# cv-stuttgart/PCFA

Hardware: AMD Instinct MI355X
Metric: attack_steps_per_sec (higher is better)
Workload: dtype f32; 1 GPU; RAFT, 1 synthetic 436x1024 pair per GPU (padded 440x1024), disjoint delta, change_of_variables, delta_bound=0.005, zero target, L-BFGS max_iter=10; weights=random:1234, parallelism=pairs sharded 1/GPU, closure_launch=hipGraph replay

## Files before the change

include/pcfa_hip.h:

```cpp
#ifndef PCFA_HIP_H
#define PCFA_HIP_H

#include <stddef.h>
#include <stdint.h>

#ifdef __cplusplus
extern "C" {
#endif

#define PCFA_OK 0
#define PCFA_ERR_INVALID_ARG (-1)
#define PCFA_ERR_UNSUPPORTED (-2)
#define PCFA_ERR_WORKSPACE (-3)

#if defined(__GNUC__)
#define PCFA_API __attribute__((visibility("default")))
#else
#define PCFA_API
#endif

#define PCFA_MAX_LEVELS 8
#define PCFA_ABI_VERSION 2

#define PCFA_LOSS_AEE 0
#define PCFA_LOSS_MSE 1
#define PCFA_LOSS_COSIM 2

#define PCFA_BOX_CLIPPING 0
#define PCFA_BOX_CHANGE_OF_VARIABLES 1

PCFA_API int pcfa_abi_version(void);
PCFA_API int pcfa_timing_arm(void* start_event, void* stop_event, int nth);

PCFA_API int pcfa_null_launch(void* stream);
PCFA_API int pcfa_poison_lds(unsigned pattern, void* stream);
PCFA_API int pcfa_peek_lds(unsigned* out, int n, void* stream);
PCFA_API long long pcfa_calib_mfma_f32(float* scratch, int blocks, int iters, void* stream);
PCFA_API int pcfa_calib_copy(const float* src, float* dst, long long n_floats, void* stream);
PCFA_API const char* pcfa_status_string(int status);


PCFA_API long long pcfa_corr_slab_floats(int H, int W, int num_levels);
PCFA_API long long pcfa_corr_level_offset(int H, int W, int num_levels, int level, int* h_l, int* w_l);

PCFA_API long long pcfa_corr_tiled_index(int H, int W, int num_levels, int level, int y, int x);

PCFA_API int pcfa_corr_f2ext_fwd(const float* fmap2, float* f2ext, int B, int D, int H, int W,
                        int num_levels, void* stream);

PCFA_API int pcfa_corr_pyramid_fwd(const float* fmap1, const float* f2ext, float* pyr, int B, int D,
                          int H, int W, int num_levels, void* stream);

PCFA_API size_t pcfa_corr_pyramid_bwd_workspace_bytes(int B, int D, int H, int W, int num_levels);
PCFA_API int pcfa_corr_pyramid_bwd(const float* dpyr, const float* fmap1, const float* f2ext,
                          float* dfmap1, float* dfmap2, void* workspace, size_t workspace_bytes,
                          int B, int D, int H, int W, int num_levels, void* stream);
PCFA_API size_t pcfa_corr_pyramid_bwd_windows_workspace_bytes(int B, int D, int H, int W, int num_levels);
PCFA_API int pcfa_corr_pyramid_bwd_windows(const float* dpyr, const float* fmap1, const float* f2ext, float* dfmap1,
                                  float* dfmap2, void* workspace, size_t workspace_bytes,
                                  const float* const* coords, int n_coords, int radius, int B, int D, int H, int W,
                                  int num_levels, void* stream);

PCFA_API int pcfa_corr_lookup_fwd(const float* pyr, const float* coords, float* out, int B, int H, int W,
                         int num_levels, int radius, void* stream);

PCFA_API int pcfa_corr_lookup_bwd(float* dpyr, const float* coords, const float* grad_out, int B, int H,
                         int W, int num_levels, int radius, void* stream);

PCFA_API size_t pcfa_corr_ondemand_workspace_bytes(int B, int D, int H, int W, int num_levels);
PCFA_API int pcfa_corr_ondemand_prepare(const float* fmap1, const float* fmap2, void* workspace, int B, int D, int H,
                               int W, int num_levels, void* stream);
PCFA_API int pcfa_corr_ondemand_fwd(const void* workspace, const float* coords, float* out, int B, int D, int H, int W,
                           int num_levels, int radius, void* stream);
PCFA_API int pcfa_corr_ondemand_bwd(void* workspace, const float* coords, const float* grad_out, int accumulate, int B,
                           int D, int H, int W, int num_levels, int radius, void* stream);
PCFA_API int pcfa_corr_ondemand_finish(const void* workspace, float* dfmap1, float* dfmap2, int B, int D, int H, int W,
                              int num_levels, void* stream);

PCFA_API size_t pcfa_gemm_f32_workspace_bytes(int M, int N, int batch, int splits);
PCFA_API int pcfa_gemm_f32(const float* A, const float* B, float* C, int M, int N, int K, long long lda, long long ldb,
                  long long ldc, int a_kmajor, int b_kmajor, int batch, long long bsA, long long bsB, long long bsC,
                  float alpha, int splits, void* workspace, size_t workspace_bytes, void* stream);
PCFA_API int pcfa_softmax_rows_fwd(const float* x, float* y, long long rows, int cols, void* stream);
PCFA_API int pcfa_softmax_rows_bwd(const float* y, const float* grad_y, float* grad_x, long long rows, int cols,
                          void* stream);

PCFA_API int pcfa_attn_stream_lse(const float* q, const float* k, float* lse, int BH, int N, int d, float scale,
                         void* stream);
PCFA_API int pcfa_attn_stream_fwd(const float* q, const float* k, const float* v, const float* lse, float* out, int BH,
                         int N, int d, float scale, void* stream);
PCFA_API int pcfa_attn_stream_dv(const float* q, const float* k, const float* g, const float* lse, float* dv, int BH,
                        int N, int d, float scale, void* stream);
PCFA_API int pcfa_attn_stream_delta(const float* g, const float* out, float* delta, long long rows, int d,
                           int accumulate, void* stream);
PCFA_API int pcfa_attn_stream_dqk(const float* q, const float* k, const float* lse, const float* G, const float* V,
                         const float* delta, float* dq, float* dk, int BH, int N, int d, int n, float scale,
                         void* stream);

PCFA_API long long pcfa_lookup_convc1_packed_floats(int Cout);
PCFA_API int pcfa_lookup_convc1_pack_weights(const float* weight, float* packed, int Cout, int Cin, void* stream);
PCFA_API int pcfa_lookup_convc1_fwd(const float* pyr, const float* coords, const float* packed, const float* bias,
                           float* out, int B, int H, int W, int num_levels, int radius, int Cout, int relu,
                           void* stream);
PCFA_API int pcfa_lookup_convc1_bwd(float* dpyr, const float* coords, const float* packed, const float* out,
                           const float* grad_out, int B, int H, int W, int num_levels, int radius, int Cout,
                           int relu, void* stream);

PCFA_API int pcfa_spatial_corr_out_size(int iH, int iW, int kH, int kW, int padH, int padW, int dilH,
                               int dilW, int dH, int dW, int* oH, int* oW);
PCFA_API int pcfa_spatial_corr_fwd(const float* in1, const float* in2, float* out, int B, int C, int iH,
                          int iW, int kH, int kW, int patchH, int patchW, int padH, int padW,
                          int dilH, int dilW, int dil_patchH, int dil_patchW, int dH, int dW,
                          void* stream);
PCFA_API int pcfa_spatial_corr_bwd(const float* in1, const float* in2, const float* grad_out,
                          float* grad_in1, float* grad_in2, int B, int C, int iH, int iW, int kH,
                          int kW, int patchH, int patchW, int padH, int padW, int dilH, int dilW,
                          int dil_patchH, int dil_patchW, int dH, int dW, void* stream);

PCFA_API int pcfa_cost_volume9_fwd(const float* in1, const float* in2, float* out, int B, int C, int iH, int iW,
                          float scale, float slope, void* stream);
PCFA_API int pcfa_cost_volume9_bwd(const float* in1, const float* in2, const float* fwd_out, const float* grad_out,
                          float* grad_in1, float* grad_in2, int B, int C, int iH, int iW, float scale,
                          float slope, void* stream);

PCFA_API int pcfa_flownet_corr_out_size(int H, int W, int pad_size, int kernel_size, int max_displacement,
                                        int stride1, int stride2, int* out_channels, int* oH, int* oW);
PCFA_API int pcfa_flownet_corr_fwd(const float* in1, const float* in2, float* out, int B, int C, int H, int W,
                                   int pad_size, int kernel_size, int max_displacement, int stride1, int stride2,
                                   void* stream);
PCFA_API int pcfa_flownet_corr_bwd(const float* in1, const float* in2, const float* grad_out, float* grad_in1,
                                   float* grad_in2, int B, int C, int H, int W, int pad_size, int kernel_size,
                                   int max_displacement, int stride1, int stride2, void* stream);
PCFA_API int pcfa_resample2d_fwd(const float* in1, const float* flow, float* out, int B, int C, int iH, int iW,
                                 int H, int W, int kernel_size, int bilinear, void* stream);
PCFA_API int pcfa_resample2d_bwd(const float* in1, const float* flow, const float* grad_out, float* grad_in1,
                                 float* grad_flow, int B, int C, int iH, int iW, int H, int W, int kernel_size,
                                 int bilinear, void* stream);
PCFA_API int pcfa_channelnorm_fwd(const float* in, float* out, int B, int C, long long plane, int norm_deg,
                                  void* stream);
PCFA_API int pcfa_channelnorm_bwd(const float* in, const float* out, const float* grad_out, float* grad_in, int B,
                                  int C, long long plane, int norm_deg, void* stream);


PCFA_API int pcfa_box_transform_fwd(const float* image, const float* delta, float* out, int B,
                           long long n_per_item, int change_of_variables, double eps_box,
                           float scale, void* stream);
PCFA_API int pcfa_box_transform_bwd(const float* image, const float* delta, const float* grad_out,
                           float* grad_image, float* grad_delta, int B, long long n_per_item,
                           int change_of_variables, double eps_box, float scale, void* stream);

PCFA_API int pcfa_pm1_pair_fwd(const float* image1, const float* image2, float* pair, float* ctx, int B, long long n,
                               void* stream);
PCFA_API int pcfa_pm1_pair_bwd(const float* grad_pair, const float* grad_ctx, float* grad_image1, float* grad_image2, int B,
                               long long n, void* stream);

PCFA_API int pcfa_extract_deltas_fwd(const float* nw_input, const float* image, float* delta,
                            long long n, int change_of_variables, double eps_box, void* stream);
PCFA_API int pcfa_extract_deltas_bwd(const float* nw_input, const float* grad_delta, float* grad_nw_input,
                            long long n, int change_of_variables, double eps_box, void* stream);

PCFA_API int pcfa_extract_deltas_joint_fwd(const float* nw_delta, const float* images_max,
                                  const float* images_min, float* delta, long long n,
                                  void* stream);
PCFA_API int pcfa_extract_deltas_joint_bwd(const float* nw_delta, const float* images_max,
                                  const float* images_min, const float* grad_delta,
                                  float* grad_nw_delta, long long n, void* stream);

PCFA_API size_t pcfa_flow_loss_workspace_bytes(void);
PCFA_API int pcfa_flow_loss_fwd(const float* pred, const long long pred_strides[4], const float* target,
                       const long long target_strides[4], int B, int H, int W,
                       const float* delta1, long long n1, const float* delta2, long long n2,
                       float delta_bound, float mu, int f_type, float* out_scalars,
                       void* workspace, void* stream);
PCFA_API int pcfa_flow_loss_bwd(const float* pred, const long long pred_strides[4], const float* target,
                       const long long target_strides[4], int B, int H, int W,
                       const float* delta1, long long n1, const float* delta2, long long n2,
                       float mu, int f_type, int joint, const float* fwd_scalars,
                       const float* grad_loss, float* grad_pred, float* grad_delta1,
                       float* grad_delta2, void* stream);

PCFA_API int pcfa_gru_gates_fwd(const float* zc, const float* rc, const float* h, const float* bias_z,
                       const float* bias_r, const float* add_z, const float* add_r, float* z, float* r,
                       float* rh, long long n, int plane, int channels, void* stream);
PCFA_API int pcfa_gru_gates_bwd(const float* z, const float* r, const float* h, const float* dz, const float* drh,
                       float* dzc, float* drc, float* dh, long long n, void* stream);
PCFA_API int pcfa_gru_gates_bwd_acc(const float* z, const float* r, const float* h, const float* dz, const float* drh,
                           const float* dh_in, float* dzc, float* drc, float* dh, long long n, void* stream);
PCFA_API int pcfa_gru_update_fwd(const float* z, const float* qc, const float* h, const float* bias_q,
                        const float* add_q, float* q, float* hnew, long long n, int plane, int channels,
                        void* stream);
PCFA_API int pcfa_gru_update_bwd(const float* z, const float* q, const float* h, const float* g, float* dz,
                        float* dqc, float* dh, long long n, void* stream);

PCFA_API long long pcfa_sepconv5_packed_floats(int Cout, int Cin);
PCFA_API int pcfa_sepconv5_algo(int use_winograd);
PCFA_API int pcfa_sepconv5_uses_winograd(int B, int Ca, int Cb, int Cout, int H, int W, int vertical);
PCFA_API int pcfa_sepconv5_pack_weights(const float* w, float* fwd_packed, float* bwd_packed, int Cout, int Cin,
                               void* stream);
PCFA_API int pcfa_sepconv5_fwd(const float* in_a, int Ca, const float* in_b, int Cb, const float* w_packed,
                      float* out, int B, int Cout, int H, int W, int vertical, void* stream);

PCFA_API int pcfa_sepconv5_fwd_split(const float* in_a, int Ca, const float* in_b, int Cb, const float* w_packed,
                            float* out_a, int Cout_a, int accumulate_a, float* out_b, int accumulate_b, int B,
                            int Cout, int H, int W, int vertical, void* stream);
PCFA_API int pcfa_sepconv5_fwd_split_masked(const float* in_a, int Ca, const float* in_b, int Cb, const float* w_packed,
                                   float* out_a, int Cout_a, int accumulate_a, float* out_b, int accumulate_b,
                                   const float* mask_b, int mask_channels, int B, int Cout, int H, int W,
                                   int vertical, void* stream);

PCFA_API int pcfa_sepconv5_gru_gates_fwd(const float* h, int C, const float* rest, int Cr, const float* w_packed,
                                const float* add_zr, float* z, float* r, float* rh, int B, int H, int W,
                                int vertical, void* stream);
PCFA_API int pcfa_sepconv5_gru_update_fwd(const float* rh, int C, const float* rest, int Cr, const float* w_packed,
                                 const float* add_q, const float* z, const float* h, float* q, float* hnew, int B,
                                 int H, int W, int vertical, void* stream);
PCFA_API int pcfa_sepconv5_gru_gates_bwd(const float* dqc, int C, int Cr, const float* w_packed_bwd, const float* z,
                                const float* r, const float* h, const float* dz, const float* dh_in, float* dzr,
                                float* dh, float* d_rest, int accumulate_rest, int B, int H, int W, int vertical,
                                void* stream);
PCFA_API int pcfa_sepconv5_gru_update_bwd(const float* dzr, int C, int Cr, const float* w_packed_bwd, const float* dh_acc,
                                 const float* z_prev, const float* q_prev, const float* h_prev, float* dz_prev,
                                 float* dqc_prev, float* dh_prev, float* d_rest, int B, int H, int W, int vertical,
                                 void* stream);

PCFA_API long long pcfa_conv3x3_packed_floats(int K, int N);
PCFA_API int pcfa_conv3x3_pack_weights(const float* w, float* fwd_packed, float* bwd_packed, int Cout, int Cin,
                              void* stream);
PCFA_API int pcfa_conv3x3_fwd(const float* x, const float* packed, const float* bias, float* out, int B, int K, int N,
                     int H, int W, int relu, void* stream);
PCFA_API int pcfa_conv3x3_act_fwd(const float* x, const float* packed, const float* bias, float* out, int B, int K,
                         int N, int H, int W, int act, float slope, void* stream);
PCFA_API int pcfa_leaky_relu_fwd(const float* x, float* y, float slope, long long n, void* stream);
PCFA_API int pcfa_leaky_relu_bwd(const float* out, const float* grad_out, float* grad_x, float slope, long long n,
                        void* stream);
PCFA_API int pcfa_conv3x3_act_fwd_pair(const float* x, const float* packed, const float* bias, float* out, int K, int N,
                              const float* x2, const float* packed2, const float* bias2, float* out2, int K2, int N2,
                              int H, int W, int act, float slope, void* stream);
PCFA_API int pcfa_conv3x3_fused_bwd(const float* g, const float* packed_bwd, const float* mask, const float* addend,
                           float* grad_in, int B, int K, int N, int H, int W, void* stream);
PCFA_API int pcfa_conv3x3_masked_fwd(const float* x, const float* packed, const float* mask, float* out, int B, int K,
                            int N, int H, int W, void* stream);
PCFA_API int pcfa_conv3x3_algo(int B, int K, int N, int H, int W);
PCFA_API size_t pcfa_conv3x3_workspace_bytes(int B, int K, int N, int H, int W);
PCFA_API int pcfa_conv3x3_run(const float* x, const float* packed, const float* bias, const float* mask,
                     const float* addend, float* out, int B, int K, int N, int H, int W, int act, float slope,
                     int mask_channels, void* workspace, size_t workspace_bytes, void* stream);

PCFA_API int pcfa_bias_relu_fwd(const float* x, const float* bias, float* out, long long n, int plane, int channels,
                       void* stream);
PCFA_API int pcfa_relu_bwd(const float* out, const float* grad_out, float* grad_x, long long n, void* stream);
PCFA_API int pcfa_relu_bwd2(const float* out, const float* out2, const float* grad_out, float* grad_x, float* grad_x2,
                   long long n, void* stream);

PCFA_API int pcfa_conv_fewin_fwd(const float* x, const float* w, const float* bias, float* out, int B, int Cin, int N,
                                 int H, int W, int ksize, int relu, void* stream);
PCFA_API long long pcfa_conv_fewin_packed_floats(int Cin, int N, int ksize);
PCFA_API int pcfa_conv_fewin_pack(const float* w, float* packed, int Cin, int N, int ksize, void* stream);
PCFA_API int pcfa_conv_fewin_packed_fwd(const float* x, const float* packed, const float* bias, float* out, int B, int Cin,
                               int N, int H, int W, int ksize, int relu, void* stream);

PCFA_API int pcfa_conv_s2_supported(int Cin, int N, int ksize, int H, int W);
PCFA_API long long pcfa_conv_s2_packed_floats(int Cin, int N, int ksize);
PCFA_API int pcfa_conv_s2_pack(const float* w, float* packed, int Cin, int N, int ksize, void* stream);
PCFA_API int pcfa_conv_s2_fwd(const float* x, const float* packed, const float* bias, float* out, int B, int Cin, int N,
                              int H, int W, int ksize, int act, float slope, void* stream);
PCFA_API int pcfa_conv_s2_bwd_supported(int Cin, int N, int ksize, int H, int W);
PCFA_API long long pcfa_conv_s2_bwd_packed_floats(int Cin, int N, int ksize);
PCFA_API int pcfa_conv_s2_bwd_pack(const float* w, float* packed, int Cin, int N, int ksize, void* stream);
PCFA_API int pcfa_conv_s2_bwd(const float* grad_out, const float* packed, float* grad_x, int B, int Cin, int N, int H, int W,
                              int ksize, void* stream);
PCFA_API long long pcfa_conv_s2_ds_packed_floats(int Cin, int N);
PCFA_API int pcfa_conv_s2_ds_pack(const float* w, const float* wd, float* packed, int Cin, int N, void* stream);
PCFA_API int pcfa_conv_s2_ds_fwd(const float* x, const float* packed, const float* bias, float* out, const float* bias_d,
                                 float* out_d, int B, int Cin, int N, int H, int W, int act, float slope, void* stream);
PCFA_API long long pcfa_conv_s2_ds_bwd_packed_floats(int Cin, int N);
PCFA_API int pcfa_conv_s2_ds_bwd_pack(const float* w, const float* wd, float* packed, int Cin, int N, void* stream);
PCFA_API int pcfa_conv_s2_ds_bwd(const float* grad_out, const float* grad_out_d, const float* packed, float* grad_x, int B,
                                 int Cin, int N, int H, int W, void* stream);

PCFA_API int pcfa_pwc_warp_fwd(const float* x, const float* flo, float* out, int B, int C, int H, int W,
                               float mask_threshold, float flow_scale, void* stream);
PCFA_API int pcfa_pwc_warp_bwd(const float* x, const float* flo, const float* grad_out, float* grad_x,
                               float* grad_flo, int B, int C, int H, int W, float mask_threshold, float flow_scale,
                               void* stream);
PCFA_API size_t pcfa_pwc_warp_bwd_det_workspace_bytes(int B, int C, int H, int W);
PCFA_API int pcfa_pwc_warp_bwd_det(const float* x, const float* flo, const float* grad_out, float* grad_x,
                          float* grad_flo, void* workspace, size_t workspace_bytes, int B, int C, int H, int W,
                          float mask_threshold, float flow_scale, void* stream);

PCFA_API int pcfa_spynet_warp_fwd(const float* x, const float* flo, const float* hor, const float* ver, float* out, int B,
                                  int C, int H, int W, float sx, float sy, void* stream);
PCFA_API size_t pcfa_spynet_warp_bwd_workspace_bytes(int B, int C, int H, int W);
PCFA_API int pcfa_spynet_warp_bwd(const float* x, const float* flo, const float* hor, const float* ver,
                                  const float* grad_out, float* grad_x, float* grad_flo, void* workspace,
                                  size_t workspace_bytes, int B, int C, int H, int W, float sx, float sy, void* stream);

PCFA_API int pcfa_conv7x7_tile(int Cout, int* mt, int* cot);
PCFA_API long long pcfa_conv7x7_packed_floats(int Cin, int Cout);
PCFA_API int pcfa_conv7x7(const float* x, const float* mask, const float* packed, const float* bias, const float* addend,
                          float* out, int B, int Cin, int Cout, int H, int W, int relu, void* stream);

PCFA_API int pcfa_conv_gather_tile(int Cout, int* mt, int* cot);
PCFA_API int pcfa_conv_gather_supported(int stride, int taps, int npar);
PCFA_API long long pcfa_conv_gather_packed_floats(int Cin, int Cout, int taps, int npar);
PCFA_API int pcfa_conv_gather(const float* x, const float* mask, float mask_slope, const float* packed, const float* bias,
                              float* out, int B, int Cin, int H, int W, int Cout, int OH, int OW, int stride, int taps,
                              int npar, int off0, int off1, int act, float slope, void* stream);

PCFA_API size_t pcfa_resample2d_bwd_det_workspace_bytes(int B, int C, int H, int W);
PCFA_API int pcfa_resample2d_bwd_det(const float* in1, const float* flow, const float* grad_out, float* grad_in1,
                                     float* grad_flow, void* workspace, size_t workspace_bytes, int B, int C, int H, int W,
                                     void* stream);

PCFA_API int pcfa_upsample_nearest4_fwd(const float* in, float* out, int planes, int H, int W, float s, int div,
                                        void* stream);
PCFA_API int pcfa_upsample_nearest4_bwd(const float* grad_out, float* grad_in, int planes, int H, int W, float s, int div,
                                        void* stream);

PCFA_API size_t pcfa_conv3x3_fewout_workspace_bytes(int B, int K, int N, int H, int W);
PCFA_API int pcfa_conv3x3_fewout_fwd(const float* x, const float* w, const float* bias, float* out, void* workspace,
                                     int B, int K, int N, int H, int W, void* stream);
PCFA_API int pcfa_conv3x3_fewout_bwd(const float* grad_out, const float* w, const float* addend, float* grad_x, int B,
                                     int K, int N, int H, int W, void* stream);

PCFA_API size_t pcfa_deconv4s2_fewout_workspace_bytes(int B, int K, int N, int H, int W);
PCFA_API int pcfa_deconv4s2_fewout_fwd(const float* x, const float* w, const float* bias, float* out, void* workspace,
                                       int B, int K, int N, int H, int W, void* stream);
PCFA_API int pcfa_deconv4s2_fewout_bwd(const float* grad_out, const float* w, float* grad_x, int B, int K, int N, int H,
                                       int W, void* stream);

PCFA_API int pcfa_upsample_bilinear_fwd(const float* in, float* out, int planes, int H, int W, int factor, float mul,
                                        void* stream);
PCFA_API int pcfa_upsample_bilinear_bwd(const float* grad_out, float* grad_in, int planes, int H, int W, int factor,
                                        float mul, void* stream);

PCFA_API size_t pcfa_instnorm_workspace_bytes(int planes, long long plane);
PCFA_API int pcfa_instnorm_fwd(const float* x, float* y, float* mean_rstd, void* workspace, int planes,
                               long long plane, float eps, int relu, void* stream);
PCFA_API int pcfa_instnorm_bwd(const float* x, const float* mean_rstd, const float* grad_out, float* grad_x,
                               void* workspace, int planes, long long plane, int relu, void* stream);
PCFA_API int pcfa_add_relu_fwd(const float* a, const float* b, float* out, long long n, void* stream);
PCFA_API int pcfa_convex_upsample_fwd(const float* flow, const float* mask, float* out, int N, int H, int W, void* stream);
PCFA_API long long pcfa_convex_upsample_workspace_floats(int N, int H, int W);
PCFA_API int pcfa_convex_upsample_bwd(const float* flow, const float* mask, const float* grad_out, float* grad_flow,
                             float* grad_mask, float* workspace, int N, int H, int W, void* stream);

PCFA_API int pcfa_flow_step(const float* coords1, const float* delta, const float* coords0, float* coords1_new,
                   float* flow_new, long long n, void* stream);

PCFA_API int pcfa_sum_n(const float* const* srcs, int n, float* out, long long numel, void* stream);

PCFA_API int pcfa_avg_epe(const float* flow1, const long long strides1[4], const float* flow2,
                 const long long strides2[4], int B, int H, int W, float* out, void* workspace,
                 void* stream);
PCFA_API int pcfa_sum_squares(const float* x, long long n, float* out, void* workspace, void* stream);

PCFA_API size_t pcfa_lbfgs_workspace_floats(void);
PCFA_API int pcfa_lbfgs_pair(const float* g, float* g_prev, const float* d, float t, float* y_out, float* s_out,
                             float* scal4, float* workspace, int update_prev, long long n, void* stream);
PCFA_API int pcfa_lbfgs_direction(const float* g, const float* S, const float* Y, const float* ro, const float* H,
                                  float* al, float* d, float* workspace, int first, int count, int capacity,
                                  long long ld, long long n, void* stream);

PCFA_API size_t pcfa_lbfgs_gram_state_bytes(int capacity);
PCFA_API size_t pcfa_lbfgs_gram_workspace_bytes(int capacity, long long ld);
PCFA_API int pcfa_lbfgs_gram_reset(void* state, int capacity, void* stream);
PCFA_API int pcfa_lbfgs_gram_update(const float* g, float* g_prev, const float* d, float t, float* S, float* Y,
                                    void* state, void* workspace, int capacity, long long ld, void* stream);
PCFA_API int pcfa_lbfgs_gram_direction(const float* g, const float* S, const float* Y, void* state, float* d,
                                       float* out_gtd_dmax, void* workspace, int capacity, long long ld, void* stream);

#ifdef __cplusplus
}
#endif
#endif
```

pcfa_amd/_hip.py:

```python
import ctypes
import os
from ctypes import c_char_p, c_double, c_float, c_int, c_longlong, c_size_t, c_uint, c_void_p, POINTER

ABI_VERSION = 2
LIB_PATH = os.environ.get("PCFA_HIP_LIB") or os.path.join(os.path.dirname(os.path.abspath(__file__)), "lib",
                                                          "libpcfa_hip.so")

PCFA_LOSS = {"aee": 0, "mse": 1, "cosim": 2}


class HipLibraryError(RuntimeError):
    pass


_P = c_void_p
_S4 = POINTER(c_longlong)

SIGNATURES = {
    "pcfa_abi_version": (c_int, []),
    "pcfa_timing_arm": (c_int, [_P, _P, c_int]),
    "pcfa_null_launch": (c_int, [_P]),
    "pcfa_poison_lds": (c_int, [c_uint, _P]),
    "pcfa_peek_lds": (c_int, [_P, c_int, _P]),
    "pcfa_calib_mfma_f32": (c_longlong, [_P, c_int, c_int, _P]),
    "pcfa_calib_copy": (c_int, [_P, _P, c_longlong, _P]),
    "pcfa_status_string": (c_char_p, [c_int]),
    "pcfa_corr_slab_floats": (c_longlong, [c_int, c_int, c_int]),
    "pcfa_corr_level_offset": (c_longlong, [c_int, c_int, c_int, c_int, POINTER(c_int), POINTER(c_int)]),
    "pcfa_corr_tiled_index": (c_longlong, [c_int, c_int, c_int, c_int, c_int, c_int]),
    "pcfa_corr_f2ext_fwd": (c_int, [_P, _P, c_int, c_int, c_int, c_int, c_int, _P]),
    "pcfa_corr_pyramid_fwd": (c_int, [_P, _P, _P, c_int, c_int, c_int, c_int, c_int, _P]),
    "pcfa_corr_pyramid_bwd_workspace_bytes": (c_size_t, [c_int, c_int, c_int, c_int, c_int]),
    "pcfa_corr_pyramid_bwd": (c_int, [_P, _P, _P, _P, _P, _P, c_size_t, c_int, c_int, c_int, c_int, c_int, _P]),
    "pcfa_corr_pyramid_bwd_windows_workspace_bytes": (c_size_t, [c_int, c_int, c_int, c_int, c_int]),
    "pcfa_corr_pyramid_bwd_windows": (c_int, [_P, _P, _P, _P, _P, _P, c_size_t, POINTER(c_void_p), c_int, c_int, c_int,
                                              c_int, c_int, c_int, c_int, _P]),
    "pcfa_corr_lookup_fwd": (c_int, [_P, _P, _P, c_int, c_int, c_int, c_int, c_int, _P]),
    "pcfa_corr_lookup_bwd": (c_int, [_P, _P, _P, c_int, c_int, c_int, c_int, c_int, _P]),
    "pcfa_corr_ondemand_workspace_bytes": (c_size_t, [c_int, c_int, c_int, c_int, c_int]),
    "pcfa_corr_ondemand_prepare": (c_int, [_P, _P, _P, c_int, c_int, c_int, c_int, c_int, _P]),
    "pcfa_corr_ondemand_fwd": (c_int, [_P, _P, _P, c_int, c_int, c_int, c_int, c_int, c_int, _P]),
    "pcfa_corr_ondemand_bwd": (c_int, [_P, _P, _P, c_int, c_int, c_int, c_int, c_int, c_int, c_int, _P]),
    "pcfa_corr_ondemand_finish": (c_int, [_P, _P, _P, c_int, c_int, c_int, c_int, c_int, _P]),
    "pcfa_gemm_f32_workspace_bytes": (c_size_t, [c_int, c_int, c_int, c_int]),
    "pcfa_gemm_f32": (c_int, [_P, _P, _P, c_int, c_int, c_int, c_longlong, c_longlong, c_longlong, c_int, c_int, c_int,
                              c_longlong, c_longlong, c_longlong, c_float, c_int, _P, c_size_t, _P]),
    "pcfa_softmax_rows_fwd": (c_int, [_P, _P, c_longlong, c_int, _P]),
    "pcfa_softmax_rows_bwd": (c_int, [_P, _P, _P, c_longlong, c_int, _P]),
    "pcfa_attn_stream_lse": (c_int, [_P, _P, _P, c_int, c_int, c_int, c_float, _P]),
    "pcfa_attn_stream_fwd": (c_int, [_P, _P, _P, _P, _P, c_int, c_int, c_int, c_float, _P]),
    "pcfa_attn_stream_dv": (c_int, [_P, _P, _P, _P, _P, c_int, c_int, c_int, c_float, _P]),
    "pcfa_attn_stream_delta": (c_int, [_P, _P, _P, c_longlong, c_int, c_int, _P]),
    "pcfa_attn_stream_dqk": (c_int, [_P, _P, _P, _P, _P, _P, _P, _P, c_int, c_int, c_int, c_int, c_float, _P]),
    "pcfa_lookup_convc1_packed_floats": (c_longlong, [c_int]),
    "pcfa_lookup_convc1_pack_weights": (c_int, [_P, _P, c_int, c_int, _P]),
    "pcfa_lookup_convc1_fwd": (c_int, [_P, _P, _P, _P, _P, c_int, c_int, c_int, c_int, c_int, c_int, c_int, _P]),
    "pcfa_lookup_convc1_bwd": (c_int, [_P, _P, _P, _P, _P, c_int, c_int, c_int, c_int, c_int, c_int, c_int, _P]),
    "pcfa_spatial_corr_out_size": (c_int, [c_int] * 10 + [POINTER(c_int), POINTER(c_int)]),
    "pcfa_spatial_corr_fwd": (c_int, [_P, _P, _P] + [c_int] * 16 + [_P]),
    "pcfa_spatial_corr_bwd": (c_int, [_P, _P, _P, _P, _P] + [c_int] * 16 + [_P]),
    "pcfa_cost_volume9_fwd": (c_int, [_P, _P, _P, c_int, c_int, c_int, c_int, c_float, c_float, _P]),
    "pcfa_cost_volume9_bwd": (c_int, [_P, _P, _P, _P, _P, _P, c_int, c_int, c_int, c_int, c_float, c_float, _P]),
    "pcfa_flownet_corr_out_size": (c_int, [c_int] * 7 + [POINTER(c_int)] * 3),
    "pcfa_flownet_corr_fwd": (c_int, [_P, _P, _P] + [c_int] * 9 + [_P]),
    "pcfa_flownet_corr_bwd": (c_int, [_P, _P, _P, _P, _P] + [c_int] * 9 + [_P]),
    "pcfa_resample2d_fwd": (c_int, [_P, _P, _P] + [c_int] * 8 + [_P]),
    "pcfa_resample2d_bwd": (c_int, [_P, _P, _P, _P, _P] + [c_int] * 8 + [_P]),
    "pcfa_channelnorm_fwd": (c_int, [_P, _P, c_int, c_int, c_longlong, c_int, _P]),
    "pcfa_channelnorm_bwd": (c_int, [_P, _P, _P, _P, c_int, c_int, c_longlong, c_int, _P]),
    "pcfa_box_transform_fwd": (c_int, [_P, _P, _P, c_int, c_longlong, c_int, c_double, c_float, _P]),
    "pcfa_box_transform_bwd": (c_int, [_P, _P, _P, _P, _P, c_int, c_longlong, c_int, c_double, c_float, _P]),
    "pcfa_pm1_pair_fwd": (c_int, [_P, _P, _P, _P, c_int, c_longlong, _P]),
    "pcfa_pm1_pair_bwd": (c_int, [_P, _P, _P, _P, c_int, c_longlong, _P]),
    "pcfa_extract_deltas_fwd": (c_int, [_P, _P, _P, c_longlong, c_int, c_double, _P]),
    "pcfa_extract_deltas_bwd": (c_int, [_P, _P, _P, c_longlong, c_int, c_double, _P]),
    "pcfa_extract_deltas_joint_fwd": (c_int, [_P, _P, _P, _P, c_longlong, _P]),
    "pcfa_extract_deltas_joint_bwd": (c_int, [_P, _P, _P, _P, _P, c_longlong, _P]),
    "pcfa_flow_loss_workspace_bytes": (c_size_t, []),
    "pcfa_flow_loss_fwd": (c_int, [_P, _S4, _P, _S4, c_int, c_int, c_int, _P, c_longlong, _P, c_longlong,
                                   c_float, c_float, c_int, _P, _P, _P]),
    "pcfa_flow_loss_bwd": (c_int, [_P, _S4, _P, _S4, c_int, c_int, c_int, _P, c_longlong, _P, c_longlong,
                                   c_float, c_int, c_int, _P, _P, _P, _P, _P, _P]),
    "pcfa_gru_gates_fwd": (c_int, [_P] * 10 + [c_longlong, c_int, c_int, _P]),
    "pcfa_gru_gates_bwd": (c_int, [_P] * 8 + [c_longlong, _P]),
    "pcfa_gru_update_fwd": (c_int, [_P] * 7 + [c_longlong, c_int, c_int, _P]),
    "pcfa_gru_update_bwd": (c_int, [_P] * 7 + [c_longlong, _P]),
    "pcfa_sepconv5_packed_floats": (c_longlong, [c_int, c_int]),
    "pcfa_sepconv5_algo": (c_int, [c_int]),
    "pcfa_sepconv5_uses_winograd": (c_int, [c_int] * 7),
    "pcfa_sepconv5_pack_weights": (c_int, [_P, _P, _P, c_int, c_int, _P]),
    "pcfa_sepconv5_fwd": (c_int, [_P, c_int, _P, c_int, _P, _P, c_int, c_int, c_int, c_int, c_int, _P]),
    "pcfa_sepconv5_fwd_split": (c_int, [_P, c_int, _P, c_int, _P, _P, c_int, c_int, _P, c_int, c_int, c_int, c_int, c_int,
                                        c_int, _P]),
    "pcfa_gru_gates_bwd_acc": (c_int, [_P, _P, _P, _P, _P, _P, _P, _P, _P, c_longlong, _P]),
    "pcfa_sepconv5_fwd_split_masked": (c_int, [_P, c_int, _P, c_int, _P, _P, c_int, c_int, _P, c_int, _P, c_int, c_int,
                                               c_int, c_int, c_int, c_int, _P]),
    "pcfa_sepconv5_gru_gates_fwd": (c_int, [_P, c_int, _P, c_int, _P, _P, _P, _P, _P, c_int, c_int, c_int, c_int, _P]),
    "pcfa_sepconv5_gru_update_fwd": (c_int, [_P, c_int, _P, c_int, _P, _P, _P, _P, _P, _P, c_int, c_int, c_int, c_int, _P]),
    "pcfa_sepconv5_gru_gates_bwd": (c_int, [_P, c_int, c_int, _P, _P, _P, _P, _P, _P, _P, _P, _P, c_int, c_int, c_int,
                                            c_int, c_int, _P]),
    "pcfa_sepconv5_gru_update_bwd": (c_int, [_P, c_int, c_int, _P, _P, _P, _P, _P, _P, _P, _P, _P, c_int, c_int, c_int,
                                             c_int, _P]),
    "pcfa_convex_upsample_fwd": (c_int, [_P, _P, _P, c_int, c_int, c_int, _P]),
    "pcfa_convex_upsample_workspace_floats": (c_longlong, [c_int, c_int, c_int]),
    "pcfa_convex_upsample_bwd": (c_int, [_P, _P, _P, _P, _P, _P, c_int, c_int, c_int, _P]),
    "pcfa_flow_step": (c_int, [_P, _P, _P, _P, _P, c_longlong, _P]),
    "pcfa_conv3x3_act_fwd_pair": (c_int, [_P, _P, _P, _P, c_int, c_int, _P, _P, _P, _P, c_int, c_int, c_int, c_int, c_int,
                                          c_float, _P]),
    "pcfa_relu_bwd2": (c_int, [_P, _P, _P, _P, _P, c_longlong, _P]),
    "pcfa_conv3x3_fused_bwd": (c_int, [_P, _P, _P, _P, _P, c_int, c_int, c_int, c_int, c_int, _P]),
    "pcfa_conv3x3_masked_fwd": (c_int, [_P, _P, _P, _P, c_int, c_int, c_int, c_int, c_int, _P]),
    "pcfa_conv3x3_algo": (c_int, [c_int] * 5),
    "pcfa_conv3x3_workspace_bytes": (c_size_t, [c_int] * 5),
    "pcfa_conv3x3_run": (c_int, [_P] * 6 + [c_int] * 6 + [c_float, c_int, _P, c_size_t, _P]),
    "pcfa_conv3x3_packed_floats": (c_longlong, [c_int, c_int]),
    "pcfa_conv3x3_pack_weights": (c_int, [_P, _P, _P, c_int, c_int, _P]),
    "pcfa_conv3x3_fwd": (c_int, [_P, _P, _P, _P, c_int, c_int, c_int, c_int, c_int, c_int, _P]),
    "pcfa_conv3x3_act_fwd": (c_int, [_P, _P, _P, _P, c_int, c_int, c_int, c_int, c_int, c_int, c_float, _P]),
    "pcfa_leaky_relu_fwd": (c_int, [_P, _P, c_float, c_longlong, _P]),
    "pcfa_leaky_relu_bwd": (c_int, [_P, _P, _P, c_float, c_longlong, _P]),
    "pcfa_lbfgs_gram_state_bytes": (c_size_t, [c_int]),
    "pcfa_lbfgs_gram_workspace_bytes": (c_size_t, [c_int, c_longlong]),
    "pcfa_lbfgs_gram_reset": (c_int, [_P, c_int, _P]),
    "pcfa_lbfgs_gram_update": (c_int, [_P, _P, _P, c_float, _P, _P, _P, _P, c_int, c_longlong, _P]),
    "pcfa_lbfgs_gram_direction": (c_int, [_P, _P, _P, _P, _P, _P, _P, c_int, c_longlong, _P]),
    "pcfa_lbfgs_workspace_floats": (c_size_t, []),
    "pcfa_lbfgs_pair": (c_int, [_P, _P, _P, c_float, _P, _P, _P, _P, c_int, c_longlong, _P]),
    "pcfa_lbfgs_direction": (c_int, [_P, _P, _P, _P, _P, _P, _P, _P, c_int, c_int, c_int, c_longlong, c_longlong,
                                     _P]),
    "pcfa_bias_relu_fwd": (c_int, [_P, _P, _P, c_longlong, c_int, c_int, _P]),
    "pcfa_relu_bwd": (c_int, [_P, _P, _P, c_longlong, _P]),
    "pcfa_conv_fewin_packed_floats": (c_longlong, [c_int, c_int, c_int]),
    "pcfa_conv_s2_supported": (c_int, [c_int, c_int, c_int, c_int, c_int]),
    "pcfa_conv_s2_packed_floats": (c_longlong, [c_int, c_int, c_int]),
    "pcfa_conv_s2_pack": (c_int, [_P, _P, c_int, c_int, c_int, _P]),
    "pcfa_conv_s2_fwd": (c_int, [_P, _P, _P, _P, c_int, c_int, c_int, c_int, c_int, c_int, c_int, c_float, _P]),
    "pcfa_conv_s2_bwd_supported": (c_int, [c_int, c_int, c_int, c_int, c_int]),
    "pcfa_conv_s2_bwd_packed_floats": (c_longlong, [c_int, c_int, c_int]),
    "pcfa_conv_s2_bwd_pack": (c_int, [_P, _P, c_int, c_int, c_int, _P]),
    "pcfa_conv_s2_bwd": (c_int, [_P, _P, _P, c_int, c_int, c_int, c_int, c_int, c_int, _P]),
    "pcfa_conv_s2_ds_packed_floats": (c_longlong, [c_int, c_int]),
    "pcfa_conv_s2_ds_pack": (c_int, [_P, _P, _P, c_int, c_int, _P]),
    "pcfa_conv_s2_ds_fwd": (c_int, [_P, _P, _P, _P, _P, _P, c_int, c_int, c_int, c_int, c_int, c_int, c_float, _P]),
    "pcfa_conv_s2_ds_bwd_packed_floats": (c_longlong, [c_int, c_int]),
    "pcfa_conv_s2_ds_bwd_pack": (c_int, [_P, _P, _P, c_int, c_int, _P]),
    "pcfa_conv_s2_ds_bwd": (c_int, [_P, _P, _P, _P, c_int, c_int, c_int, c_int, c_int, _P]),
    "pcfa_conv_fewin_pack": (c_int, [_P, _P, c_int, c_int, c_int, _P]),
    "pcfa_conv_fewin_packed_fwd": (c_int, [_P, _P, _P, _P, c_int, c_int, c_int, c_int, c_int, c_int, c_int, _P]),
    "pcfa_conv_fewin_fwd": (c_int, [_P, _P, _P, _P, c_int, c_int, c_int, c_int, c_int, c_int, c_int, _P]),
    "pcfa_pwc_warp_fwd": (c_int, [_P, _P, _P, c_int, c_int, c_int, c_int, c_float, c_float, _P]),
    "pcfa_pwc_warp_bwd": (c_int, [_P, _P, _P, _P, _P, c_int, c_int, c_int, c_int, c_float, c_float, _P]),
    "pcfa_pwc_warp_bwd_det_workspace_bytes": (c_size_t, [c_int, c_int, c_int, c_int]),
    "pcfa_pwc_warp_bwd_det": (c_int, [_P, _P, _P, _P, _P, _P, c_size_t, c_int, c_int, c_int, c_int, c_float, c_float, _P]),
    "pcfa_conv3x3_fewout_workspace_bytes": (c_size_t, [c_int, c_int, c_int, c_int, c_int]),
    "pcfa_conv3x3_fewout_fwd": (c_int, [_P, _P, _P, _P, _P, c_int, c_int, c_int, c_int, c_int, _P]),
    "pcfa_conv3x3_fewout_bwd": (c_int, [_P, _P, _P, _P, c_int, c_int, c_int, c_int, c_int, _P]),
    "pcfa_deconv4s2_fewout_workspace_bytes": (c_size_t, [c_int, c_int, c_int, c_int, c_int]),
    "pcfa_deconv4s2_fewout_fwd": (c_int, [_P, _P, _P, _P, _P, c_int, c_int, c_int, c_int, c_int, _P]),
    "pcfa_deconv4s2_fewout_bwd": (c_int, [_P, _P, _P, c_int, c_int, c_int, c_int, c_int, _P]),
    "pcfa_spynet_warp_fwd": (c_int, [_P, _P, _P, _P, _P, c_int, c_int, c_int, c_int, c_float, c_float, _P]),
    "pcfa_spynet_warp_bwd_workspace_bytes": (c_size_t, [c_int, c_int, c_int, c_int]),
    "pcfa_spynet_warp_bwd": (c_int, [_P, _P, _P, _P, _P, _P, _P, _P, c_size_t, c_int, c_int, c_int, c_int, c_float, c_float,
                                     _P]),
    "pcfa_conv7x7_tile": (c_int, [c_int, POINTER(c_int), POINTER(c_int)]),
    "pcfa_conv7x7_packed_floats": (c_longlong, [c_int, c_int]),
    "pcfa_conv7x7": (c_int, [_P, _P, _P, _P, _P, _P, c_int, c_int, c_int, c_int, c_int, c_int, _P]),
    "pcfa_conv_gather_tile": (c_int, [c_int, POINTER(c_int), POINTER(c_int)]),
    "pcfa_conv_gather_supported": (c_int, [c_int, c_int, c_int]),
    "pcfa_conv_gather_packed_floats": (c_longlong, [c_int, c_int, c_int, c_int]),
    "pcfa_conv_gather": (c_int, [_P, _P, c_float, _P, _P, _P] + [c_int] * 12 + [c_int, c_float, _P]),
    "pcfa_resample2d_bwd_det_workspace_bytes": (c_size_t, [c_int, c_int, c_int, c_int]),
    "pcfa_resample2d_bwd_det": (c_int, [_P, _P, _P, _P, _P, _P, c_size_t, c_int, c_int, c_int, c_int, _P]),
    "pcfa_upsample_nearest4_fwd": (c_int, [_P, _P, c_int, c_int, c_int, c_float, c_int, _P]),
    "pcfa_upsample_nearest4_bwd": (c_int, [_P, _P, c_int, c_int, c_int, c_float, c_int, _P]),
    "pcfa_upsample_bilinear_fwd": (c_int, [_P, _P, c_int, c_int, c_int, c_int, c_float, _P]),
    "pcfa_upsample_bilinear_bwd": (c_int, [_P, _P, c_int, c_int, c_int, c_int, c_float, _P]),
    "pcfa_instnorm_workspace_bytes": (c_size_t, [c_int, c_longlong]),
    "pcfa_instnorm_fwd": (c_int, [_P, _P, _P, _P, c_int, c_longlong, c_float, c_int, _P]),
    "pcfa_instnorm_bwd": (c_int, [_P, _P, _P, _P, _P, c_int, c_longlong, c_int, _P]),
    "pcfa_add_relu_fwd": (c_int, [_P, _P, _P, c_longlong, _P]),
    "pcfa_sum_n": (c_int, [POINTER(c_void_p), c_int, _P, c_longlong, _P]),
    "pcfa_avg_epe": (c_int, [_P, _S4, _P, _S4, c_int, c_int, c_int, _P, _P, _P]),
    "pcfa_sum_squares": (c_int, [_P, c_longlong, _P, _P, _P]),
}

_lib = None


def load(path=None):
    global _lib
    if _lib is not None and path is None:
        return _lib
    p = path or LIB_PATH
    if not os.path.exists(p):
        raise HipLibraryError(
            "libpcfa_hip.so not found at %s -- build it with `python -c 'import __graft_entry__ as g; g.build()'` "
            "or `make -C pcfa_amd/csrc`. pcfa_amd has no CPU fallback." % p)
    try:
        lib = ctypes.CDLL(p)
    except OSError as e:
        raise HipLibraryError("cannot load %s: %s" % (p, e))
    for name, (res, args) in SIGNATURES.items():
        try:
            fn = getattr(lib, name)
        except AttributeError:
            raise HipLibraryError("%s does not export %s (stale build?)" % (p, name))
        fn.restype = res
        fn.argtypes = args
    v = lib.pcfa_abi_version()
    if v != ABI_VERSION:
        raise HipLibraryError("ABI version mismatch: library %d, binding %d" % (v, ABI_VERSION))
    if path is None:
        _lib = lib
    return lib


def check(status, what):
    if status != 0:
        msg = load().pcfa_status_string(status)
        raise RuntimeError("%s failed: %s (status %d)" % (what, msg.decode() if msg else "?", status))


def strides4(t):
    return (c_longlong * 4)(*t.stride())
```

pcfa_amd/csrc/conv3x3_fewout.hip:

```cpp
#include "common.hpp"

namespace {

constexpr int FO_PX = 64;
constexpr int FO_WAVES = 8;
constexpr int FO_FWD_WAVES = 16;

template <int N>
__global__ __launch_bounds__(FO_PX* FO_FWD_WAVES) void conv3x3_fewout_fwd_kernel(
    const float* __restrict__ x, const float* __restrict__ w, const float* __restrict__ bias,
    float* __restrict__ out, int K, int H, int W, int splits, int kper) {
  __shared__ float red[FO_FWD_WAVES][N][FO_PX];
  const int lane = threadIdx.x & 63;
  const int wave = __builtin_amdgcn_readfirstlane(threadIdx.x >> 6);
  const int nb = gridDim.y / splits;
  const int b = blockIdx.y / splits, split = blockIdx.y - b * splits;
  const int kbeg = split * kper, kend = min(K, kbeg + kper);
  const long long plane = (long long)H * W;
  const long long p = (long long)blockIdx.x * FO_PX + lane;
  const bool live = p < plane;
  const int y = live ? (int)(p / W) : 0, xx = live ? (int)(p % W) : 0;
  int off[9];
  bool ok[9];
#pragma unroll
  for (int ky = 0; ky < 3; ++ky)
#pragma unroll
    for (int kx = 0; kx < 3; ++kx) {
      const int yy = y + ky - 1, xq = xx + kx - 1;
      ok[ky * 3 + kx] = live && yy >= 0 && yy < H && xq >= 0 && xq < W;
      off[ky * 3 + kx] = ok[ky * 3 + kx] ? yy * W + xq : 0;
    }
  float acc[N];
#pragma unroll
  for (int o = 0; o < N; ++o) acc[o] = 0.f;
  const float* xb = x + (size_t)b * K * plane;
  constexpr int U = 8;
  for (int c0 = kbeg + wave; c0 < kend; c0 += U * FO_FWD_WAVES) {
    float v[U][9];
#pragma unroll
    for (int u = 0; u < U; ++u) {
      const int c = c0 + u * FO_FWD_WAVES;
      const float* xc = xb + (size_t)(c < kend ? c : c0) * plane;
#pragma unroll
      for (int k = 0; k < 9; ++k) {
        const float t = xc[off[k]];
        v[u][k] = ok[k] ? t : 0.f;
      }
    }
#pragma unroll
    for (int u = 0; u < U; ++u) {
      const int c = c0 + u * FO_FWD_WAVES;
      if (c < kend) {
#pragma unroll
        for (int o = 0; o < N; ++o) {
          const float* wc = w + ((size_t)o * K + c) * 9;
#pragma unroll
          for (int k = 0; k < 9; ++k) acc[o] += wc[k] * v[u][k];
        }
      }
    }
  }
#pragma unroll
  for (int o = 0; o < N; ++o) red[wave][o][lane] = acc[o];
  __syncthreads();
  for (int e = threadIdx.x; e < N * FO_PX; e += FO_PX * FO_FWD_WAVES) {
    const int o = e / FO_PX, l = e % FO_PX;
    float s = 0.f;
#pragma unroll
    for (int g = 0; g < FO_FWD_WAVES; ++g) s += red[g][o][l];
    const long long q = (long long)blockIdx.x * FO_PX + l;
    if (q < plane) {
      if (splits > 1) out[(((size_t)split * nb + b) * N + o) * plane + q] = s;
      else out[((size_t)b * N + o) * plane + q] = s + (bias ? bias[o] : 0.f);
    }
  }
}

constexpr int FO_SEG = 72;
constexpr int FO_UL = 4;

template <int N>
__global__ __launch_bounds__(FO_PX* FO_FWD_WAVES) void conv3x3_fewout_fwd_lds_kernel(
    const float* __restrict__ x, const float* __restrict__ w, const float* __restrict__ bias,
    float* __restrict__ out, int K, int H, int W, int splits, int kper) {
  typedef float f32x4 __attribute__((ext_vector_type(4)));
  __shared__ float red[FO_FWD_WAVES][N][FO_PX];
  __shared__ __attribute__((aligned(16))) float seg[FO_FWD_WAVES][FO_UL][3][FO_SEG];
  const int lane = threadIdx.x & 63;
  const int wave = __builtin_amdgcn_readfirstlane(threadIdx.x >> 6);
  const int nb = gridDim.y / splits;
  const int b = blockIdx.y / splits, split = blockIdx.y - b * splits;
  const int kbeg = split * kper, kend = min(K, kbeg + kper);
  const long long plane = (long long)H * W;
  const long long p0 = (long long)blockIdx.x * FO_PX;
  const long long p = p0 + lane;
  const bool live = p < plane;
  const int y = live ? (int)(p / W) : 0, xx = live ? (int)(p % W) : 0;
  bool ok[9];
#pragma unroll
  for (int ky = 0; ky < 3; ++ky)
#pragma unroll
    for (int kx = 0; kx < 3; ++kx) {
      const int yy = y + ky - 1, xq = xx + kx - 1;
      ok[ky * 3 + kx] = live && yy >= 0 && yy < H && xq >= 0 && xq < W;
    }
  const int lr = lane / 18, lm = lane - lr * 18;
  long long s4[3];
  int dsh[3];
#pragma unroll
  for (int r = 0; r < 3; ++r) {
    const long long st = p0 + (long long)(r - 1) * W - 1;
    s4[r] = st & ~3LL;
    dsh[r] = (int)(st - s4[r]);
  }
  const long long myidx = (lr == 0 ? s4[0] : (lr == 1 ? s4[1] : s4[2])) + 4 * lm;
  const bool myok = lane < 54 && myidx >= 0 && myidx + 3 < plane;
  const long long myoff = myok ? myidx : 0;

  float acc[N];
#pragma unroll
  for (int o = 0; o < N; ++o) acc[o] = 0.f;
  const float* xb = x + (size_t)b * K * plane;
  float* mine = &seg[wave][0][0][0];
  for (int c0 = kbeg + wave; c0 < kend; c0 += FO_UL * FO_FWD_WAVES) {
    f32x4 t[FO_UL];
#pragma unroll
    for (int u = 0; u < FO_UL; ++u) {
      const int c = c0 + u * FO_FWD_WAVES;
      const float* xc = xb + (size_t)(c < kend ? c : c0) * plane;
      const f32x4 q = *reinterpret_cast<const f32x4*>(xc + myoff);
      t[u] = myok ? q : (f32x4)(0.f);
    }
#pragma unroll
    for (int u = 0; u < FO_UL; ++u)
      if (lane < 54) *reinterpret_cast<f32x4*>(mine + (u * 3 + lr) * FO_SEG + 4 * lm) = t[u];
    __builtin_amdgcn_wave_barrier();
#pragma unroll
    for (int u = 0; u < FO_UL; ++u) {
      const int c = c0 + u * FO_FWD_WAVES;
      if (c < kend) {
        float v[9];
#pragma unroll
        for (int r = 0; r < 3; ++r)
#pragma unroll
          for (int kx = 0; kx < 3; ++kx) {
            const float q = mine[(u * 3 + r) * FO_SEG + dsh[r] + lane + kx];
            v[3 * r + kx] = ok[3 * r + kx] ? q : 0.f;
          }
#pragma unroll
        for (int o = 0; o < N; ++o) {
          const float* wc = w + ((size_t)o * K + c) * 9;
#pragma unroll
          for (int k = 0; k < 9; ++k) acc[o] += wc[k] * v[k];
        }
      }
    }
    __builtin_amdgcn_wave_barrier();
  }
#pragma unroll
  for (int o = 0; o < N; ++o) red[wave][o][lane] = acc[o];
  __syncthreads();
  for (int e = threadIdx.x; e < N * FO_PX; e += FO_PX * FO_FWD_WAVES) {
    const int o = e / FO_PX, l = e % FO_PX;
    float sum = 0.f;
#pragma unroll
    for (int g = 0; g < FO_FWD_WAVES; ++g) sum += red[g][o][l];
    const long long q = p0 + l;
    if (q < plane) {
      if (splits > 1) out[(((size_t)split * nb + b) * N + o) * plane + q] = sum;
      else out[((size_t)b * N + o) * plane + q] = sum + (bias ? bias[o] : 0.f);
    }
  }
}

__global__ void fewout_reduce_kernel(const float* __restrict__ part, const float* __restrict__ bias,
                                     float* __restrict__ out, long long n, long long plane, int N, int splits) {
  const long long step = (long long)gridDim.x * blockDim.x;
  for (long long i = (long long)blockIdx.x * blockDim.x + threadIdx.x; i < n; i += step) {
    float s = 0.f;
    for (int k = 0; k < splits; ++k) s += part[(size_t)k * n + i];
    out[i] = s + (bias ? bias[(i / plane) % N] : 0.f);
  }
}

template <int N>
__global__ __launch_bounds__(FO_PX* FO_WAVES) void conv3x3_fewout_bwd_kernel(
    const float* __restrict__ gout, const float* __restrict__ w, const float* __restrict__ addend, float* __restrict__ gx,
    int K, int H, int W, int csplit) {
  const int lane = threadIdx.x & 63;
  const int wave = __builtin_amdgcn_readfirstlane(threadIdx.x >> 6);
  const int b = blockIdx.y / csplit, part = blockIdx.y % csplit;
  const long long plane = (long long)H * W;
  const long long p = (long long)blockIdx.x * FO_PX + lane;
  const bool live = p < plane;
  const int y = live ? (int)(p / W) : 0, xx = live ? (int)(p % W) : 0;
  float g[N][9];
  const float* gb = gout + (size_t)b * N * plane;
#pragma unroll
  for (int ky = 0; ky < 3; ++ky)
#pragma unroll
    for (int kx = 0; kx < 3; ++kx) {
      const int yy = y + 1 - ky, xq = xx + 1 - kx;
      const bool ok = live && yy >= 0 && yy < H && xq >= 0 && xq < W;
      const int o_ = ok ? yy * W + xq : 0;
#pragma unroll
      for (int o = 0; o < N; ++o) {
        const float t = gb[(size_t)o * plane + o_];
        g[o][ky * 3 + kx] = ok ? t : 0.f;
      }
    }
  float* xb = gx + (size_t)b * K * plane;
  const float* ab = addend != nullptr ? addend + (size_t)b * K * plane : nullptr;
  constexpr int U = 4;
  const int cstep = FO_WAVES * csplit;
  for (int c0 = part * FO_WAVES + wave; c0 < K; c0 += U * cstep) {
    float s[U], a[U];
#pragma unroll
    for (int u = 0; u < U; ++u) {
      const int c = c0 + u * cstep;
      a[u] = (ab != nullptr && c < K && live) ? ab[(size_t)c * plane + p] : 0.f;
    }
#pragma unroll
    for (int u = 0; u < U; ++u) {
      const int c = c0 + u * cstep;
      s[u] = 0.f;
      if (c < K) {
#pragma unroll
        for (int o = 0; o < N; ++o) {
          const float* wc = w + ((size_t)o * K + c) * 9;
#pragma unroll
          for (int k = 0; k < 9; ++k) s[u] += wc[k] * g[o][k];
        }
      }
    }
#pragma unroll
    for (int u = 0; u < U; ++u) {
      const int c = c0 + u * cstep;
      if (c < K && live) xb[(size_t)c * plane + p] = s[u] + a[u];
    }
  }
}


template <int N>
__global__ __launch_bounds__(FO_PX* FO_FWD_WAVES) void deconv4s2_fewout_fwd_kernel(
    const float* __restrict__ x, const float* __restrict__ w, const float* __restrict__ bias,
    float* __restrict__ out, int K, int H, int W, int splits, int kper) {
  __shared__ float red[FO_FWD_WAVES][4 * N][FO_PX];
  const int lane = threadIdx.x & 63;
  const int wave = __builtin_amdgcn_readfirstlane(threadIdx.x >> 6);
  const int nb = gridDim.y / splits;
  const int b = blockIdx.y / splits, split = blockIdx.y - b * splits;
  const int kbeg = split * kper, kend = min(K, kbeg + kper);
  const long long plane = (long long)H * W;
  const long long p = (long long)blockIdx.x * FO_PX + lane;
  const bool live = p < plane;
  const int y = live ? (int)(p / W) : 0, xx = live ? (int)(p % W) : 0;
  int off[9];
  bool ok[9];
#pragma unroll
  for (int ky = 0; ky < 3; ++ky)
#pragma unroll
    for (int kx = 0; kx < 3; ++kx) {
      const int yy = y + ky - 1, xq = xx + kx - 1;
      ok[ky * 3 + kx] = live && yy >= 0 && yy < H && xq >= 0 && xq < W;
      off[ky * 3 + kx] = ok[ky * 3 + kx] ? yy * W + xq : 0;
    }
  float acc[4][N];
#pragma unroll
  for (int q = 0; q < 4; ++q)
#pragma unroll
    for (int o = 0; o < N; ++o) acc[q][o] = 0.f;
  const float* xb = x + (size_t)b * K * plane;
  constexpr int U = 4;
  for (int c0 = kbeg + wave; c0 < kend; c0 += U * FO_FWD_WAVES) {
    float v[U][9];
#pragma unroll
    for (int u = 0; u < U; ++u) {
      const int c = c0 + u * FO_FWD_WAVES;
      const float* xc = xb + (size_t)(c < kend ? c : c0) * plane;
#pragma unroll
      for (int k = 0; k < 9; ++k) {
        const float t = xc[off[k]];
        v[u][k] = ok[k] ? t : 0.f;
      }
    }
#pragma unroll
    for (int u = 0; u < U; ++u) {
      const int c = c0 + u * FO_FWD_WAVES;
      if (c < kend) {
#pragma unroll
        for (int o = 0; o < N; ++o) {
          const float* wc = w + ((size_t)c * N + o) * 16;
#pragma unroll
          for (int a = 0; a < 2; ++a)
#pragma unroll
            for (int bb = 0; bb < 2; ++bb)
#pragma unroll
              for (int ty = 0; ty < 2; ++ty)
#pragma unroll
                for (int tx = 0; tx < 2; ++tx) {
                  const int dy = a ? 1 - ty : -ty, ky = a ? 2 * ty : 1 + 2 * ty;
                  const int dx = bb ? 1 - tx : -tx, kx = bb ? 2 * tx : 1 + 2 * tx;
                  acc[a * 2 + bb][o] += wc[ky * 4 + kx] * v[u][(dy + 1) * 3 + dx + 1];
                }
        }
      }
    }
  }
#pragma unroll
  for (int q = 0; q < 4; ++q)
#pragma unroll
    for (int o = 0; o < N; ++o) red[wave][q * N + o][lane] = acc[q][o];
  __syncthreads();
  const long long oplane = 4 * plane;
  for (int e = threadIdx.x; e < 4 * N * FO_PX; e += FO_PX * FO_FWD_WAVES) {
    const int qo = e / FO_PX, l = e % FO_PX;
    const int q = qo / N, o = qo - q * N;
    float s = 0.f;
#pragma unroll
    for (int g = 0; g < FO_FWD_WAVES; ++g) s += red[g][qo][l];
    const long long pp = (long long)blockIdx.x * FO_PX + l;
    if (pp < plane) {
      const int py = (int)(pp / W), px = (int)(pp % W);
      const long long oi = (long long)(2 * py + (q >> 1)) * (2 * W) + 2 * px + (q & 1);
      if (splits > 1) out[(((size_t)split * nb + b) * N + o) * oplane + oi] = s;
      else out[((size_t)b * N + o) * oplane + oi] = s + (bias ? bias[o] : 0.f);
    }
  }
}

template <int N>
__global__ __launch_bounds__(FO_PX* FO_WAVES) void deconv4s2_fewout_bwd_kernel(
    const float* __restrict__ gout, const float* __restrict__ w, float* __restrict__ gx, int K, int H, int W,
    int csplit) {
  const int lane = threadIdx.x & 63;
  const int wave = __builtin_amdgcn_readfirstlane(threadIdx.x >> 6);
  const int b = blockIdx.y / csplit, part = blockIdx.y % csplit;
  const long long plane = (long long)H * W;
  const long long p = (long long)blockIdx.x * FO_PX + lane;
  const bool live = p < plane;
  const int y = live ? (int)(p / W) : 0, xx = live ? (int)(p % W) : 0;
  const int OH = 2 * H, OW = 2 * W;
  float g[N][16];
  const float* gb = gout + (size_t)b * N * 4 * plane;
#pragma unroll
  for (int ky = 0; ky < 4; ++ky)
#pragma unroll
    for (int kx = 0; kx < 4; ++kx) {
      const int yy = 2 * y - 1 + ky, xq = 2 * xx - 1 + kx;
      const bool ok = live && yy >= 0 && yy < OH && xq >= 0 && xq < OW;
      const long long o_ = ok ? (long long)yy * OW + xq : 0;
#pragma unroll
      for (int o = 0; o < N; ++o) {
        const float t = gb[(size_t)o * 4 * plane + o_];
        g[o][ky * 4 + kx] = ok ? t : 0.f;
      }
    }
  float* xb = gx + (size_t)b * K * plane;
  constexpr int U = 4;
  const int cstep = FO_WAVES * csplit;
  for (int c0 = part * FO_WAVES + wave; c0 < K; c0 += U * cstep) {
    float s[U];
#pragma unroll
    for (int u = 0; u < U; ++u) {
      const int c = c0 + u * cstep;
      s[u] = 0.f;
      if (c < K) {
#pragma unroll
        for (int o = 0; o < N; ++o) {
          const float* wc = w + ((size_t)c * N + o) * 16;
#pragma unroll
          for (int k = 0; k < 16; ++k) s[u] += wc[k] * g[o][k];
        }
      }
    }
#pragma unroll
    for (int u = 0; u < U; ++u) {
      const int c = c0 + u * cstep;
      if (c < K && live) xb[(size_t)c * plane + p] = s[u];
    }
  }
}

}

static int fewout_splits(int B, int K, long long plane) {
  const long long tiles = (long long)pcfa_cdiv(plane, FO_PX) * B;
  long long want = (256 + tiles - 1) / tiles;
  const long long by_k = K / 64 > 0 ? K / 64 : 1;
  if (want > by_k) want = by_k;
  if (want > 64) want = 64;
  return want < 4 ? 1 : (int)want;
}

extern "C" size_t pcfa_conv3x3_fewout_workspace_bytes(int B, int K, int N, int H, int W) {
  if (B < 1 || K < 1 || N < 1 || N > 4 || H < 1 || W < 1) return 0;
  const long long plane = (long long)H * W;
  const int splits = fewout_splits(B, K, plane);
  return splits > 1 ? (size_t)splits * B * N * plane * sizeof(float) : 0;
}

extern "C" int pcfa_conv3x3_fewout_fwd(const float* x, const float* w, const float* bias, float* out,
                                       void* workspace, int B, int K, int N, int H, int W, void* stream) {
  if (!x || !w || !out || B < 1 || K < 1 || H < 1 || W < 1) return PCFA_ERR_INVALID_ARG;
  if (N < 1 || N > 4) return PCFA_ERR_UNSUPPORTED;
  const long long plane = (long long)H * W;
  const int splits = fewout_splits(B, K, plane);
  if (splits > 1 && !workspace) return PCFA_ERR_WORKSPACE;
  const int kper = ((K + splits - 1) / splits + FO_FWD_WAVES - 1) / FO_FWD_WAVES * FO_FWD_WAVES;
  float* dst = splits > 1 ? (float*)workspace : out;
  dim3 grid(pcfa_cdiv(plane, FO_PX), B * splits), block(FO_PX * FO_FWD_WAVES);
  hipStream_t s = (hipStream_t)stream;
  const bool wide = plane % 4 == 0 && (reinterpret_cast<uintptr_t>(x) & 15) == 0;
  if (wide) {
    switch (N) {
      case 1: pcfa_launch(conv3x3_fewout_fwd_lds_kernel<1>, grid, block, 0, s, x, w, bias, dst, K, H, W, splits, kper); break;
      case 2: pcfa_launch(conv3x3_fewout_fwd_lds_kernel<2>, grid, block, 0, s, x, w, bias, dst, K, H, W, splits, kper); break;
      case 3: pcfa_launch(conv3x3_fewout_fwd_lds_kernel<3>, grid, block, 0, s, x, w, bias, dst, K, H, W, splits, kper); break;
      default: pcfa_launch(conv3x3_fewout_fwd_lds_kernel<4>, grid, block, 0, s, x, w, bias, dst, K, H, W, splits, kper); break;
    }
  } else {
    switch (N) {
      case 1: pcfa_launch(conv3x3_fewout_fwd_kernel<1>, grid, block, 0, s, x, w, bias, dst, K, H, W, splits, kper); break;
      case 2: pcfa_launch(conv3x3_fewout_fwd_kernel<2>, grid, block, 0, s, x, w, bias, dst, K, H, W, splits, kper); break;
      case 3: pcfa_launch(conv3x3_fewout_fwd_kernel<3>, grid, block, 0, s, x, w, bias, dst, K, H, W, splits, kper); break;
      default: pcfa_launch(conv3x3_fewout_fwd_kernel<4>, grid, block, 0, s, x, w, bias, dst, K, H, W, splits, kper); break;
    }
  }
  PCFA_LAUNCH_CHECK();
  if (splits > 1) {
    const long long n = (long long)B * N * plane;
    long long blocks = (n + 255) / 256;
    if (blocks > 1024) blocks = 1024;
    pcfa_launch(fewout_reduce_kernel, dim3((int)blocks), dim3(256), 0, s, (const float*)workspace, bias, out, n, plane,
                N, splits);
    PCFA_LAUNCH_CHECK();
  }
  return PCFA_OK;
}

extern "C" int pcfa_conv3x3_fewout_bwd(const float* grad_out, const float* w, const float* addend, float* grad_x, int B,
                                       int K, int N, int H, int W, void* stream) {
  if (!grad_out || !w || !grad_x || B < 1 || K < 1 || H < 1 || W < 1) return PCFA_ERR_INVALID_ARG;
  if (N < 1 || N > 4) return PCFA_ERR_UNSUPPORTED;
  const long long plane = (long long)H * W;
  const int tiles = pcfa_cdiv(plane, FO_PX) * B;
  int csplit = 1;
  while (tiles * csplit < 512 && FO_WAVES * csplit * 2 <= K) csplit *= 2;
  dim3 grid(pcfa_cdiv(plane, FO_PX), B * csplit), block(FO_PX * FO_WAVES);
  hipStream_t s = (hipStream_t)stream;
  switch (N) {
    case 1: pcfa_launch(conv3x3_fewout_bwd_kernel<1>, grid, block, 0, s, grad_out, w, addend, grad_x, K, H, W, csplit); break;
    case 2: pcfa_launch(conv3x3_fewout_bwd_kernel<2>, grid, block, 0, s, grad_out, w, addend, grad_x, K, H, W, csplit); break;
    case 3: pcfa_launch(conv3x3_fewout_bwd_kernel<3>, grid, block, 0, s, grad_out, w, addend, grad_x, K, H, W, csplit); break;
    default: pcfa_launch(conv3x3_fewout_bwd_kernel<4>, grid, block, 0, s, grad_out, w, addend, grad_x, K, H, W, csplit); break;
  }
  PCFA_LAUNCH_CHECK();
  return PCFA_OK;
}

static int deconv_splits(int B, int K, long long plane) {
  const long long tiles = (long long)pcfa_cdiv(plane, FO_PX) * B;
  long long want = (256 + tiles - 1) / tiles;
  const long long by_k = K / 64 > 0 ? K / 64 : 1;
  if (want > by_k) want = by_k;
  if (want > 64) want = 64;
  return want < 4 ? 1 : (int)want;
}

extern "C" size_t pcfa_deconv4s2_fewout_workspace_bytes(int B, int K, int N, int H, int W) {
  if (B < 1 || K < 1 || N < 1 || N > 4 || H < 1 || W < 1) return 0;
  const long long plane = (long long)H * W;
  const int splits = deconv_splits(B, K, plane);
  return splits > 1 ? (size_t)splits * B * N * 4 * plane * sizeof(float) : 0;
}

extern "C" int pcfa_deconv4s2_fewout_fwd(const float* x, const float* w, const float* bias, float* out,
                                         void* workspace, int B, int K, int N, int H, int W, void* stream) {
  if (!x || !w || !out || B < 1 || K < 1 || H < 1 || W < 1) return PCFA_ERR_INVALID_ARG;
  if (N < 1 || N > 4) return PCFA_ERR_UNSUPPORTED;
  const long long plane = (long long)H * W;
  const int splits = deconv_splits(B, K, plane);
  if (splits > 1 && !workspace) return PCFA_ERR_WORKSPACE;
  const int kper = ((K + splits - 1) / splits + FO_FWD_WAVES - 1) / FO_FWD_WAVES * FO_FWD_WAVES;
  float* dst = splits > 1 ? (float*)workspace : out;
  dim3 grid(pcfa_cdiv(plane, FO_PX), B * splits), block(FO_PX * FO_FWD_WAVES);
  hipStream_t s = (hipStream_t)stream;
  switch (N) {
    case 1: pcfa_launch(deconv4s2_fewout_fwd_kernel<1>, grid, block, 0, s, x, w, bias, dst, K, H, W, splits, kper); break;
    case 2: pcfa_launch(deconv4s2_fewout_fwd_kernel<2>, grid, block, 0, s, x, w, bias, dst, K, H, W, splits, kper); break;
    case 3: pcfa_launch(deconv4s2_fewout_fwd_kernel<3>, grid, block, 0, s, x, w, bias, dst, K, H, W, splits, kper); break;
    default: pcfa_launch(deconv4s2_fewout_fwd_kernel<4>, grid, block, 0, s, x, w, bias, dst, K, H, W, splits, kper); break;
  }
  PCFA_LAUNCH_CHECK();
  if (splits > 1) {
    const long long n = (long long)B * N * 4 * plane;
    long long blocks = (n + 255) / 256;
    if (blocks > 1024) blocks = 1024;
    pcfa_launch(fewout_reduce_kernel, dim3((int)blocks), dim3(256), 0, s, (const float*)workspace, bias, out, n,
                4 * plane, N, splits);
    PCFA_LAUNCH_CHECK();
  }
  return PCFA_OK;
}

extern "C" int pcfa_deconv4s2_fewout_bwd(const float* grad_out, const float* w, float* grad_x, int B, int K, int N,
                                         int H, int W, void* stream) {
  if (!grad_out || !w || !grad_x || B < 1 || K < 1 || H < 1 || W < 1) return PCFA_ERR_INVALID_ARG;
  if (N < 1 || N > 4) return PCFA_ERR_UNSUPPORTED;
  const long long plane = (long long)H * W;
  const int tiles = pcfa_cdiv(plane, FO_PX) * B;
  int csplit = 1;
  while (tiles * csplit < 512 && FO_WAVES * csplit * 2 <= K) csplit *= 2;
  dim3 grid(pcfa_cdiv(plane, FO_PX), B * csplit), block(FO_PX * FO_WAVES);
  hipStream_t s = (hipStream_t)stream;
  switch (N) {
    case 1: pcfa_launch(deconv4s2_fewout_bwd_kernel<1>, grid, block, 0, s, grad_out, w, grad_x, K, H, W, csplit); break;
    case 2: pcfa_launch(deconv4s2_fewout_bwd_kernel<2>, grid, block, 0, s, grad_out, w, grad_x, K, H, W, csplit); break;
    case 3: pcfa_launch(deconv4s2_fewout_bwd_kernel<3>, grid, block, 0, s, grad_out, w, grad_x, K, H, W, csplit); break;
    default: pcfa_launch(deconv4s2_fewout_bwd_kernel<4>, grid, block, 0, s, grad_out, w, grad_x, K, H, W, csplit); break;
  }
  PCFA_LAUNCH_CHECK();
  return PCFA_OK;
}
```

pcfa_amd/nets/raft.py:

```python

import torch
import torch.nn as nn
import torch.nn.functional as F

from .. import ops
from ..config import cfg


def _norm(kind, planes):
    if kind == 'batch':
        return nn.BatchNorm2d(planes)
    if kind == 'instance':
        return nn.InstanceNorm2d(planes)
    if kind == 'group':
        return nn.GroupNorm(num_groups=planes // 8, num_channels=planes)
    if kind == 'none':
        return nn.Sequential()
    raise ValueError("unknown norm_fn %r" % kind)


def _fold_batchnorm(conv, bn, cache, tag):
    tensors = (conv.weight, conv.bias, bn.weight, bn.bias, bn.running_mean, bn.running_var)
    key = tuple((t.data_ptr(), t._version) for t in tensors if t is not None) + (conv.weight.device,)
    hit = cache.get(tag)
    if hit is None or hit[0] != key:
        with torch.no_grad():
            s = torch.rsqrt(bn.running_var + bn.eps)
            if bn.weight is not None:
                s = s * bn.weight
            b = -bn.running_mean if conv.bias is None else conv.bias - bn.running_mean
            b = b * s
            if bn.bias is not None:
                b = b + bn.bias
            hit = (key, (conv.weight * s[:, None, None, None]).contiguous(), b.contiguous())
        cache[tag] = hit
    return hit[1], hit[2]




def _conv_norm(conv, norm, x, relu, cache, tag, skip=False, grad_premasked=False, mask_input_grad=False):
    frozen = not (conv.weight.requires_grad or (conv.bias is not None and conv.bias.requires_grad))
    if (frozen and isinstance(norm, nn.BatchNorm2d) and not norm.training and norm.track_running_stats
            and not (norm.affine and (norm.weight.requires_grad or norm.bias.requires_grad))):
        w, b = _fold_batchnorm(conv, norm, cache, tag)
        if _is_plain3x3(conv):
            return ops.get().conv3x3(x, w, b, relu, skip=skip, grad_premasked=grad_premasked,
                                     mask_input_grad=mask_input_grad)
        assert not (skip or grad_premasked or mask_input_grad)
        if _is_stride2(conv, x, cfg(conv)):
            return ops.get().conv_s2(x, w, b, relu, own_bwd=cfg(conv).conv_s2_bwd)
        if relu:
            return ops.get().bias_relu(conv._conv_forward(x, w, None), b)
        return conv._conv_forward(x, w, b)
    if (frozen and isinstance(norm, nn.InstanceNorm2d) and not norm.affine and not norm.track_running_stats):
        xs = None
        if _is_plain3x3(conv):
            y = ops.get().conv3x3(x, conv.weight, None, False, skip=skip)
            if skip:
                y, xs = y
        elif _is_stride2(conv, x, cfg(conv)):
            assert not skip
            y = ops.get().conv_s2(x, conv.weight, None, False, own_bwd=cfg(conv).conv_s2_bwd)
        else:
            assert not skip
            y = conv._conv_forward(x, conv.weight, None)
        y = ops.get().instance_norm_relu(y, norm.eps, relu)
        return (y, xs) if skip else y
    assert not skip
    y = norm(conv(x))
    return F.relu(y, inplace=True) if relu else y


def _is_stride2(conv, x, conf):
    k = conv.kernel_size[0]
    return (conf.conv_s2 and conv.kernel_size == (k, k) and conv.stride == (2, 2) and conv.padding == (k // 2, k // 2)
            and conv.dilation == (1, 1) and conv.groups == 1 and conv.padding_mode == "zeros"
            and ops.get().conv_s2_supported(x, conv.weight))


def _can_skip(conv, norm):
    frozen = not (conv.weight.requires_grad or (conv.bias is not None and conv.bias.requires_grad))
    if not (frozen and _is_plain3x3(conv)):
        return False
    if isinstance(norm, nn.BatchNorm2d):
        return (not norm.training and norm.track_running_stats
                and not (norm.affine and (norm.weight.requires_grad or norm.bias.requires_grad)))
    return isinstance(norm, nn.InstanceNorm2d) and not norm.affine and not norm.track_running_stats


class ResidualBlock(nn.Module):
    def __init__(self, in_planes, planes, norm_fn='group', stride=1):
        super().__init__()
        self.conv1 = nn.Conv2d(in_planes, planes, kernel_size=3, padding=1, stride=stride)
        self.conv2 = nn.Conv2d(planes, planes, kernel_size=3, padding=1)
        self.relu = nn.ReLU(inplace=True)
        self.norm1 = _norm(norm_fn, planes)
        self.norm2 = _norm(norm_fn, planes)
        self.downsample = None
        if stride != 1:
            self.norm3 = _norm(norm_fn, planes)
            self.downsample = nn.Sequential(nn.Conv2d(in_planes, planes, kernel_size=1, stride=stride), self.norm3)
        self._fold_cache = {}

    def _entry_pair(self, x):
        conv1, convd, n1, nd = self.conv1, self.downsample[0], self.norm1, self.downsample[1]
        o = ops.get()
        if not (cfg(self).fused_downsample and _all_frozen(self) and conv1.stride == (2, 2) and convd.stride == (2, 2)
                and convd.kernel_size == (1, 1) and convd.padding == (0, 0) and _is_stride2(conv1, x, cfg(self))
                and o.conv_s2_ds_supported(x, conv1.weight, convd.weight)):
            return None
        if all(isinstance(n, nn.BatchNorm2d) and not n.training and n.track_running_stats for n in (n1, nd)):
            w1, b1 = _fold_batchnorm(conv1, n1, self._fold_cache, "1")
            wd, bd = _fold_batchnorm(convd, nd, self._fold_cache, "d")
            if not o.conv_s2_ds_supported(x, w1, wd):
                return None
            return o.conv_s2_ds(x, w1, wd, b1, bd, relu=True)
        if all(isinstance(n, nn.InstanceNorm2d) and not n.affine and not n.track_running_stats for n in (n1, nd)):
            y, xd = o.conv_s2_ds(x, conv1.weight, convd.weight)
            return o.instance_norm_relu(y, n1.eps, True), o.instance_norm_relu(xd, nd.eps, False)
        return None

    def forward(self, x):
        pair = self._entry_pair(x) if self.downsample is not None else None
        if pair is not None:
            y, xd = pair
            y = _conv_norm(self.conv2, self.norm2, y, True, self._fold_cache, "2")
            return ops.get().add_relu(xd, y)
        if self.downsample is None and _all_frozen(self) and _can_skip(self.conv1, self.norm1):
            y, x = _conv_norm(self.conv1, self.norm1, x, True, self._fold_cache, "1", skip=True,
                              grad_premasked=cfg(self).defer_relu and isinstance(self.norm1, nn.BatchNorm2d) and isinstance(self.norm2, nn.BatchNorm2d)
                              and _can_skip(self.conv2, self.norm2))
        else:
            y = _conv_norm(self.conv1, self.norm1, x, True, self._fold_cache, "1")
        chain = (cfg(self).defer_relu and _all_frozen(self) and isinstance(self.norm2, nn.BatchNorm2d) and _can_skip(self.conv2, self.norm2)
                 and _can_skip(self.conv1, self.norm1) and self.downsample is None)
        y = _conv_norm(self.conv2, self.norm2, y, True, self._fold_cache, "2", grad_premasked=chain, mask_input_grad=chain)
        if self.downsample is not None:
            x = _conv_norm(self.downsample[0], self.downsample[1], x, False, self._fold_cache, "d")
        if _all_frozen(self):
            return ops.get().add_relu(x, y, b_is_relu=chain)
        return self.relu(x + y)


class BasicEncoder(nn.Module):

    def __init__(self, output_dim=128, norm_fn='batch', dropout=0.0):
        super().__init__()
        self.norm_fn = norm_fn
        self.norm1 = nn.GroupNorm(num_groups=8, num_channels=64) if norm_fn == 'group' else _norm(norm_fn, 64)
        self.conv1 = nn.Conv2d(3, 64, kernel_size=7, stride=2, padding=3)
        self.relu1 = nn.ReLU(inplace=True)
        self.layer1 = self._stage(64, 64, 1)
        self.layer2 = self._stage(64, 96, 2)
        self.layer3 = self._stage(96, 128, 2)
        self.conv2 = nn.Conv2d(128, output_dim, kernel_size=1)
        self.dropout = nn.Dropout2d(p=dropout) if dropout > 0 else None
        self._fold_cache = {}
        for m in self.modules():
            if isinstance(m, nn.Conv2d):
                nn.init.kaiming_normal_(m.weight, mode='fan_out', nonlinearity='relu')
            elif isinstance(m, (nn.BatchNorm2d, nn.InstanceNorm2d, nn.GroupNorm)):
                if m.weight is not None:
                    nn.init.constant_(m.weight, 1)
                if m.bias is not None:
                    nn.init.constant_(m.bias, 0)

    def _stage(self, cin, cout, stride):
        return nn.Sequential(ResidualBlock(cin, cout, self.norm_fn, stride=stride),
                             ResidualBlock(cout, cout, self.norm_fn, stride=1))

    def forward(self, x, split=None):
        pair = isinstance(x, (tuple, list)) or split is not None
        if split is not None:
            n = split
        elif pair:
            n = x[0].shape[0]
            x = torch.cat(x, dim=0)
        x = _conv_norm(self.conv1, self.norm1, x, True, self._fold_cache, "1")
        x = self.layer3(self.layer2(self.layer1(x)))
        x = _conv1x1(self.conv2, x, cfg(self))
        if self.training and self.dropout is not None:
            x = self.dropout(x)
        if pair:
            x = torch.split(x, [n, n], dim=0)
        return x


def _all_frozen(module):
    return not any(p.requires_grad for p in module.parameters())


def _conv_nobias(conv, x):
    return conv._conv_forward(x, conv.weight, None)


def _is_plain3x3(conv, min_out=16):
    return (conv.kernel_size == (3, 3) and conv.stride == (1, 1) and conv.padding == (1, 1) and conv.dilation == (1, 1)
            and conv.groups == 1 and conv.padding_mode == "zeros" and conv.out_channels >= min_out)


def _is_plain1x1(conv):
    return (conv.kernel_size == (1, 1) and conv.stride == (1, 1) and conv.padding == (0, 0) and conv.dilation == (1, 1)
            and conv.groups == 1)


def _conv1x1(conv, x, config):
    if config.conv1x1 == "hip" and x.is_cuda and _is_plain1x1(conv) and _frozen_conv(conv):
        return ops.get().conv1x1(x, conv.weight, conv.bias)
    return conv(x)


def _frozen_conv(conv):
    return not (conv.weight.requires_grad or (conv.bias is not None and conv.bias.requires_grad))


def _conv_relu(conv, x):
    if _is_plain3x3(conv) and _frozen_conv(conv):
        return ops.get().conv3x3(x, conv.weight, conv.bias, True)
    o = ops.get()
    k = conv.kernel_size[0]
    if (_frozen_conv(conv) and not x.requires_grad and conv.kernel_size == (k, k) and conv.stride == (1, 1)
            and conv.padding == (k // 2, k // 2) and conv.dilation == (1, 1) and conv.groups == 1
            and conv.padding_mode == "zeros" and (conv.in_channels, k) in o.FEWIN_SHAPES):
        return o.conv_fewin(x, conv.weight, conv.bias, True)
    return o.bias_relu(_conv_nobias(conv, x), conv.bias)


def _predict_flow(conv, x):
    if (conv.kernel_size == (3, 3) and conv.stride == (1, 1) and conv.padding == (1, 1) and conv.dilation == (1, 1)
            and conv.groups == 1 and conv.padding_mode == "zeros" and conv.out_channels <= 4 and _frozen_conv(conv)):
        return ops.get().conv3x3_fewout(x, conv.weight, conv.bias)
    return conv(x)


class FlowHead(nn.Module):
    def __init__(self, input_dim=128, hidden_dim=256):
        super().__init__()
        self.conv1 = nn.Conv2d(input_dim, hidden_dim, 3, padding=1)
        self.conv2 = nn.Conv2d(hidden_dim, 2, 3, padding=1)
        self.relu = nn.ReLU(inplace=True)

    def forward(self, x):
        return _predict_flow(self.conv2, _conv_relu(self.conv1, x))


class SepConvGRU(nn.Module):

    def __init__(self, hidden_dim=128, input_dim=192 + 128, const_dim=128):
        super().__init__()
        c = hidden_dim + input_dim
        self.hidden_dim, self.const_dim = hidden_dim, const_dim
        self.convz1 = nn.Conv2d(c, hidden_dim, (1, 5), padding=(0, 2))
        self.convr1 = nn.Conv2d(c, hidden_dim, (1, 5), padding=(0, 2))
        self.convq1 = nn.Conv2d(c, hidden_dim, (1, 5), padding=(0, 2))
        self.convz2 = nn.Conv2d(c, hidden_dim, (5, 1), padding=(2, 0))
        self.convr2 = nn.Conv2d(c, hidden_dim, (5, 1), padding=(2, 0))
        self.convq2 = nn.Conv2d(c, hidden_dim, (5, 1), padding=(2, 0))
        self._split_cache = {}

    @staticmethod
    def _half(h, x, convz, convr, convq):
        o = ops.get()
        hx = torch.cat([h, x], dim=1)
        z, rh = o.gru_gates(_conv_nobias(convz, hx), _conv_nobias(convr, hx), h, convz.bias, convr.bias)
        return o.gru_update(z, _conv_nobias(convq, torch.cat([rh, x], dim=1)), h, convq.bias)

    def forward(self, h, x):
        h = self._half(h, x, self.convz1, self.convr1, self.convq1)
        return self._half(h, x, self.convz2, self.convr2, self.convq2)

    def frozen(self):
        return not any(p.requires_grad for p in self.parameters())

    def _split(self, tag, convs):
        key = tuple((c.weight.data_ptr(), c.weight._version) for c in convs) + (convs[0].weight.device,)
        hit = self._split_cache.get(tag)
        if hit is None or hit[0] != key:
            hd, cd = self.hidden_dim, self.const_dim
            with torch.no_grad():
                w = torch.cat([c.weight for c in convs], dim=0)
                b = torch.cat([c.bias for c in convs], dim=0).contiguous()
                w_dyn = torch.cat([w[:, :hd], w[:, hd + cd:]], dim=1).contiguous()
                w_const = w[:, hd:hd + cd].contiguous()
            hit = (key, w_dyn, w_const, b)
            self._split_cache[tag] = hit
        return hit[1:]

    def precompute(self, inp):
        ctx = {}
        for tag, convs in (("zr1", (self.convz1, self.convr1)), ("q1", (self.convq1,)),
                           ("zr2", (self.convz2, self.convr2)), ("q2", (self.convq2,))):
            w_dyn, w_const, b = self._split(tag, convs)
            ctx[tag] = (w_dyn, ops.get().sepconv5(inp, None, w_const) + b.view(1, -1, 1, 1))
        return ctx

    def per_iteration(self, ctx, iters):
        fans = {tag: ops.get().fanout(p, iters) for tag, (_, p) in ctx.items()}
        return [{tag: (ctx[tag][0], fans[tag][i]) for tag in ctx} for i in range(iters)]

    def step(self, h, ctx, rest, rest_relu_channels=0):
        return ops.get().gru_step(h, rest, tuple(ctx[zr] + ctx[q] for zr, q in (("zr1", "q1"), ("zr2", "q2"))),
                                  rest_relu_channels)


class LookupRef:

    def __init__(self, corr_fn, coords):
        self.corr_fn, self.coords = corr_fn, coords

    def tensor(self):
        return self.corr_fn(self.coords)

    def conv_relu(self, conv):
        fused = getattr(self.corr_fn, "lookup_conv_relu", None)
        if fused is not None and _frozen_conv(conv) and cfg(conv).fused_lookup:
            out = fused(self.coords, conv.weight, conv.bias, True)
            if out is not None:
                return out
        x = self.tensor()
        c = cfg(conv)
        if c.corr == "on_demand" and c.conv1x1 == "hip" and x.is_cuda and _is_plain1x1(conv) and _frozen_conv(conv):
            return ops.get().bias_relu(ops.get().conv1x1(x, conv.weight, None), conv.bias)
        return _conv_relu(conv, x)


class BasicMotionEncoder(nn.Module):
    def __init__(self, corr_levels=4, corr_radius=4):
        super().__init__()
        cor_planes = corr_levels * (2 * corr_radius + 1) ** 2
        self.convc1 = nn.Conv2d(cor_planes, 256, 1, padding=0)
        self.convc2 = nn.Conv2d(256, 192, 3, padding=1)
        self.convf1 = nn.Conv2d(2, 128, 7, padding=3)
        self.convf2 = nn.Conv2d(128, 64, 3, padding=1)
        self.conv = nn.Conv2d(64 + 192, 128 - 2, 3, padding=1)

    RELU_CHANNELS = 128 - 2

    def can_defer_relu(self, flow):
        return (flow.shape[0] == 1 and _all_frozen(self)
                and all(_is_plain3x3(c) for c in (self.convc2, self.convf2, self.conv)))

    def forward(self, flow, corr, defer_relu=False):
        cor1 = corr.conv_relu(self.convc1) if isinstance(corr, LookupRef) else _conv_relu(self.convc1, corr)
        if self.can_defer_relu(flow):
            o = ops.get()
            flo1 = _conv_relu(self.convf1, flow)
            cf = o.conv3x3_cat([(cor1, self.convc2.weight, self.convc2.bias), (flo1, self.convf2.weight, self.convf2.bias)],
                               grad_premasked=defer_relu)
            return o.conv3x3_cat([(cf, self.conv.weight, self.conv.bias)], (flow,), grad_premasked=defer_relu,
                                 mask_input_grads=defer_relu)
        if defer_relu:
            raise RuntimeError("BasicMotionEncoder: defer_relu needs the in-place path (check can_defer_relu first)")
        cor = _conv_relu(self.convc2, cor1)
        flo = _conv_relu(self.convf2, _conv_relu(self.convf1, flow))
        out = _conv_relu(self.conv, torch.cat([cor, flo], dim=1))
        return torch.cat([out, flow], dim=1)


def _mask_head():
    return nn.Sequential(nn.Conv2d(128, 256, 3, padding=1), nn.ReLU(inplace=True), nn.Conv2d(256, 64 * 9, 1, padding=0))


def mask_logits(head, net, cache):
    c0, c2 = head[0], head[2]
    if not (_frozen_conv(c0) and _frozen_conv(c2) and _is_plain3x3(c0)):
        return .25 * head(net)
    key = (c2.weight.data_ptr(), c2.weight._version, c2.bias.data_ptr(), c2.bias._version)
    if cache.get("key") != key:
        with torch.no_grad():
            cache["key"], cache["w"], cache["b"] = key, (.25 * c2.weight).contiguous(), (.25 * c2.bias).contiguous()
    y = _conv_relu(c0, net)
    if cfg(head).conv1x1 == "hip" and y.is_cuda and _is_plain1x1(c2):
        return ops.get().conv1x1(y, cache["w"], cache["b"])
    return c2._conv_forward(y, cache["w"], cache["b"])


class BasicUpdateBlock(nn.Module):
    def __init__(self, corr_levels=4, corr_radius=4, hidden_dim=128):
        super().__init__()
        self.encoder = BasicMotionEncoder(corr_levels, corr_radius)
        self.gru = SepConvGRU(hidden_dim=hidden_dim, input_dim=128 + hidden_dim)
        self.flow_head = FlowHead(hidden_dim, hidden_dim=256)
        self.mask = _mask_head()
        self._mask_cache = {}

    def forward(self, net, inp, corr, flow, want_mask=True, gru_ctx=None):
        defer = cfg(self).defer_relu and gru_ctx is not None and self.encoder.can_defer_relu(flow)
        motion_features = self.encoder(flow, corr, defer_relu=defer)
        if gru_ctx is not None:
            net = self.gru.step(net, gru_ctx, motion_features, self.encoder.RELU_CHANNELS if defer else 0)
        else:
            net = self.gru(net, torch.cat([inp, motion_features], dim=1))
        delta_flow = self.flow_head(net)
        mask = mask_logits(self.mask, net, self._mask_cache) if want_mask else None
        return net, mask, delta_flow


def _f32(x):
    return x if x.dtype == torch.float64 else x.float()


def coords_grid(batch, ht, wd, device, dtype=torch.float32):
    ys, xs = torch.meshgrid(torch.arange(ht, device=device), torch.arange(wd, device=device), indexing="ij")
    return torch.stack([xs, ys], dim=0).to(dtype)[None].repeat(batch, 1, 1, 1)


def convex_upsample(flow, mask):
    return ops.get().convex_upsample(flow, mask)


class RAFT(nn.Module):
    def __init__(self, args=None):
        super().__init__()
        self.args = dict(args or {})
        if self.args.get("small", False):
            raise NotImplementedError("RAFT-small is not part of the PCFA configurations (raft_config.json: small=false)")
        self.hidden_dim = hdim = 128
        self.context_dim = cdim = 128
        self.args["corr_levels"] = 4
        self.args["corr_radius"] = 4
        self.args.setdefault("dropout", 0)
        self.fnet = BasicEncoder(output_dim=256, norm_fn='instance', dropout=self.args["dropout"])
        self.cnet = BasicEncoder(output_dim=hdim + cdim, norm_fn='batch', dropout=self.args["dropout"])
        self.update_block = BasicUpdateBlock(4, 4, hidden_dim=hdim)

    def freeze_bn(self):
        for m in self.modules():
            if isinstance(m, nn.BatchNorm2d):
                m.eval()

    def forward(self, image1, image2, iters=12, flow_init=None, upsample=True, test_mode=False):
        images12, image1 = ops.get().pm1_pair(image1, image2)
        hdim, cdim = self.hidden_dim, self.context_dim

        side = None
        if cfg(self).overlap_encoders and image1.is_cuda and hasattr(ops.get(), "side_stream"):
            main = torch.cuda.current_stream()
            side = ops.get().side_stream(image1.device)
            side.wait_stream(main)
            with torch.cuda.stream(side):
                cnet_out = self.cnet(image1)
        fmap1, fmap2 = self.fnet(images12, split=image1.shape[0])
        if cfg(self).corr == "on_demand":
            corr_fn = ops.get().OnDemandCorrBlock(_f32(fmap1), _f32(fmap2), num_levels=self.args["corr_levels"],
                                                  radius=self.args["corr_radius"])
        else:
            corr_fn = ops.get().CorrBlock(_f32(fmap1), _f32(fmap2), num_levels=self.args["corr_levels"],
                                          radius=self.args["corr_radius"], bwd_windows=cfg(self).pyramid_bwd_windows)
        if side is not None:
            main.wait_stream(side)
        else:
            cnet_out = self.cnet(image1)

        net, inp = torch.split(cnet_out, [hdim, cdim], dim=1)
        net, inp = torch.tanh(net), torch.relu(inp)

        N, _, H, W = image1.shape
        coords0 = coords_grid(N, H // 8, W // 8, image1.device, _f32(image1).dtype)
        coords1 = coords_grid(N, H // 8, W // 8, image1.device, _f32(image1).dtype)
        if flow_init is not None:
            coords1 = coords1 + flow_init

        gru = self.update_block.gru
        gru_ctx = gru.per_iteration(gru.precompute(inp), iters) if gru.frozen() else None
        flow_predictions = []
        flow_up = None
        flow_cur = coords1 - coords0
        for itr in range(iters):
            coords1 = coords1.detach()
            corr = LookupRef(corr_fn, coords1)
            flow = flow_cur.detach()
            need_up = (not test_mode) or itr == iters - 1
            net, up_mask, delta_flow = self.update_block(net, inp, corr, flow, want_mask=need_up,
                                                         gru_ctx=None if gru_ctx is None else gru_ctx[itr])
            coords1, flow_cur = ops.get().flow_step(coords1, delta_flow, coords0)
            if need_up:
                flow_up = convex_upsample(flow_cur, up_mask)
                flow_predictions.append(flow_up)
        if test_mode:
            return flow_cur, flow_up
        return flow_predictions
```

pcfa_amd/ops/conv.py:

```python
import ctypes
import os

import torch

from .. import _hip
from . import core
from .core import _call, _dev, _ptr, _ptr_off, cached_pack, current_lane


FEWIN_SHAPES = {(2, 7), (1, 7), (2, 5), (2, 3)}
_FEWIN_PACKED = os.environ.get("PCFA_FEWIN_PACKED", "1") != "0"


def _pack_cin_n_k(w, pack, packed_floats):
    N, Cin, k, _ = w.shape
    w = w.contiguous()
    packed = torch.empty(int(getattr(_hip.load(), packed_floats)(Cin, N, k)), device=w.device, dtype=torch.float32)
    _call(pack, _ptr(w), _ptr(packed), Cin, N, k)
    return packed


def _fewin_packed(weight):
    return cached_pack("fewin", (weight,),
                       lambda w: _pack_cin_n_k(w, "pcfa_conv_fewin_pack", "pcfa_conv_fewin_packed_floats"))


class _Conv1x1(torch.autograd.Function):

    @staticmethod
    def forward(ctx, x, w, b):
        _dev(x, w)
        if w.dim() != 4 or tuple(w.shape[2:]) != (1, 1) or x.dim() != 4 or x.shape[1] != w.shape[1]:
            raise ValueError("conv1x1: weight %s does not fit input %s" % (tuple(w.shape), tuple(x.shape)))
        if x.dtype != torch.float32 or w.dtype != torch.float32:
            raise ValueError("conv1x1: float32 only")
        x = x.contiguous()
        B, K, H, W = x.shape
        N, hw = w.shape[0], H * W
        w2 = w.reshape(N, K).contiguous()
        out = torch.empty((B, N, H, W), device=x.device, dtype=torch.float32)
        _call("pcfa_gemm_f32", _ptr(w2), _ptr(x), _ptr(out), N, hw, K, K, hw, hw, 0, 1, B, 0, K * hw, N * hw, 1.0, 1,
              _ptr(None), ctypes.c_size_t(0))
        if b is not None:
            out.add_(b.view(1, N, 1, 1))
        ctx.save_for_backward(w2)
        ctx.dims = (B, K, N, H, W)
        return out

    @staticmethod
    @torch.autograd.function.once_differentiable
    def backward(ctx, g):
        if ctx.needs_input_grad[1] or ctx.needs_input_grad[2]:
            raise RuntimeError("conv1x1 is the frozen-weight path: no weight / bias gradient")
        (w2,) = ctx.saved_tensors
        B, K, N, H, W = ctx.dims
        hw = H * W
        g = g.contiguous()
        gx = torch.empty((B, K, H, W), device=g.device, dtype=torch.float32)
        _call("pcfa_gemm_f32", _ptr(w2), _ptr(g), _ptr(gx), K, hw, N, K, hw, hw, 1, 1, B, 0, N * hw, K * hw, 1.0, 1,
              _ptr(None), ctypes.c_size_t(0))
        return gx, None, None


def conv1x1(x, weight, bias=None):
    return _Conv1x1.apply(x, weight, bias)


def conv_fewin(x, weight, bias=None, relu=False):
    _dev(x, weight, bias)
    if x.requires_grad or weight.requires_grad or (bias is not None and bias.requires_grad):
        raise RuntimeError("conv_fewin is forward-only: input and parameters must not require gradients")
    N, Cin, kh, kw = weight.shape
    if kh != kw or (Cin, kh) not in FEWIN_SHAPES or x.shape[1] != Cin:
        raise ValueError("conv_fewin: unsupported weight %s for input %s" % (tuple(weight.shape), tuple(x.shape)))
    x = x.contiguous()
    B, _, H, W = x.shape
    out = torch.empty((B, N, H, W), device=x.device, dtype=torch.float32)
    if _FEWIN_PACKED:
        _call("pcfa_conv_fewin_packed_fwd", _ptr(x), _ptr(_fewin_packed(weight)), _ptr(bias), _ptr(out), B, Cin, N, H, W,
              kh, int(bool(relu)))
    else:
        _call("pcfa_conv_fewin_fwd", _ptr(x), _ptr(weight.contiguous()), _ptr(bias), _ptr(out), B, Cin, N, H, W, kh,
              int(bool(relu)))
    return out


def _s2_packed(weight):
    return cached_pack("s2", (weight,), lambda w: _pack_cin_n_k(w, "pcfa_conv_s2_pack", "pcfa_conv_s2_packed_floats"))


def _s2_bwd_packed(weight):
    return cached_pack("s2_bwd", (weight,),
                       lambda w: _pack_cin_n_k(w, "pcfa_conv_s2_bwd_pack", "pcfa_conv_s2_bwd_packed_floats"))


def conv_s2_supported(x, weight):
    N, Cin, kh, kw = weight.shape
    return bool(x.dim() == 4 and kh == kw and x.shape[1] == Cin and not weight.requires_grad and x.is_cuda
                and _hip.load().pcfa_conv_s2_supported(Cin, N, kh, x.shape[2], x.shape[3]))


def _act_bwd(out, g, act, slope=0.):
    if not act:
        return g
    gm = torch.empty_like(g)
    if act == 1:
        _call("pcfa_relu_bwd", _ptr(out), _ptr(g), _ptr(gm), g.numel())
    else:
        _call("pcfa_leaky_relu_bwd", _ptr(out), _ptr(g), _ptr(gm), float(slope), g.numel())
    return gm


class _ConvS2(torch.autograd.Function):
    @staticmethod
    def forward(ctx, x, weight, bias, act, slope, grad_premasked=False, own_bwd=True):
        _dev(x, weight, bias)
        ctx.grad_premasked = bool(grad_premasked)
        ctx.own_bwd = bool(own_bwd)
        x = x.contiguous()
        B, Cin, H, W = x.shape
        N, _, k, _ = weight.shape
        Ho, Wo = (H + 2 * (k // 2) - k) // 2 + 1, (W + 2 * (k // 2) - k) // 2 + 1
        out = torch.empty((B, N, Ho, Wo), device=x.device, dtype=torch.float32)
        _call("pcfa_conv_s2_fwd", _ptr(x), _ptr(_s2_packed(weight)), _ptr(bias), _ptr(out), B, Cin, N, H, W, k, act,
              float(slope))
        ctx.act, ctx.slope, ctx.xshape = act, float(slope), tuple(x.shape)
        ctx.save_for_backward(weight, out if (act and not ctx.grad_premasked) else None)
        return out

    @staticmethod
    def backward(ctx, g):
        weight, out = ctx.saved_tensors
        g = g.contiguous()
        if not ctx.grad_premasked:
            g = _act_bwd(out, g, ctx.act, ctx.slope)
        N, Cin, k, _ = weight.shape
        B, _, H, W = ctx.xshape
        if ctx.own_bwd and _hip.load().pcfa_conv_s2_bwd_supported(Cin, N, k, H, W):
            gx = torch.empty(ctx.xshape, device=g.device, dtype=torch.float32)
            _call("pcfa_conv_s2_bwd", _ptr(g), _ptr(_s2_bwd_packed(weight)), _ptr(gx), B, Cin, N, H, W, k)
        else:
            gx = torch.nn.grad.conv2d_input(ctx.xshape, weight, g, stride=2, padding=k // 2)
        return gx, None, None, None, None, None, None


def _s2_ds_packed(weight, weight_d):
    def make(w, wd):
        lib = _hip.load()
        N, Cin, _, _ = w.shape
        w, wd = w.contiguous(), wd.contiguous()
        pf = torch.empty(int(lib.pcfa_conv_s2_ds_packed_floats(Cin, N)), device=w.device, dtype=torch.float32)
        pb = torch.empty(int(lib.pcfa_conv_s2_ds_bwd_packed_floats(Cin, N)), device=w.device, dtype=torch.float32)
        _call("pcfa_conv_s2_ds_pack", _ptr(w), _ptr(wd), _ptr(pf), Cin, N)
        _call("pcfa_conv_s2_ds_bwd_pack", _ptr(w), _ptr(wd), _ptr(pb), Cin, N)
        return pf, pb
    return cached_pack("s2_ds", (weight, weight_d), make)


def conv_s2_ds_supported(x, weight, weight_d):
    N, Cin, kh, kw = weight.shape
    if not (x.dim() == 4 and x.is_cuda and (kh, kw) == (3, 3) and tuple(weight_d.shape) == (N, Cin, 1, 1)
            and x.shape[1] == Cin and not weight.requires_grad and not weight_d.requires_grad):
        return False
    lib = _hip.load()
    return bool(lib.pcfa_conv_s2_supported(Cin, N, 3, x.shape[2], x.shape[3])
                and lib.pcfa_conv_s2_bwd_supported(Cin, N, 3, x.shape[2], x.shape[3]))


class _ConvS2DS(torch.autograd.Function):
    @staticmethod
    def forward(ctx, x, weight, weight_d, bias, bias_d, act):
        _dev(x, weight, weight_d, bias, bias_d)
        x = x.contiguous()
        B, Cin, H, W = x.shape
        N = weight.shape[0]
        Ho, Wo = (H - 1) // 2 + 1, (W - 1) // 2 + 1
        out = torch.empty((B, N, Ho, Wo), device=x.device, dtype=torch.float32)
        out_d = torch.empty_like(out)
        pf, pb = _s2_ds_packed(weight, weight_d)
        _call("pcfa_conv_s2_ds_fwd", _ptr(x), _ptr(pf), _ptr(bias), _ptr(out), _ptr(bias_d), _ptr(out_d), B, Cin, N, H, W,
              act, 0.0)
        ctx.act, ctx.xshape, ctx.packed_bwd = act, tuple(x.shape), pb
        ctx.save_for_backward(out if act else None)
        return out, out_d

    @staticmethod
    def backward(ctx, g, gd):
        (out,) = ctx.saved_tensors
        B, Cin, H, W = ctx.xshape
        g = g.contiguous()
        gd = gd.contiguous()
        g = _act_bwd(out, g, ctx.act)
        gx = torch.empty(ctx.xshape, device=g.device, dtype=torch.float32)
        _call("pcfa_conv_s2_ds_bwd", _ptr(g), _ptr(gd), _ptr(ctx.packed_bwd), _ptr(gx), B, Cin, g.shape[1], H, W)
        return gx, None, None, None, None, None


def conv_s2_ds(x, weight, weight_d, bias=None, bias_d=None, relu=False):
    _dev(x, weight, weight_d, bias, bias_d)
    if not conv_s2_ds_supported(x, weight, weight_d):
        raise ValueError("conv_s2_ds: unsupported weights %s / %s for input %s"
                         % (tuple(weight.shape), tuple(weight_d.shape), tuple(x.shape)))
    if any(b is not None and b.requires_grad for b in (bias, bias_d)):
        raise RuntimeError("conv_s2_ds: frozen parameters only")
    return _ConvS2DS.apply(x, weight, weight_d, bias, bias_d, int(bool(relu)))


def conv_s2(x, weight, bias=None, relu=False, leaky_slope=None, grad_premasked=False, own_bwd=True):
    _dev(x, weight, bias)
    if weight.requires_grad or (bias is not None and bias.requires_grad):
        raise RuntimeError("conv_s2: frozen parameters only")
    if not conv_s2_supported(x, weight):
        raise ValueError("conv_s2: unsupported weight %s for input %s" % (tuple(weight.shape), tuple(x.shape)))
    act = 2 if leaky_slope is not None else int(bool(relu))
    if grad_premasked and not act:
        raise ValueError("conv_s2: grad_premasked needs an activation")
    return _ConvS2.apply(x, weight, bias, act, 0.0 if leaky_slope is None else leaky_slope, bool(grad_premasked),
                         bool(own_bwd))


class _Conv3x3FewOut(torch.autograd.Function):
    @staticmethod
    def forward(ctx, x, weight, bias, skip=False):
        _dev(x, weight, bias)
        ctx.set_materialize_grads(False)
        if weight.dim() != 4 or tuple(weight.shape[2:]) != (3, 3) or not 1 <= weight.shape[0] <= 4:
            raise ValueError("conv3x3_fewout expects a [N<=4, K, 3, 3] weight, got %s" % (tuple(weight.shape),))
        x = x.contiguous()
        B, K, H, W = x.shape
        N = weight.shape[0]
        if weight.shape[1] != K:
            raise ValueError("conv3x3_fewout: input %s does not match weight %s" % (tuple(x.shape), tuple(weight.shape)))
        w = weight.detach().contiguous()
        out = torch.empty((B, N, H, W), device=x.device, dtype=torch.float32)
        nws = int(_hip.load().pcfa_conv3x3_fewout_workspace_bytes(B, K, N, H, W))
        ws = torch.empty(nws // 4, device=x.device, dtype=torch.float32) if nws else None
        _call("pcfa_conv3x3_fewout_fwd", _ptr(x), _ptr(w), _ptr(bias), _ptr(out), _ptr(ws), B, K, N, H, W)
        ctx.save_for_backward(w)
        ctx.dims = (B, K, N, H, W)
        if skip:
            return out, x.view_as(x)
        return out

    @staticmethod
    @torch.autograd.function.once_differentiable
    def backward(ctx, g, g_skip=None):
        if ctx.needs_input_grad[1] or ctx.needs_input_grad[2]:
            raise RuntimeError("conv3x3_fewout is the frozen-weight path: no weight / bias gradient")
        if g is None:
            return g_skip, None, None, None
        (w,) = ctx.saved_tensors
        B, K, N, H, W = ctx.dims
        g = g.contiguous()
        gx = torch.empty((B, K, H, W), device=g.device, dtype=torch.float32)
        _call("pcfa_conv3x3_fewout_bwd", _ptr(g), _ptr(w), _ptr(None if g_skip is None else g_skip.contiguous()), _ptr(gx),
              B, K, N, H, W)
        return gx, None, None, None


def conv3x3_fewout(x, weight, bias=None, skip=False):
    return _Conv3x3FewOut.apply(x, weight, bias, skip)


class _InstNormRelu(torch.autograd.Function):

    @staticmethod
    def forward(ctx, x, eps, relu):
        _dev(x)
        x = x.contiguous()
        B, C, H, W = x.shape
        planes, plane = B * C, H * W
        lib = _hip.load()
        ws = torch.empty((int(lib.pcfa_instnorm_workspace_bytes(planes, plane)) + 3) // 4, device=x.device,
                         dtype=torch.float32)
        y = torch.empty_like(x)
        stats = torch.empty((planes, 2), device=x.device, dtype=torch.float32)
        _call("pcfa_instnorm_fwd", _ptr(x), _ptr(y), _ptr(stats), _ptr(ws), planes, plane, float(eps), int(bool(relu)))
        ctx.save_for_backward(x, stats)
        ctx.dims = (planes, plane, int(bool(relu)))
        return y

    @staticmethod
    @torch.autograd.function.once_differentiable
    def backward(ctx, g):
        x, stats = ctx.saved_tensors
        planes, plane, relu = ctx.dims
        g = g.contiguous()
        lib = _hip.load()
        ws = torch.empty((int(lib.pcfa_instnorm_workspace_bytes(planes, plane)) + 3) // 4, device=x.device,
                         dtype=torch.float32)
        gx = torch.empty_like(x)
        _call("pcfa_instnorm_bwd", _ptr(x), _ptr(stats), _ptr(g), _ptr(gx), _ptr(ws), planes, plane, relu)
        return gx, None, None


def instance_norm_relu(x, eps=1e-5, relu=False):
    return _InstNormRelu.apply(x, eps, relu)


class _AddRelu(torch.autograd.Function):
    @staticmethod
    def forward(ctx, a, b, b_is_relu):
        _dev(a, b)
        if a.shape != b.shape:
            raise ValueError("add_relu: shapes differ: %s vs %s" % (tuple(a.shape), tuple(b.shape)))
        a, b = a.contiguous(), b.contiguous()
        out = torch.empty_like(a)
        _call("pcfa_add_relu_fwd", _ptr(a), _ptr(b), _ptr(out), a.numel())
        ctx.b_is_relu = bool(b_is_relu)
        ctx.save_for_backward(out, *((b,) if ctx.b_is_relu else ()))
        return out

    @staticmethod
    @torch.autograd.function.once_differentiable
    def backward(ctx, g):
        out = ctx.saved_tensors[0]
        g = g.contiguous()
        gm = torch.empty_like(g)
        if ctx.b_is_relu:
            gb = torch.empty_like(g)
            _call("pcfa_relu_bwd2", _ptr(out), _ptr(ctx.saved_tensors[1]), _ptr(g), _ptr(gm), _ptr(gb), g.numel())
            return gm, gb, None
        _call("pcfa_relu_bwd", _ptr(out), _ptr(g), _ptr(gm), g.numel())
        return gm, gm, None


def add_relu(a, b, b_is_relu=False):
    return _AddRelu.apply(a, b, b_is_relu)


def _sepconv5_packed(weight):
    def make(w):
        cout, cin = w.shape[:2]
        w = w.contiguous()
        lib = _hip.load()
        fwd = torch.empty(int(lib.pcfa_sepconv5_packed_floats(cout, cin)), device=w.device, dtype=torch.float32)
        bwd = torch.empty(int(lib.pcfa_sepconv5_packed_floats(cin, cout)), device=w.device, dtype=torch.float32)
        _call("pcfa_sepconv5_pack_weights", _ptr(w), _ptr(fwd), _ptr(bwd), cout, cin)
        return fwd, bwd
    return cached_pack("sepconv5", (weight,), make)


class _SepConv5(torch.autograd.Function):
    @staticmethod
    def forward(ctx, a, b, weight):
        _dev(a, b, weight)
        if weight.dim() != 4 or tuple(weight.shape[2:]) not in ((1, 5), (5, 1)) or weight.dtype != torch.float32:
            raise ValueError("sepconv5 expects a float32 (1,5) or (5,1) Conv2d weight, got %s" % (tuple(weight.shape),))
        vertical = int(weight.shape[2] == 5)
        a = a.contiguous()
        b = None if b is None else b.contiguous()
        B, Ca, H, W = a.shape
        Cb = 0 if b is None else b.shape[1]
        cout = weight.shape[0]
        if weight.shape[1] != Ca + Cb or (b is not None and (b.shape[0], b.shape[2], b.shape[3]) != (B, H, W)):
            raise ValueError("sepconv5: operands %s / %s do not match weight %s"
                             % (tuple(a.shape), None if b is None else tuple(b.shape), tuple(weight.shape)))
        fwd, bwd = _sepconv5_packed(weight)
        out = torch.empty((B, cout, H, W), device=a.device, dtype=torch.float32)
        _call("pcfa_sepconv5_fwd", _ptr(a), Ca, _ptr(b), Cb, _ptr(fwd), _ptr(out), B, cout, H, W, vertical)
        ctx.bwd, ctx.dims = bwd, (B, Ca, Cb, cout, H, W, vertical)
        return out

    @staticmethod
    def backward(ctx, grad_out):
        if ctx.needs_input_grad[2]:
            raise RuntimeError("sepconv5 is the frozen-weight path: no weight gradient (use the module's "
                               "reference forward when training)")
        B, Ca, Cb, cout, H, W, vertical = ctx.dims
        g = grad_out.contiguous()
        gin = torch.empty((B, Ca + Cb, H, W), device=g.device, dtype=torch.float32)
        _call("pcfa_sepconv5_fwd", _ptr(g), cout, None, 0, _ptr(ctx.bwd), _ptr(gin), B, Ca + Cb, H, W, vertical)
        return gin[:, :Ca], (gin[:, Ca:] if Cb else None), None


def _conv3x3_packed(weight):
    def make(w):
        cout, cin = w.shape[:2]
        lib = _hip.load()
        w = w.contiguous()
        fwd = torch.empty(int(lib.pcfa_conv3x3_packed_floats(cin, cout)), device=w.device, dtype=torch.float32)
        bwd = torch.empty(int(lib.pcfa_conv3x3_packed_floats(cout, cin)), device=w.device, dtype=torch.float32)
        _call("pcfa_conv3x3_pack_weights", _ptr(w), _ptr(fwd), _ptr(bwd), cout, cin)
        return fwd, bwd
    return cached_pack("conv3x3", (weight,), make)


_CONV_WS = {}
_CONV_WS_RETIRED = []


_SIDE_STREAMS = {}
_SIDE_HANDLES = set()


def side_stream(device):
    idx = device.index if device.index is not None else torch.cuda.current_device()
    k = current_lane()
    s = _SIDE_STREAMS.get((idx, k))
    if s is None:
        s = _SIDE_STREAMS[(idx, k)] = core.own_stream(device, k)
        _SIDE_HANDLES.add(s.cuda_stream)
    return s


def _conv_workspace(device, nbytes):
    dev_idx = device.index if device.index is not None else torch.cuda.current_device()
    idx = (dev_idx, torch.cuda.current_stream(device).cuda_stream in _SIDE_HANDLES, current_lane())
    ws = _CONV_WS.get(idx)
    if ws is None or ws.numel() * 4 < nbytes:
        if torch.cuda.is_current_stream_capturing():
            raise RuntimeError("conv3x3 workspace would have to grow inside a graph capture (no eager warm-up of this "
                               "shape ran before it)")
        if ws is not None:
            _CONV_WS_RETIRED.append(ws)
        ws = torch.empty((nbytes + 3) // 4, device=device, dtype=torch.float32)
        _CONV_WS[idx] = ws
    return ws


def _conv3x3_run(device, x_ptr, packed, bias_ptr, mask_ptr, addend_ptr, out_ptr, B, K, N, H, W, act=0, slope=0.,
                 mask_channels=0):
    nws = int(_hip.load().pcfa_conv3x3_workspace_bytes(B, K, N, H, W))
    ws = _conv_workspace(device, nws) if nws else None
    _call("pcfa_conv3x3_run", x_ptr, _ptr(packed), bias_ptr, mask_ptr, addend_ptr, out_ptr, B, K, N, H, W, int(act),
          float(slope), int(mask_channels), _ptr(ws), nws)


class _Conv3x3(torch.autograd.Function):
    @staticmethod
    def forward(ctx, x, weight, bias, relu, slope=None, skip=False, flags=0, input_slope=0.):
        _dev(x, weight, bias)
        ctx.skip = bool(skip)
        ctx.grad_premasked, ctx.mask_input_grad = bool(flags & 1), bool(flags & 2)
        ctx.input_slope = float(input_slope)
        ctx.set_materialize_grads(False)
        if weight.dim() != 4 or tuple(weight.shape[2:]) != (3, 3) or weight.dtype != torch.float32:
            raise ValueError("conv3x3 expects a float32 3x3 Conv2d weight, got %s" % (tuple(weight.shape),))
        x = x.contiguous()
        B, K, H, W = x.shape
        N = weight.shape[0]
        if weight.shape[1] != K:
            raise ValueError("conv3x3: input %s does not match weight %s" % (tuple(x.shape), tuple(weight.shape)))
        fwd, bwd = _conv3x3_packed(weight)
        out = torch.empty((B, N, H, W), device=x.device, dtype=torch.float32)
        act = 2 if slope is not None else int(bool(relu))
        _conv3x3_run(x.device, _ptr(x), fwd, _ptr(bias), None, None, _ptr(out), B, K, N, H, W, act, float(slope or 0.))
        ctx.bwd, ctx.dims, ctx.act, ctx.slope = bwd, (B, K, N, H, W), act, float(slope or 0.)
        if ctx.grad_premasked and not act:
            raise ValueError("conv3x3: grad_premasked needs an activation (relu=True or leaky_slope)")
        ctx.save_for_backward(*(([out] if act and not ctx.grad_premasked else []) + ([x] if ctx.mask_input_grad else [])))
        if ctx.skip:
            return out, x.view_as(x)
        return out

    @staticmethod
    def backward(ctx, g, g_skip=None):
        if ctx.needs_input_grad[1] or ctx.needs_input_grad[2]:
            raise RuntimeError("conv3x3 is the frozen-weight path: no weight / bias gradient")
        B, K, N, H, W = ctx.dims
        if g is None:
            return (None if g_skip is None else g_skip), None, None, None, None, None, None, None
        g = g.contiguous()
        if ctx.act and not ctx.grad_premasked:
            g = _act_bwd(ctx.saved_tensors[0], g, ctx.act, ctx.slope)
        gin = torch.empty((B, K, H, W), device=g.device, dtype=torch.float32)
        if g_skip is not None or ctx.mask_input_grad:
            xin = ctx.saved_tensors[-1] if ctx.mask_input_grad else None
            _conv3x3_run(g.device, _ptr(g), ctx.bwd, None, _ptr(xin),
                         _ptr(None if g_skip is None else g_skip.contiguous()), _ptr(gin), B, N, K, H, W,
                         slope=ctx.input_slope if ctx.mask_input_grad else 0.)
        else:
            _conv3x3_run(g.device, _ptr(g), ctx.bwd, None, None, None, _ptr(gin), B, N, K, H, W)
        return gin, None, None, None, None, None, None, None


_PAIR_LAUNCH = os.environ.get("PCFA_CONV3X3_PAIR", "1") != "0"


class _Conv3x3Cat(torch.autograd.Function):

    @staticmethod
    def forward(ctx, n_conv, flags, *args):
        xs, ws, bs = args[0:3 * n_conv:3], args[1:3 * n_conv:3], args[2:3 * n_conv:3]
        tails = args[3 * n_conv:]
        ctx.grad_premasked, ctx.mask_input_grads = bool(flags & 1), bool(flags & 2)
        _dev(*xs, *ws, *tails)
        xs = [x.contiguous() for x in xs]
        B, _, H, W = xs[0].shape
        if B != 1:
            raise ValueError("conv3x3_cat: batch size 1 only")
        plane = H * W
        widths = [w.shape[0] for w in ws] + [t.shape[1] for t in tails]
        buf = torch.empty((1, sum(widths), H, W), device=xs[0].device, dtype=torch.float32)
        off, packs, fwds, offs = 0, [], [], []
        for x, w, b in zip(xs, ws, bs):
            if tuple(x.shape) != (1, w.shape[1], H, W) or tuple(w.shape[2:]) != (3, 3):
                raise ValueError("conv3x3_cat: input %s does not fit weight %s" % (tuple(x.shape), tuple(w.shape)))
            fwd, bwd = _conv3x3_packed(w)
            fwds.append(fwd)
            offs.append(off)
            packs.append((bwd, w.shape[1], w.shape[0], off))
            off += w.shape[0]
        lib = _hip.load()
        f23 = all(lib.pcfa_conv3x3_algo(1, w.shape[1], w.shape[0], H, W) == 23 for w in ws)
        if n_conv == 2 and (ws[0].shape[1] % 8 == 0) == (ws[1].shape[1] % 8 == 0) and _PAIR_LAUNCH and f23:
            i, j = (0, 1) if ws[0].shape[0] * ws[0].shape[1] >= ws[1].shape[0] * ws[1].shape[1] else (1, 0)
            _call("pcfa_conv3x3_act_fwd_pair", _ptr(xs[i]), _ptr(fwds[i]), _ptr(bs[i]), _ptr_off(buf, offs[i] * plane),
                  ws[i].shape[1], ws[i].shape[0], _ptr(xs[j]), _ptr(fwds[j]), _ptr(bs[j]),
                  _ptr_off(buf, offs[j] * plane), ws[j].shape[1], ws[j].shape[0], H, W, 1, 0.)
        else:
            for x, w, b, fwd, o_ in zip(xs, ws, bs, fwds, offs):
                _conv3x3_run(x.device, _ptr(x), fwd, _ptr(b), None, None, _ptr_off(buf, o_ * plane), 1, w.shape[1],
                             w.shape[0], H, W, 1, 0.)
        for t in tails:
            buf[:, off:off + t.shape[1]].copy_(t)
            off += t.shape[1]
        ctx.packs, ctx.dims, ctx.n_conv, ctx.tail_widths = packs, (H, W), n_conv, [t.shape[1] for t in tails]
        ctx.save_for_backward(buf, *(xs if ctx.mask_input_grads else ()))
        return buf

    @staticmethod
    def backward(ctx, g):
        buf = ctx.saved_tensors[0]
        H, W = ctx.dims
        plane = H * W
        g = g.contiguous()
        grads = [None, None]
        for i, (bwd, k, n, off) in enumerate(ctx.packs):
            if ctx.needs_input_grad[3 + 3 * i] or ctx.needs_input_grad[4 + 3 * i]:
                raise RuntimeError("conv3x3_cat is the frozen-weight path: no weight / bias gradient")
            gx = None
            if ctx.needs_input_grad[2 + 3 * i]:
                if ctx.grad_premasked:
                    gm = g[:, off:off + n]
                else:
                    gm = torch.empty((1, n, H, W), device=g.device, dtype=torch.float32)
                    _call("pcfa_relu_bwd", _ptr_off(buf, off * plane), _ptr_off(g, off * plane), _ptr(gm), n * plane)
                gx = torch.empty((1, k, H, W), device=g.device, dtype=torch.float32)
                if ctx.mask_input_grads:
                    _conv3x3_run(g.device, _ptr(gm), bwd, None, _ptr(ctx.saved_tensors[1 + i]), None, _ptr(gx), 1, n, k,
                                 H, W)
                else:
                    _conv3x3_run(g.device, _ptr(gm), bwd, None, None, None, _ptr(gx), 1, n, k, H, W)
            grads += [gx, None, None]
        off = sum(p[2] for p in ctx.packs)
        for j, tw in enumerate(ctx.tail_widths):
            grads.append(g[:, off:off + tw] if ctx.needs_input_grad[2 + 3 * ctx.n_conv + j] else None)
            off += tw
        return tuple(grads)


def conv3x3_cat(convs, tails=(), grad_premasked=False, mask_input_grads=False):
    flat = []
    for x, w, b in convs:
        flat += [x, w, b]
    return _Conv3x3Cat.apply(len(convs), int(bool(grad_premasked)) | 2 * int(bool(mask_input_grads)), *flat, *tails)


class _DenseBlock(torch.autograd.Function):

    @staticmethod
    def forward(ctx, slope, fused_masks, nparts, *rest):
        parts, wb = rest[:nparts], rest[nparts:]
        weights, biases = wb[0::2], wb[1::2]
        ctx.fused_masks = bool(fused_masks)
        _dev(*parts, *weights)
        x0 = parts[0]
        B, _, H, W = x0.shape
        if B != 1:
            raise ValueError("dense_block: batch size 1 only")
        if any(p.shape[0] != 1 or tuple(p.shape[2:]) != (H, W) or p.dtype != torch.float32 for p in parts):
            raise ValueError("dense_block: input parts %s do not share batch 1 / size / fp32" % ([tuple(p.shape) for p in parts],))
        ctx.part_widths = [p.shape[1] for p in parts]
        K0 = sum(ctx.part_widths)
        widths = [w.shape[0] for w in weights]
        total = K0 + sum(widths)
        buf = torch.empty((1, total, H, W), device=x0.device, dtype=torch.float32)
        plane = H * W
        start = total - K0
        if nparts == 1:
            buf[:, start:].copy_(x0)
        else:
            torch.cat(parts, 1, out=buf[:, start:])
        packs = []
        k = K0
        for w, b, n in zip(weights, biases, widths):
            if tuple(w.shape[1:]) != (k, 3, 3):
                raise ValueError("dense_block: weight %s does not fit %d input channels" % (tuple(w.shape), k))
            fwd, bwd = _conv3x3_packed(w)
            _conv3x3_run(x0.device, _ptr_off(buf, start * plane), fwd, _ptr(b), None, None,
                         _ptr_off(buf, (start - n) * plane), 1, k, n, H, W, 2, float(slope))
            packs.append((bwd, k, n, start))
            start -= n
            k += n
        ctx.packs, ctx.dims, ctx.slope = packs, (total, K0, H, W), float(slope)
        ctx.save_for_backward(buf)
        return buf

    @staticmethod
    def backward(ctx, g):
        if any(ctx.needs_input_grad[3 + len(ctx.part_widths):]):
            raise RuntimeError("dense_block is the frozen-weight path: no weight / bias gradient")
        (buf,) = ctx.saved_tensors
        total, K0, H, W = ctx.dims
        plane = H * W
        g = g.contiguous()
        gb = torch.empty_like(g)
        npk = len(ctx.packs)
        for i in range(npk - 1, -1, -1):
            bwd, k, n, start = ctx.packs[i]
            if i == npk - 1 or not ctx.fused_masks:
                gm = torch.empty((1, n, H, W), device=g.device, dtype=torch.float32)
                _call("pcfa_leaky_relu_bwd", _ptr_off(buf, (start - n) * plane),
                      _ptr_off(g if i == npk - 1 else gb, (start - n) * plane), _ptr(gm), ctx.slope, n * plane)
                gm_ptr = _ptr(gm)
            else:
                gm_ptr = _ptr_off(gb, (start - n) * plane)
            dst = _ptr_off(gb, start * plane)
            src = _ptr_off(g, start * plane) if i == npk - 1 else dst
            if i > 0 and ctx.fused_masks:
                _conv3x3_run(g.device, gm_ptr, bwd, None, _ptr_off(buf, start * plane), src, dst, 1, n, k, H, W,
                             slope=ctx.slope, mask_channels=ctx.packs[i - 1][2])
            else:
                _conv3x3_run(g.device, gm_ptr, bwd, None, None, src, dst, 1, n, k, H, W)
        grads, c0 = [], total - K0
        for wdt, need in zip(ctx.part_widths, ctx.needs_input_grad[3:]):
            grads.append(gb[:, c0:c0 + wdt] if need else None)
            c0 += wdt
        return (None, None, None) + tuple(grads) + (None,) * (2 * len(ctx.packs))


def dense_block(x, layers, slope=0.1, fused_masks=True):
    flat = []
    for w, b in layers:
        flat += [w, b]
    parts = tuple(x) if isinstance(x, (tuple, list)) else (x,)
    return _DenseBlock.apply(slope, fused_masks, len(parts), *[p.contiguous() for p in parts], *flat)


def conv3x3(x, weight, bias=None, relu=False, leaky_slope=None, skip=False, grad_premasked=False, mask_input_grad=False,
            input_slope=0.):
    return _Conv3x3.apply(x, weight, bias, relu, leaky_slope, skip,
                          int(bool(grad_premasked)) | 2 * int(bool(mask_input_grad)), float(input_slope))
```

pcfa_amd/ops/core.py:

```python
import contextlib
import ctypes
import threading
import weakref

import torch

from .. import _hip

_lane_state = threading.local()
_STREAM_LANE = {}


def current_lane():
    if _STREAM_LANE and torch.cuda.is_available():
        k = _STREAM_LANE.get(torch.cuda.current_stream().cuda_stream)
        if k is not None:
            return k
    return getattr(_lane_state, "k", 0)


@contextlib.contextmanager
def lane(k):
    prev = getattr(_lane_state, "k", 0)
    _lane_state.k = int(k)
    try:
        yield
    finally:
        _lane_state.k = prev


def bind_stream(stream, k=None):
    k = getattr(_lane_state, "k", 0) if k is None else int(k)
    if k != 0:
        _STREAM_LANE[stream.cuda_stream] = k
    else:
        _STREAM_LANE.pop(stream.cuda_stream, None)
    return stream


_hiprt = None
_FREE_STREAMS = {}


def _hip_runtime():
    global _hiprt
    if _hiprt is None:
        rt = ctypes.CDLL("libamdhip64.so")
        rt.hipStreamCreateWithFlags.argtypes = [ctypes.POINTER(ctypes.c_void_p), ctypes.c_uint]
        rt.hipStreamCreateWithFlags.restype = ctypes.c_int
        _hiprt = rt
    return _hiprt


def release_stream(stream):
    try:
        handle = stream.cuda_stream
        idx = stream.device.index
    except Exception:
        return
    if handle in _OWN_HANDLES.get(idx, ()) and handle not in _FREE_STREAMS.setdefault(idx, []):
        _STREAM_LANE.pop(handle, None)
        _FREE_STREAMS[idx].append(handle)


_OWN_HANDLES = {}


def own_stream(device, k=None):
    dev = torch.device(device)
    idx = dev.index if dev.index is not None else torch.cuda.current_device()
    _run_pool(idx)
    free = _FREE_STREAMS.setdefault(idx, [])
    if free:
        handle = free.pop()
    else:
        h = ctypes.c_void_p()
        with torch.cuda.device(idx):
            err = _hip_runtime().hipStreamCreateWithFlags(ctypes.byref(h), 1)
        if err != 0 or not h.value:
            raise RuntimeError("hipStreamCreateWithFlags failed: %d" % err)
        handle = h.value
        _OWN_HANDLES.setdefault(idx, set()).add(handle)
    return bind_stream(torch.cuda.ExternalStream(handle, device=torch.device("cuda", idx)), k)


_LANE_RUN_STREAMS = {}


def _run_pool(idx):
    pool = _LANE_RUN_STREAMS.get(idx)
    if pool is None:
        pool, seen = [], set()
        for _ in range(64):
            s = torch.cuda.Stream(torch.device("cuda", idx))
            if s.cuda_stream not in seen:
                seen.add(s.cuda_stream)
                pool.append(s)
        lib = _hip.load()
        for s in pool[:8]:
            _hip.check(lib.pcfa_null_launch(ctypes.c_void_p(s.cuda_stream)), "pcfa_null_launch")
        _LANE_RUN_STREAMS[idx] = pool
    return pool


def lane_run_streams(device, n):
    dev = torch.device(device)
    idx = dev.index if dev.index is not None else torch.cuda.current_device()
    pool = _run_pool(idx)
    if n > len(pool):
        raise ValueError("%d pairs in flight: at most %d lanes per device" % (n, len(pool)))
    return [bind_stream(pool[k], k) for k in range(n)]


def new_stream(device):
    return own_stream(device)


def _stream():
    return ctypes.c_void_p(torch.cuda.current_stream().cuda_stream)


def _dev(*tensors):
    for t in tensors:
        if t is None:
            continue
        if not t.is_cuda:
            raise RuntimeError(
                "pcfa_amd HIP operator called with a %s tensor: the MI355X path has no CPU fallback"
                % t.device)
        if t.dtype != torch.float32:
            raise TypeError("pcfa_amd kernels compute in float32, got %s" % t.dtype)


def _ptr(t):
    return ctypes.c_void_p(0 if t is None else t.data_ptr())


def _ptr_off(t, offset_floats):
    return ctypes.c_void_p(0 if t is None else t.data_ptr() + 4 * offset_floats)


def scratch_for(size_fn, dims, device):
    nbytes = int(getattr(_hip.load(), size_fn)(*dims))
    return torch.empty((nbytes + 7) // 8, device=device, dtype=torch.int64), nbytes


def _pair(v):
    return (v, v) if isinstance(v, int) else tuple(v)


_profiler = None
_dispatch_timer = None


def set_launch_profiler(profiler):
    global _profiler
    _profiler = profiler


def set_dispatch_timer(timer):
    global _dispatch_timer
    _dispatch_timer = timer


_work = None


def set_work_recorder(rec):
    global _work
    _work = rec


def _note_work(family, direct, issued):
    e = _work.setdefault(family, [0.0, 0.0, 0])
    e[0] += direct
    e[1] += issued
    e[2] += 1


def _conv3x3_work(B, K, N, H, W):
    direct = 2.0 * 9 * K * N * B * H * W
    if _hip.load().pcfa_conv3x3_algo(B, K, N, H, W) == 43:
        _note_work("conv3x3_f43", direct, direct / 4.0)
    else:
        _note_work("conv3x3_winograd", direct, direct / 2.25)


def _sepconv5_work(B, Ca, Cb, Cout, H, W, vertical):
    direct = 2.0 * 5 * (Ca + Cb) * Cout * B * H * W
    if _hip.load().pcfa_sepconv5_uses_winograd(B, Ca, Cb, Cout, H, W, int(vertical)):
        _note_work("sepconv5_winograd", direct, direct * 0.6)
    else:
        _note_work("sepconv5_direct", direct, direct)


_WORK_TABLE = {
    "pcfa_conv3x3_run": lambda a: _conv3x3_work(a[6], a[7], a[8], a[9], a[10]),
    "pcfa_conv3x3_act_fwd_pair": lambda a: (_conv3x3_work(1, a[4], a[5], a[12], a[13]),
                                            _conv3x3_work(1, a[10], a[11], a[12], a[13])),
    "pcfa_sepconv5_fwd": lambda a: _sepconv5_work(a[6], a[1], a[3], a[7], a[8], a[9], a[10]),
    "pcfa_sepconv5_fwd_split": lambda a: _sepconv5_work(a[10], a[1], a[3], a[11], a[12], a[13], a[14]),
    "pcfa_sepconv5_fwd_split_masked": lambda a: _sepconv5_work(a[12], a[1], a[3], a[13], a[14], a[15], a[16]),
    "pcfa_sepconv5_gru_gates_fwd": lambda a: _sepconv5_work(a[9], a[1], a[3], 2 * a[1], a[10], a[11], a[12]),
    "pcfa_sepconv5_gru_update_fwd": lambda a: _sepconv5_work(a[10], a[1], a[3], a[1], a[11], a[12], a[13]),
    "pcfa_sepconv5_gru_gates_bwd": lambda a: _sepconv5_work(a[13], a[1], 0, a[1] + a[2], a[14], a[15], a[16]),
    "pcfa_sepconv5_gru_update_bwd": lambda a: _sepconv5_work(a[12], 2 * a[1], 0, a[1] + a[2], a[13], a[14], a[15]),
    "pcfa_instnorm_fwd": lambda a: _note_work("instnorm_fwd", 2.0 * a[4] * a[5] * 4, 0.0),
    "pcfa_instnorm_bwd": lambda a: _note_work("instnorm_bwd", 3.0 * a[5] * a[6] * 4, 0.0),
    "pcfa_conv3x3_fewout_fwd": lambda a: _note_work("conv3x3_fewout_fwd", 4.0 * a[5] * (a[6] + a[7]) * a[8] * a[9], 0.0),
    "pcfa_conv3x3_fewout_bwd": lambda a: _note_work("conv3x3_fewout_bwd", 4.0 * a[4] * (a[5] + a[6]) * a[7] * a[8], 0.0),
    "pcfa_relu_bwd": lambda a: _note_work("relu_bwd", 12.0 * a[3], 0.0),
    "pcfa_relu_bwd2": lambda a: _note_work("relu_bwd2", 20.0 * a[5], 0.0),
    "pcfa_add_relu_fwd": lambda a: _note_work("add_relu_fwd", 12.0 * a[3], 0.0),
    "pcfa_conv_fewin_packed_fwd": lambda a: _note_work("conv_fewin_fwd", *(2 * [2.0 * a[5] * a[9] * a[9] * a[6] * a[4] * a[7] * a[8]])),
}


_spy = None


def set_call_spy(spy):
    global _spy
    _spy = spy


def _call(name, *args):
    if _spy is not None:
        return _spy(name, args, _invoke)
    return _invoke(name, *args)


def _invoke(name, *args):
    fn = getattr(_hip.load(), name)
    if _work is not None and name in _WORK_TABLE:
        _WORK_TABLE[name](args)
    prof = _profiler
    timer = _dispatch_timer
    if timer is not None and name in timer.plan:
        lib = _hip.load()
        for label, nth in timer.plan[name]:
            e0, e1 = timer.new_pair(label)
            _hip.check(lib.pcfa_timing_arm(e0, e1, nth), "pcfa_timing_arm")
        try:
            status = fn(*args, _stream())
        finally:
            lib.pcfa_timing_arm(None, None, -1)
    elif prof is not None and prof.wants(name):
        s, e = torch.cuda.Event(enable_timing=True), torch.cuda.Event(enable_timing=True)
        s.record()
        status = fn(*args, _stream())
        e.record()
        prof.events.setdefault(name, []).append((s, e))
    else:
        status = fn(*args, _stream())
    _hip.check(status, name)


_packs = {}


def cached_pack(kind, weights, make):
    key = (kind,) + tuple(id(w) for w in weights)
    ver = tuple(w._version for w in weights)
    hit = _packs.get(key)
    if hit is None or hit[1] != ver or any(r() is not w for r, w in zip(hit[0], weights)):
        drop = lambda _r, k=key: _packs.pop(k, None)
        hit = (tuple(weakref.ref(w, drop) for w in weights), ver, make(*(w.detach() for w in weights)))
        _packs[key] = hit
    return hit[2]


def work_recorder():
    return _work
```

pcfa_amd/ops/corr.py:

```python
import ctypes
import os

import torch

from .. import _hip
from . import core
from .core import _call, _dev, _note_work, _pair, _ptr, _ptr_off, _stream, cached_pack


class _CorrState:
    __slots__ = ("B", "D", "H", "W", "L", "r", "slab", "pyr", "f2ext", "dpyr", "token_grad", "coords_bwd", "bwd_windows")


class _CorrBuild(torch.autograd.Function):

    @staticmethod
    def forward(ctx, fmap1, fmap2, state):
        lib = _hip.load()
        B, D, H, W = fmap1.shape
        f1 = fmap1.contiguous()
        f2 = fmap2.contiguous()
        slab = state.slab
        state.f2ext = torch.empty((B, D, slab), device=f1.device, dtype=torch.float32)
        state.pyr = torch.empty((B * H * W, slab), device=f1.device, dtype=torch.float32)
        _call("pcfa_corr_f2ext_fwd", _ptr(f2), _ptr(state.f2ext), B, D, H, W, state.L)
        _call("pcfa_corr_pyramid_fwd", _ptr(f1), _ptr(state.f2ext), _ptr(state.pyr), B, D, H, W,
                                             state.L)
        ctx.state = state
        ctx.save_for_backward(f1)
        return torch.zeros(1, device=f1.device, dtype=torch.float32)

    @staticmethod
    def backward(ctx, grad_token):
        st = ctx.state
        (f1,) = ctx.saved_tensors
        if st.dpyr is None:
            z = torch.zeros_like(f1)
            st.token_grad = None
            return z, z.clone(), None
        lib = _hip.load()
        B, D, H, W = st.B, st.D, st.H, st.W
        df1 = torch.empty_like(f1)
        df2 = torch.empty_like(f1)
        cs = st.coords_bwd if (st.coords_bwd and len(st.coords_bwd) <= 32 and st.bwd_windows and st.L <= 4) else []
        if cs:
            nbytes = lib.pcfa_corr_pyramid_bwd_windows_workspace_bytes(B, D, H, W, st.L)
            ws = torch.empty((nbytes + 3) // 4, device=f1.device, dtype=torch.float32)
            ptrs = (ctypes.c_void_p * len(cs))(*[c.data_ptr() for c in cs])
            _call("pcfa_corr_pyramid_bwd_windows", _ptr(st.dpyr), _ptr(f1), _ptr(st.f2ext), _ptr(df1), _ptr(df2), _ptr(ws),
                  ctypes.c_size_t(nbytes), ptrs, len(cs), st.r, B, D, H, W, st.L)
            if core.work_recorder() is not None:
                base = (int(lib.pcfa_corr_pyramid_bwd_workspace_bytes(B, D, H, W, st.L)) + 15) & ~15
                nbA, nbB = -(-(H * W) // 128), -(-st.slab // 128)
                seg = ws.view(torch.int32)[base // 4: base // 4 + 10 * B * (nbA + nbB)].cpu().view(-1, 10).long()
                live = torch.arange(4)[None, :] < seg[:, :1]
                k = ((seg[:, 2:9:2] - seg[:, 1:8:2]) * live).sum(1)
                dense = 2.0 * B * D * (H * W) ** 2
                _note_work("corr_pyramid_gemm_dfmap1", dense, 2.0 * D * 128 * float(k[:B * nbA].sum()))
                _note_work("corr_pyramid_gemm_df2ext", dense, 2.0 * D * 128 * float(k[B * nbA:].sum()))
        else:
            nbytes = lib.pcfa_corr_pyramid_bwd_workspace_bytes(B, D, H, W, st.L)
            ws = torch.empty((nbytes + 3) // 4, device=f1.device, dtype=torch.float32)
            _call("pcfa_corr_pyramid_bwd", _ptr(st.dpyr), _ptr(f1), _ptr(st.f2ext), _ptr(df1), _ptr(df2), _ptr(ws),
                  ctypes.c_size_t(nbytes), B, D, H, W, st.L)
        st.dpyr = None
        st.token_grad = None
        st.coords_bwd = None
        return df1, df2, None


def _token_grad(st, device):
    if st.token_grad is None:
        st.token_grad = torch.zeros(1, device=device, dtype=torch.float32)
        return st.token_grad
    return None


class _CorrLookup(torch.autograd.Function):
    @staticmethod
    def forward(ctx, token, coords, state):
        if coords.requires_grad and torch.is_grad_enabled():
            raise RuntimeError("CorrBlock lookup: coords.requires_grad is not supported (detach the coordinates, as "
                               "models/raft/raft.py:122-123 does)")
        lib = _hip.load()
        st = state
        c = coords.contiguous()
        n1 = 2 * st.r + 1
        out = torch.empty((st.B, st.L * n1 * n1, st.H, st.W), device=c.device, dtype=torch.float32)
        _call("pcfa_corr_lookup_fwd", _ptr(st.pyr), _ptr(c), _ptr(out), st.B, st.H, st.W, st.L, st.r)
        ctx.state = st
        ctx.save_for_backward(c)
        return out

    @staticmethod
    def backward(ctx, grad_out):
        st = ctx.state
        (c,) = ctx.saved_tensors
        lib = _hip.load()
        if st.dpyr is None:
            st.dpyr = torch.zeros_like(st.pyr)
            st.coords_bwd = []
        st.coords_bwd.append(c)
        g = grad_out.contiguous()
        _call("pcfa_corr_lookup_bwd", _ptr(st.dpyr), _ptr(c), _ptr(g), st.B, st.H, st.W, st.L, st.r)
        return _token_grad(st, g.device), None, None


def _convc1_packed(weight):
    def make(w):
        cout = w.shape[0]
        w = w.reshape(cout, -1).contiguous()
        packed = torch.empty(int(_hip.load().pcfa_lookup_convc1_packed_floats(cout)), device=w.device, dtype=torch.float32)
        _call("pcfa_lookup_convc1_pack_weights", _ptr(w), _ptr(packed), cout, w.shape[1])
        return packed
    return cached_pack("convc1", (weight,), make)


class _CorrLookupConv(torch.autograd.Function):

    @staticmethod
    def forward(ctx, token, coords, state, weight, bias, relu):
        if coords.requires_grad and torch.is_grad_enabled():
            raise RuntimeError("CorrBlock lookup: coords.requires_grad is not supported (detach the coordinates, as "
                               "models/raft/raft.py:122-123 does)")
        st = state
        c = coords.contiguous()
        packed = _convc1_packed(weight)
        out = torch.empty((st.B, weight.shape[0], st.H, st.W), device=c.device, dtype=torch.float32)
        _call("pcfa_lookup_convc1_fwd", _ptr(st.pyr), _ptr(c), _ptr(packed), _ptr(bias), _ptr(out), st.B, st.H, st.W,
              st.L, st.r, weight.shape[0], int(relu))
        ctx.state, ctx.packed, ctx.relu, ctx.cout = st, packed, int(relu), weight.shape[0]
        ctx.save_for_backward(c, out)
        return out

    @staticmethod
    def backward(ctx, grad_out):
        if ctx.needs_input_grad[3] or ctx.needs_input_grad[4]:
            raise RuntimeError("lookup_conv is the frozen-weight path: no weight / bias gradient")
        st = ctx.state
        c, out = ctx.saved_tensors
        if st.dpyr is None:
            st.dpyr = torch.zeros_like(st.pyr)
            st.coords_bwd = []
        st.coords_bwd.append(c)
        g = grad_out.contiguous()
        _call("pcfa_lookup_convc1_bwd", _ptr(st.dpyr), _ptr(c), _ptr(ctx.packed), _ptr(out), _ptr(g), st.B, st.H, st.W,
              st.L, st.r, ctx.cout, ctx.relu)
        return _token_grad(st, g.device), None, None, None, None, None


class CorrBlock:

    def __init__(self, fmap1, fmap2, num_levels=4, radius=4, bwd_windows=True):
        _dev(fmap1, fmap2)
        if fmap1.shape != fmap2.shape or fmap1.dim() != 4:
            raise ValueError("CorrBlock expects two [B,D,H,W] feature maps of equal shape")
        lib = _hip.load()
        self.num_levels = num_levels
        self.radius = radius
        st = _CorrState()
        st.B, st.D, st.H, st.W = fmap1.shape
        st.L, st.r = num_levels, radius
        st.slab = lib.pcfa_corr_slab_floats(st.H, st.W, num_levels)
        if st.slab <= 0 or (st.H >> (num_levels - 1)) < 1 or (st.W >> (num_levels - 1)) < 1:
            raise ValueError("feature map %dx%d too small for %d pyramid levels" % (st.H, st.W, num_levels))
        st.dpyr = None
        st.token_grad = None
        st.coords_bwd = None
        st.bwd_windows = bool(bwd_windows)
        self._state = st
        self._token = _CorrBuild.apply(fmap1, fmap2, st)

    def __call__(self, coords):
        _dev(coords)
        return _CorrLookup.apply(self._token, coords, self._state)

    def lookup_conv_relu(self, coords, weight, bias, relu=True):
        if (self.num_levels != 4 or self.radius != 4 or bias is None or weight.dim() != 4
                or tuple(weight.shape) != (256, 324, 1, 1) or weight.requires_grad or bias.requires_grad):
            return None
        _dev(coords, weight, bias)
        return _CorrLookupConv.apply(self._token, coords, self._state, weight, bias, relu)

    @property
    def corr_pyramid(self):
        st = self._state
        return [st.pyr[:, idx.to(st.pyr.device)].reshape(-1, 1, h, w)
                for (idx, h, w) in tiled_index_maps(st.H, st.W, st.L)]


class _OnDemandState:
    __slots__ = ("B", "D", "H", "W", "L", "r", "ws", "token_grad", "accumulating")


class _OnDemandBuild(torch.autograd.Function):

    @staticmethod
    def forward(ctx, fmap1, fmap2, state):
        lib = _hip.load()
        st = state
        f1 = fmap1.contiguous()
        f2 = fmap2.contiguous()
        nbytes = int(lib.pcfa_corr_ondemand_workspace_bytes(st.B, st.D, st.H, st.W, st.L))
        st.ws = torch.empty(nbytes, device=f1.device, dtype=torch.uint8)
        _call("pcfa_corr_ondemand_prepare", _ptr(f1), _ptr(f2), _ptr(st.ws), st.B, st.D, st.H, st.W, st.L)
        ctx.state = st
        ctx.shape = f1.shape
        return torch.zeros(1, device=f1.device, dtype=torch.float32)

    @staticmethod
    def backward(ctx, grad_token):
        st = ctx.state
        if not st.accumulating:
            z = torch.zeros(ctx.shape, device=st.ws.device, dtype=torch.float32)
            st.token_grad = None
            return z, z.clone(), None
        df1 = torch.empty(ctx.shape, device=st.ws.device, dtype=torch.float32)
        df2 = torch.empty_like(df1)
        _call("pcfa_corr_ondemand_finish", _ptr(st.ws), _ptr(df1), _ptr(df2), st.B, st.D, st.H, st.W, st.L)
        st.accumulating = False
        st.token_grad = None
        return df1, df2, None


class _OnDemandLookup(torch.autograd.Function):
    @staticmethod
    def forward(ctx, token, coords, state):
        st = state
        c = coords.contiguous()
        n1 = 2 * st.r + 1
        out = torch.empty((st.B, st.L * n1 * n1, st.H, st.W), device=c.device, dtype=torch.float32)
        _call("pcfa_corr_ondemand_fwd", _ptr(st.ws), _ptr(c), _ptr(out), st.B, st.D, st.H, st.W, st.L, st.r)
        ctx.state = st
        ctx.save_for_backward(c)
        return out

    @staticmethod
    def backward(ctx, grad_out):
        st = ctx.state
        (c,) = ctx.saved_tensors
        g = grad_out.contiguous()
        _call("pcfa_corr_ondemand_bwd", _ptr(st.ws), _ptr(c), _ptr(g), int(st.accumulating), st.B, st.D, st.H, st.W,
              st.L, st.r)
        st.accumulating = True
        return _token_grad(st, g.device), None, None


class OnDemandCorrBlock:

    def __init__(self, fmap1, fmap2, num_levels=4, radius=4):
        _dev(fmap1, fmap2)
        if fmap1.shape != fmap2.shape or fmap1.dim() != 4:
            raise ValueError("OnDemandCorrBlock expects two [B,D,H,W] feature maps of equal shape")
        lib = _hip.load()
        self.num_levels = num_levels
        self.radius = radius
        st = _OnDemandState()
        st.B, st.D, st.H, st.W = fmap1.shape
        st.L, st.r = num_levels, radius
        if (st.H >> (num_levels - 1)) < 1 or (st.W >> (num_levels - 1)) < 1:
            raise ValueError("feature map %dx%d too small for %d pyramid levels" % (st.H, st.W, num_levels))
        if lib.pcfa_corr_ondemand_workspace_bytes(st.B, st.D, st.H, st.W, num_levels) == 0 or not 1 <= radius <= 4:
            raise ValueError("OnDemandCorrBlock: D=%d, %d levels, radius %d not served (D %% 4 == 0, D <= 512, radius 1..4)"
                             % (st.D, num_levels, radius))
        st.token_grad = None
        st.accumulating = False
        self._state = st
        self._token = _OnDemandBuild.apply(fmap1, fmap2, st)

    def __call__(self, coords):
        _dev(coords)
        if coords.requires_grad and torch.is_grad_enabled():
            raise RuntimeError("OnDemandCorrBlock lookup: coords.requires_grad is not supported (detach the coordinates, "
                               "as models/raft/raft.py:122-123 does)")
        return _OnDemandLookup.apply(self._token, coords, self._state)

    def lookup_conv_relu(self, coords, weight, bias, relu=True):
        return None


def tiled_index_maps(H, W, num_levels):
    out, off, h, w = [], 0, H, W
    for _ in range(num_levels):
        tw = (w + 3) // 4
        ys, xs = torch.meshgrid(torch.arange(h), torch.arange(w), indexing="ij")
        idx = off + ((ys // 4) * tw + xs // 4) * 16 + (ys % 4) * 4 + xs % 4
        out.append((idx.reshape(-1), h, w))
        off += ((h + 3) // 4) * tw * 16
        h, w = h // 2, w // 2
    return out
```

pcfa_amd/ops/gru.py:

```python
import ctypes
import os
import weakref

import torch

from .. import _hip
from . import core
from .core import _call, _dev, _note_work, _pair, _ptr, _ptr_off, _stream
from .conv import _sepconv5_packed, _SepConv5


def _plane_channels(t):
    return t.shape[-2] * t.shape[-1], t.shape[-3]


class _GruGates(torch.autograd.Function):
    @staticmethod
    def forward(ctx, zc, rc, h, bias_z, bias_r, add_z, add_r):
        _dev(zc, rc, h, bias_z, bias_r, add_z, add_r)
        zc, rc, h = zc.contiguous(), rc.contiguous(), h.contiguous()
        az = None if add_z is None else add_z.contiguous()
        ar = None if add_r is None else add_r.contiguous()
        z, r, rh = torch.empty_like(zc), torch.empty_like(zc), torch.empty_like(zc)
        plane, C = _plane_channels(zc)
        _call("pcfa_gru_gates_fwd", _ptr(zc), _ptr(rc), _ptr(h), _ptr(bias_z), _ptr(bias_r), _ptr(az), _ptr(ar),
              _ptr(z), _ptr(r), _ptr(rh), zc.numel(), plane, C)
        ctx.save_for_backward(z, r, h)
        ctx.has_add = (add_z is not None, add_r is not None)
        return z, rh

    @staticmethod
    def backward(ctx, dz, drh):
        z, r, h = ctx.saved_tensors
        dz = torch.zeros_like(z) if dz is None else dz.contiguous()
        drh = torch.zeros_like(z) if drh is None else drh.contiguous()
        dzc, drc, dh = torch.empty_like(z), torch.empty_like(z), torch.empty_like(z)
        _call("pcfa_gru_gates_bwd", _ptr(z), _ptr(r), _ptr(h), _ptr(dz), _ptr(drh), _ptr(dzc), _ptr(drc), _ptr(dh),
              z.numel())
        return dzc, drc, dh, None, None, (dzc if ctx.has_add[0] else None), (drc if ctx.has_add[1] else None)


class _GruGatesPacked(torch.autograd.Function):

    @staticmethod
    def forward(ctx, zr, h, bias_zr, add_zr):
        _dev(zr, h, bias_zr, add_zr)
        zr, h = zr.contiguous(), h.contiguous()
        add = None if add_zr is None else add_zr.contiguous()
        B, C2, H, W = zr.shape
        C, plane = C2 // 2, H * W
        z, r, rh = torch.empty_like(h), torch.empty_like(h), torch.empty_like(h)
        bz = None if bias_zr is None else bias_zr[:C]
        br = None if bias_zr is None else bias_zr[C:]
        n = C * plane
        for b in range(B):
            o, oz = b * n, b * 2 * n
            _call("pcfa_gru_gates_fwd", _ptr_off(zr, oz), _ptr_off(zr, oz + n), _ptr_off(h, o), _ptr(bz), _ptr(br),
                  _ptr_off(add, oz), _ptr_off(add, oz + n), _ptr_off(z, o), _ptr_off(r, o), _ptr_off(rh, o), n,
                  plane, C)
        ctx.save_for_backward(z, r, h)
        ctx.has_add = add_zr is not None
        return z, rh

    @staticmethod
    def backward(ctx, dz, drh):
        z, r, h = ctx.saved_tensors
        B, C, H, W = z.shape
        n = C * H * W
        dz = torch.zeros_like(z) if dz is None else dz.contiguous()
        drh = torch.zeros_like(z) if drh is None else drh.contiguous()
        dzr = torch.empty((B, 2 * C, H, W), device=z.device, dtype=torch.float32)
        dh = torch.empty_like(z)
        for b in range(B):
            o, oz = b * n, b * 2 * n
            _call("pcfa_gru_gates_bwd", _ptr_off(z, o), _ptr_off(r, o), _ptr_off(h, o), _ptr_off(dz, o),
                  _ptr_off(drh, o), _ptr_off(dzr, oz), _ptr_off(dzr, oz + n), _ptr_off(dh, o), n)
        return dzr, dh, None, (dzr if ctx.has_add else None)


class _GruUpdate(torch.autograd.Function):
    @staticmethod
    def forward(ctx, z, qc, h, bias_q, add_q):
        _dev(z, qc, h, bias_q, add_q)
        z, qc, h = z.contiguous(), qc.contiguous(), h.contiguous()
        aq = None if add_q is None else add_q.contiguous()
        q, hnew = torch.empty_like(z), torch.empty_like(z)
        plane, C = _plane_channels(z)
        _call("pcfa_gru_update_fwd", _ptr(z), _ptr(qc), _ptr(h), _ptr(bias_q), _ptr(aq), _ptr(q), _ptr(hnew),
              z.numel(), plane, C)
        ctx.save_for_backward(z, q, h)
        ctx.has_add = add_q is not None
        return hnew

    @staticmethod
    def backward(ctx, g):
        z, q, h = ctx.saved_tensors
        g = g.contiguous()
        dz, dqc, dh = torch.empty_like(z), torch.empty_like(z), torch.empty_like(z)
        _call("pcfa_gru_update_bwd", _ptr(z), _ptr(q), _ptr(h), _ptr(g), _ptr(dz), _ptr(dqc), _ptr(dh), z.numel())
        return dz, dqc, dh, None, (dqc if ctx.has_add else None)


class _BiasRelu(torch.autograd.Function):
    @staticmethod
    def forward(ctx, x, bias):
        _dev(x, bias)
        x = x.contiguous()
        out = torch.empty_like(x)
        plane, C = _plane_channels(x)
        _call("pcfa_bias_relu_fwd", _ptr(x), _ptr(bias), _ptr(out), x.numel(), plane, C)
        ctx.save_for_backward(out)
        return out

    @staticmethod
    def backward(ctx, g):
        (out,) = ctx.saved_tensors
        g = g.contiguous()
        gx = torch.empty_like(out)
        _call("pcfa_relu_bwd", _ptr(out), _ptr(g), _ptr(gx), out.numel())
        return gx, None


_GRU_EPILOGUES = os.environ.get("PCFA_GRU_EPILOGUES", "1") != "0"


class _GruStep(torch.autograd.Function):

    @staticmethod
    def forward(ctx, h, rest, w_zr1, p_zr1, w_q1, p_q1, w_zr2, p_zr2, w_q2, p_q2, rest_relu_channels=0):
        _dev(h, rest, w_zr1, p_zr1, w_q1, p_q1, w_zr2, p_zr2, w_q2, p_q2)
        h, rest = h.contiguous(), rest.contiguous()
        B, C, H, W = h.shape
        Cr = rest.shape[1]
        n, plane = C * H * W, H * W
        new = lambda c: torch.empty((B, c, H, W), device=h.device, dtype=torch.float32)
        saved, packs = [], []
        for w_zr, p_zr, w_q, p_q in ((w_zr1, p_zr1, w_q1, p_q1), (w_zr2, p_zr2, w_q2, p_q2)):
            if tuple(w_zr.shape[:2]) != (2 * C, C + Cr) or tuple(w_q.shape[:2]) != (C, C + Cr):
                raise ValueError("gru_step: weights %s / %s do not fit h %s, rest %s"
                                 % (tuple(w_zr.shape), tuple(w_q.shape), tuple(h.shape), tuple(rest.shape)))
            vertical = int(w_zr.shape[2] == 5)
            f_zr, b_zr = _sepconv5_packed(w_zr)
            f_q, b_q = _sepconv5_packed(w_q)
            p_zr, p_q = p_zr.contiguous(), p_q.contiguous()
            z, r, rh, q, hnew = new(C), new(C), new(C), new(C), new(C)
            if C % 32 == 0 and _GRU_EPILOGUES:
                _call("pcfa_sepconv5_gru_gates_fwd", _ptr(h), C, _ptr(rest), Cr, _ptr(f_zr), _ptr(p_zr), _ptr(z), _ptr(r),
                      _ptr(rh), B, H, W, vertical)
                _call("pcfa_sepconv5_gru_update_fwd", _ptr(rh), C, _ptr(rest), Cr, _ptr(f_q), _ptr(p_q), _ptr(z), _ptr(h),
                      _ptr(q), _ptr(hnew), B, H, W, vertical)
            else:
                zr, qc = new(2 * C), new(C)
                _call("pcfa_sepconv5_fwd", _ptr(h), C, _ptr(rest), Cr, _ptr(f_zr), _ptr(zr), B, 2 * C, H, W, vertical)
                for b in range(B):
                    o, oz = b * n, b * 2 * n
                    _call("pcfa_gru_gates_fwd", _ptr_off(zr, oz), _ptr_off(zr, oz + n), _ptr_off(h, o), None, None,
                          _ptr_off(p_zr, oz), _ptr_off(p_zr, oz + n), _ptr_off(z, o), _ptr_off(r, o), _ptr_off(rh, o),
                          n, plane, C)
                _call("pcfa_sepconv5_fwd", _ptr(rh), C, _ptr(rest), Cr, _ptr(f_q), _ptr(qc), B, C, H, W, vertical)
                _call("pcfa_gru_update_fwd", _ptr(z), _ptr(qc), _ptr(h), None, _ptr(p_q), _ptr(q), _ptr(hnew),
                      z.numel(), plane, C)
            saved += [z, r, q, h]
            packs.append((b_zr, b_q, vertical))
            h = hnew
        ctx.rest_relu = int(rest_relu_channels)
        if not 0 <= ctx.rest_relu <= Cr:
            raise ValueError("gru_step: rest_relu_channels %d outside [0, %d]" % (ctx.rest_relu, Cr))
        ctx.save_for_backward(*saved, *((rest,) if ctx.rest_relu else ()))
        ctx.packs, ctx.dims = packs, (B, C, Cr, H, W)
        return h

    @staticmethod
    def backward(ctx, g):
        if any(ctx.needs_input_grad[i] for i in (2, 4, 6, 8)):
            raise RuntimeError("gru_step is the frozen-weight path: no weight gradient")
        B, C, Cr, H, W = ctx.dims
        n = C * H * W
        new = lambda c: torch.empty((B, c, H, W), device=g.device, dtype=torch.float32)
        g = g.contiguous()
        d_rest = new(Cr)
        grads_p = [None, None, None, None]
        if C % 32 == 0 and _GRU_EPILOGUES:
            z1, r1, q1, h1 = ctx.saved_tensors[4:8]
            z0, r0, q0, h0 = ctx.saved_tensors[0:4]
            (b_zr1, b_q1, v1), (b_zr0, b_q0, v0) = ctx.packs[1], ctx.packs[0]
            dz1, dqc1, dh1, dzr1 = new(C), new(C), new(C), new(2 * C)
            _call("pcfa_gru_update_bwd", _ptr(z1), _ptr(q1), _ptr(h1), _ptr(g), _ptr(dz1), _ptr(dqc1), _ptr(dh1), z1.numel())
            _call("pcfa_sepconv5_gru_gates_bwd", _ptr(dqc1), C, Cr, _ptr(b_q1), _ptr(z1), _ptr(r1), _ptr(h1), _ptr(dz1),
                  _ptr(dh1), _ptr(dzr1), _ptr(dh1), _ptr(d_rest), 0, B, H, W, v1)
            dz0, dqc0, dh0, dzr0 = new(C), new(C), new(C), new(2 * C)
            _call("pcfa_sepconv5_gru_update_bwd", _ptr(dzr1), C, Cr, _ptr(b_zr1), _ptr(dh1), _ptr(z0), _ptr(q0), _ptr(h0),
                  _ptr(dz0), _ptr(dqc0), _ptr(dh0), _ptr(d_rest), B, H, W, v1)
            _call("pcfa_sepconv5_gru_gates_bwd", _ptr(dqc0), C, Cr, _ptr(b_q0), _ptr(z0), _ptr(r0), _ptr(h0), _ptr(dz0),
                  _ptr(dh0), _ptr(dzr0), _ptr(dh0), _ptr(d_rest), 1, B, H, W, v0)
            if ctx.rest_relu:
                _call("pcfa_sepconv5_fwd_split_masked", _ptr(dzr0), 2 * C, None, 0, _ptr(b_zr0), _ptr(dh0), C, 1,
                      _ptr(d_rest), 1, _ptr(ctx.saved_tensors[8]), ctx.rest_relu, B, C + Cr, H, W, v0)
            else:
                _call("pcfa_sepconv5_fwd_split", _ptr(dzr0), 2 * C, None, 0, _ptr(b_zr0), _ptr(dh0), C, 1, _ptr(d_rest), 1,
                      B, C + Cr, H, W, v0)
            return dh0, d_rest, None, dzr0, None, dqc0, None, dzr1, None, dqc1, None
        rest_started = 0
        for half in (1, 0):
            z, r, q, h = ctx.saved_tensors[4 * half: 4 * half + 4]
            b_zr, b_q, vertical = ctx.packs[half]
            dz, dqc, dh, drh, dzr = new(C), new(C), new(C), new(C), new(2 * C)
            _call("pcfa_gru_update_bwd", _ptr(z), _ptr(q), _ptr(h), _ptr(g), _ptr(dz), _ptr(dqc), _ptr(dh), z.numel())
            _call("pcfa_sepconv5_fwd_split", _ptr(dqc), C, None, 0, _ptr(b_q), _ptr(drh), C, 0, _ptr(d_rest),
                  rest_started, B, C + Cr, H, W, vertical)
            rest_started = 1
            for b in range(B):
                o, oz = b * n, b * 2 * n
                _call("pcfa_gru_gates_bwd_acc", _ptr_off(z, o), _ptr_off(r, o), _ptr_off(h, o), _ptr_off(dz, o),
                      _ptr_off(drh, o), _ptr_off(dh, o), _ptr_off(dzr, oz), _ptr_off(dzr, oz + n), _ptr_off(dh, o), n)
            if half == 0 and ctx.rest_relu:
                _call("pcfa_sepconv5_fwd_split_masked", _ptr(dzr), 2 * C, None, 0, _ptr(b_zr), _ptr(dh), C, 1,
                      _ptr(d_rest), 1, _ptr(ctx.saved_tensors[8]), ctx.rest_relu, B, C + Cr, H, W, vertical)
            else:
                _call("pcfa_sepconv5_fwd_split", _ptr(dzr), 2 * C, None, 0, _ptr(b_zr), _ptr(dh), C, 1, _ptr(d_rest), 1,
                      B, C + Cr, H, W, vertical)
            grads_p[2 * half], grads_p[2 * half + 1] = dzr, dqc
            g = dh
        return g, d_rest, None, grads_p[0], None, grads_p[1], None, grads_p[2], None, grads_p[3], None


class _Fanout(torch.autograd.Function):

    @staticmethod
    def forward(ctx, x, n):
        ctx.set_materialize_grads(False)
        return tuple(x.view_as(x) for _ in range(n))

    @staticmethod
    def backward(ctx, *grads):
        live = [g.contiguous() for g in grads if g is not None]
        if not live:
            return None, None
        if len(live) == 1:
            return live[0], None
        _dev(*live)
        out = torch.empty_like(live[0])
        for i in range(0, len(live), 15):
            part = ([out] if i else []) + live[i:i + 15]
            arr = (ctypes.c_void_p * len(part))(*[t.data_ptr() for t in part])
            _call("pcfa_sum_n", arr, len(part), _ptr(out), out.numel())
        return out, None


class _ConvexUpsample(torch.autograd.Function):
    @staticmethod
    def forward(ctx, flow, mask):
        _dev(flow, mask)
        N, C, H, W = flow.shape
        if C != 2 or tuple(mask.shape) != (N, 576, H, W):
            raise ValueError("convex_upsample: flow %s / mask %s (expected [N,2,H,W] and [N,576,H,W])"
                             % (tuple(flow.shape), tuple(mask.shape)))
        flow, mask = flow.contiguous(), mask.contiguous()
        out = torch.empty((N, 2, 8 * H, 8 * W), device=flow.device, dtype=torch.float32)
        _call("pcfa_convex_upsample_fwd", _ptr(flow), _ptr(mask), _ptr(out), N, H, W)
        ctx.save_for_backward(flow, mask)
        return out

    @staticmethod
    @torch.autograd.function.once_differentiable
    def backward(ctx, g):
        flow, mask = ctx.saved_tensors
        N, _, H, W = flow.shape
        g = g.contiguous()
        gflow, gmask = torch.empty_like(flow), torch.empty_like(mask)
        ws = torch.empty(int(_hip.load().pcfa_convex_upsample_workspace_floats(N, H, W)), device=g.device,
                         dtype=torch.float32)
        _call("pcfa_convex_upsample_bwd", _ptr(flow), _ptr(mask), _ptr(g), _ptr(gflow), _ptr(gmask), _ptr(ws), N, H, W)
        return gflow, gmask


def convex_upsample(flow, mask):
    return _ConvexUpsample.apply(flow, mask)


class _FlowStep(torch.autograd.Function):
    @staticmethod
    def forward(ctx, coords1, delta, coords0):
        _dev(coords1, delta, coords0)
        if not (coords1.shape == delta.shape == coords0.shape):
            raise ValueError("flow_step: shapes differ: %s %s %s" % (tuple(coords1.shape), tuple(delta.shape),
                                                                     tuple(coords0.shape)))
        c1, d, c0 = coords1.contiguous(), delta.contiguous(), coords0.contiguous()
        c1n, fl = torch.empty_like(c1), torch.empty_like(c1)
        _call("pcfa_flow_step", _ptr(c1), _ptr(d), _ptr(c0), _ptr(c1n), _ptr(fl), c1.numel())
        ctx.set_materialize_grads(False)
        return c1n, fl

    @staticmethod
    def backward(ctx, g1, g2):
        g = g1 if g2 is None else g2 if g1 is None else g1 + g2
        return (g if ctx.needs_input_grad[0] else None, g if ctx.needs_input_grad[1] else None,
                (None if g is None else -g) if ctx.needs_input_grad[2] else None)


def flow_step(coords1, delta, coords0):
    return _FlowStep.apply(coords1, delta, coords0)


def fanout(x, n):
    return _Fanout.apply(x, n) if n > 1 else (x,)


def gru_step(h, rest, halves, rest_relu_channels=0):
    (a, b, c, d), (e, f, g_, i_) = halves
    return _GruStep.apply(h, rest, a, b, c, d, e, f, g_, i_, int(rest_relu_channels))


def sepconv5(a, b, weight):
    return _SepConv5.apply(a, b, weight)


def gru_gates_packed(zr, h, bias_zr=None, add_zr=None):
    return _GruGatesPacked.apply(zr, h, bias_zr, add_zr)


def gru_gates(zc, rc, h, bias_z=None, bias_r=None, add_z=None, add_r=None):
    return _GruGates.apply(zc, rc, h, bias_z, bias_r, add_z, add_r)


def gru_update(z, qc, h, bias_q=None, add_q=None):
    return _GruUpdate.apply(z, qc, h, bias_q, add_q)


def bias_relu(x, bias=None):
    return _BiasRelu.apply(x, bias)
```

pcfa_amd/ops/profiling.py:

```python
import ctypes

import torch

from .. import _hip


class LaunchProfiler:

    def __init__(self, names=None):
        self.names = set(names) if names else None
        self.events = {}

    def wants(self, name):
        return self.names is None or name in self.names

    def summary(self):
        torch.cuda.synchronize()
        out = {}
        for name, pairs in self.events.items():
            tot = sum(s.elapsed_time(e) for s, e in pairs)
            out[name] = (1e3 * tot / len(pairs), len(pairs))
        return out


class DispatchTimer:

    DEFAULT_PLAN = {
        "pcfa_corr_lookup_fwd": [("corr_lookup_fwd", 0)],
        "pcfa_corr_lookup_bwd": [("corr_lookup_bwd", 0)],
        "pcfa_corr_pyramid_fwd": [("corr_pyramid_gemm_fwd", 0)],
        "pcfa_corr_pyramid_bwd": [("corr_pyramid_gemm_dfmap1", 0), ("corr_pyramid_gemm_df2ext", 2)],
        "pcfa_corr_pyramid_bwd_windows": [("corr_pyramid_gemm_dfmap1", 2), ("corr_pyramid_gemm_df2ext", 4)],
        "pcfa_corr_f2ext_fwd": [("corr_f2ext_fwd", 0)],
        "pcfa_spatial_corr_fwd": [("spatial_corr_fwd", 0)],
        "pcfa_spatial_corr_bwd": [("spatial_corr_bwd_in1", 0), ("spatial_corr_bwd_in2", 1)],
        "pcfa_flownet_corr_fwd": [("flownet_corr_fwd", 0)],
        "pcfa_flownet_corr_bwd": [("flownet_corr_bwd_in1", 0), ("flownet_corr_bwd_in2", 1)],
        "pcfa_resample2d_fwd": [("resample2d_fwd", 0)],
        "pcfa_resample2d_bwd": [("resample2d_bwd", 1)],
        "pcfa_channelnorm_fwd": [("channelnorm_fwd", 0)],
        "pcfa_channelnorm_bwd": [("channelnorm_bwd", 0)],
        "pcfa_box_transform_fwd": [("box_transform_fwd", 0)],
        "pcfa_box_transform_bwd": [("box_transform_bwd", 0)],
        "pcfa_flow_loss_fwd": [("flow_loss_partial", 0)],
        "pcfa_gru_gates_fwd": [("gru_gates_fwd", 0)],
        "pcfa_gru_gates_bwd": [("gru_gates_bwd", 0)],
        "pcfa_gru_update_fwd": [("gru_update_fwd", 0)],
        "pcfa_gru_update_bwd": [("gru_update_bwd", 0)],
        "pcfa_conv_fewin_fwd": [("conv_fewin_fwd", 0)],
        "pcfa_pwc_warp_fwd": [("pwc_warp_fwd", 0)],
        "pcfa_pwc_warp_bwd": [("pwc_warp_bwd", 1)],
        "pcfa_pwc_warp_bwd_det": [("pwc_warp_bwd", 1)],
        "pcfa_conv3x3_fewout_fwd": [("conv3x3_fewout_fwd", 0)],
        "pcfa_conv3x3_fewout_bwd": [("conv3x3_fewout_bwd", 0)],
        "pcfa_instnorm_fwd": [("instnorm_stats_fwd", 0), ("instnorm_apply_fwd", 1)],
        "pcfa_instnorm_bwd": [("instnorm_stats_bwd", 0), ("instnorm_apply_bwd", 1)],
        "pcfa_add_relu_fwd": [("add_relu_fwd", 0)],
        "pcfa_bias_relu_fwd": [("bias_relu_fwd", 0)],
        "pcfa_relu_bwd": [("relu_bwd", 0)],
    }

    EVENT_FLAGS = 0x20000000

    def __init__(self, plan=None):
        self.plan = dict(self.DEFAULT_PLAN if plan is None else plan)
        self.hip = ctypes.CDLL("libamdhip64.so")
        self.hip.hipEventCreateWithFlags.argtypes = [ctypes.POINTER(ctypes.c_void_p), ctypes.c_uint]
        self.hip.hipEventElapsedTime.argtypes = [ctypes.POINTER(ctypes.c_float), ctypes.c_void_p, ctypes.c_void_p]
        self.hip.hipEventDestroy.argtypes = [ctypes.c_void_p]
        self.pairs = {}

    def new_pair(self, name):
        e0, e1 = ctypes.c_void_p(), ctypes.c_void_p()
        for e in (e0, e1):
            err = self.hip.hipEventCreateWithFlags(ctypes.byref(e), self.EVENT_FLAGS)
            if err != 0:
                raise RuntimeError("hipEventCreateWithFlags failed: %d" % err)
        self.pairs.setdefault(name, []).append((e0, e1))
        return e0, e1

    def summary(self):
        torch.cuda.synchronize()
        out = {}
        for name, pairs in self.pairs.items():
            tot, n = 0.0, 0
            for e0, e1 in pairs:
                ms = ctypes.c_float()
                if self.hip.hipEventElapsedTime(ctypes.byref(ms), e0, e1) == 0:
                    tot += ms.value
                    n += 1
                self.hip.hipEventDestroy(e0)
                self.hip.hipEventDestroy(e1)
            if n:
                out[name] = (1e3 * tot / n, n)
        self.pairs = {}
        self.hip.hipGetLastError()
        return out
```

Measured before the change: 7.573 attack_steps/s.

## Fuse RAFT flow-head conv with coords update and write flow into next encoder buffer

Adds a fewout conv3x3 forward variant whose epilogue also computes coords1+delta and the new flow, replacing the separate flow_step launch. The flow tensor is written straight into the tail slot of the next iteration's motion-encoder concat buffer, which conv3x3_cat adopts instead of allocating a new buffer and copying the tail. Also drops a zeros fill in the corr token and a redundant coords_grid build and repeat. This removes small kernel launches and copies per GRU iteration, at the cost of more complex storage aliasing and a larger conv epilogue.

```diff
diff --git a/include/pcfa_hip.h b/include/pcfa_hip.h
--- a/include/pcfa_hip.h
+++ b/include/pcfa_hip.h
@@ -320,6 +320,9 @@
 PCFA_API size_t pcfa_conv3x3_fewout_workspace_bytes(int B, int K, int N, int H, int W);
 PCFA_API int pcfa_conv3x3_fewout_fwd(const float* x, const float* w, const float* bias, float* out, void* workspace,
                                      int B, int K, int N, int H, int W, void* stream);
+PCFA_API int pcfa_conv3x3_fewout_flow_fwd(const float* x, const float* w, const float* bias, const float* coords1_in,
+                                          const float* coords0, float* delta, float* coords1_out, float* flow,
+                                          void* workspace, int B, int K, int N, int H, int W, void* stream);
 PCFA_API int pcfa_conv3x3_fewout_bwd(const float* grad_out, const float* w, const float* addend, float* grad_x, int B,
                                      int K, int N, int H, int W, void* stream);
 
diff --git a/pcfa_amd/_hip.py b/pcfa_amd/_hip.py
--- a/pcfa_amd/_hip.py
+++ b/pcfa_amd/_hip.py
@@ -154,6 +154,7 @@
     "pcfa_pwc_warp_bwd_det": (c_int, [_P, _P, _P, _P, _P, _P, c_size_t, c_int, c_int, c_int, c_int, c_float, c_float, _P]),
     "pcfa_conv3x3_fewout_workspace_bytes": (c_size_t, [c_int, c_int, c_int, c_int, c_int]),
     "pcfa_conv3x3_fewout_fwd": (c_int, [_P, _P, _P, _P, _P, c_int, c_int, c_int, c_int, c_int, _P]),
+    "pcfa_conv3x3_fewout_flow_fwd": (c_int, [_P, _P, _P, _P, _P, _P, _P, _P, _P, c_int, c_int, c_int, c_int, c_int, _P]),
     "pcfa_conv3x3_fewout_bwd": (c_int, [_P, _P, _P, _P, c_int, c_int, c_int, c_int, c_int, _P]),
     "pcfa_deconv4s2_fewout_workspace_bytes": (c_size_t, [c_int, c_int, c_int, c_int, c_int]),
     "pcfa_deconv4s2_fewout_fwd": (c_int, [_P, _P, _P, _P, _P, c_int, c_int, c_int, c_int, c_int, _P]),
diff --git a/pcfa_amd/csrc/conv3x3_fewout.hip b/pcfa_amd/csrc/conv3x3_fewout.hip
--- a/pcfa_amd/csrc/conv3x3_fewout.hip
+++ b/pcfa_amd/csrc/conv3x3_fewout.hip
@@ -6,10 +6,36 @@
 constexpr int FO_WAVES = 8;
 constexpr int FO_FWD_WAVES = 16;
 
+struct FlowTail {
+  const float* c1;
+  const float* c0;
+  float* c1n;
+  float* fl;
+};
+
+struct FlowTailIn {
+  float c1, c0;
+};
+__device__ __forceinline__ FlowTailIn flow_tail_fetch(const FlowTail& ft, bool live, size_t i) {
+  FlowTailIn t = {0.f, 0.f};
+  if (ft.c1 != nullptr && live) {
+    t.c1 = ft.c1[i];
+    t.c0 = ft.c0[i];
+  }
+  return t;
+}
+__device__ __forceinline__ void flow_tail_store(const FlowTail& ft, const FlowTailIn& t, size_t i, float delta) {
+  if (ft.c1 != nullptr) {
+    const float v = t.c1 + delta;
+    ft.c1n[i] = v;
+    ft.fl[i] = v - t.c0;
+  }
+}
+
 template <int N>
 __global__ __launch_bounds__(FO_PX* FO_FWD_WAVES) void conv3x3_fewout_fwd_kernel(
     const float* __restrict__ x, const float* __restrict__ w, const float* __restrict__ bias,
-    float* __restrict__ out, int K, int H, int W, int splits, int kper) {
+    float* __restrict__ out, int K, int H, int W, int splits, int kper, FlowTail ft) {
   __shared__ float red[FO_FWD_WAVES][N][FO_PX];
   const int lane = threadIdx.x & 63;
   const int wave = __builtin_amdgcn_readfirstlane(threadIdx.x >> 6);
@@ -34,6 +60,11 @@
 #pragma unroll
   for (int o = 0; o < N; ++o) acc[o] = 0.f;
   const float* xb = x + (size_t)b * K * plane;
+  const int eo = threadIdx.x / FO_PX;
+  const long long eq = (long long)blockIdx.x * FO_PX + (threadIdx.x % FO_PX);
+  const bool elive = threadIdx.x < N * FO_PX && eq < plane;
+  const size_t ei = ((size_t)b * N + (elive ? eo : 0)) * plane + (elive ? eq : 0);
+  const FlowTailIn fti = flow_tail_fetch(ft, elive, ei);
   constexpr int U = 8;
   for (int c0 = kbeg + wave; c0 < kend; c0 += U * FO_FWD_WAVES) {
     float v[U][9];
@@ -70,8 +101,13 @@
     for (int g = 0; g < FO_FWD_WAVES; ++g) s += red[g][o][l];
     const long long q = (long long)blockIdx.x * FO_PX + l;
     if (q < plane) {
-      if (splits > 1) out[(((size_t)split * nb + b) * N + o) * plane + q] = s;
-      else out[((size_t)b * N + o) * plane + q] = s + (bias ? bias[o] : 0.f);
+      if (splits > 1) {
+        out[(((size_t)split * nb + b) * N + o) * plane + q] = s;
+      } else {
+        const float v = s + (bias ? bias[o] : 0.f);
+        out[((size_t)b * N + o) * plane + q] = v;
+        flow_tail_store(ft, fti, ei, v);
+      }
     }
   }
 }
@@ -82,7 +118,7 @@
 template <int N>
 __global__ __launch_bounds__(FO_PX* FO_FWD_WAVES) void conv3x3_fewout_fwd_lds_kernel(
     const float* __restrict__ x, const float* __restrict__ w, const float* __restrict__ bias,
-    float* __restrict__ out, int K, int H, int W, int splits, int kper) {
+    float* __restrict__ out, int K, int H, int W, int splits, int kper, FlowTail ft) {
   typedef float f32x4 __attribute__((ext_vector_type(4)));
   __shared__ float red[FO_FWD_WAVES][N][FO_PX];
   __shared__ __attribute__((aligned(16))) float seg[FO_FWD_WAVES][FO_UL][3][FO_SEG];
@@ -121,6 +157,11 @@
 #pragma unroll
   for (int o = 0; o < N; ++o) acc[o] = 0.f;
   const float* xb = x + (size_t)b * K * plane;
+  const int eo = threadIdx.x / FO_PX;
+  const long long eq = p0 + (threadIdx.x % FO_PX);
+  const bool elive = threadIdx.x < N * FO_PX && eq < plane;
+  const size_t ei = ((size_t)b * N + (elive ? eo : 0)) * plane + (elive ? eq : 0);
+  const FlowTailIn fti = flow_tail_fetch(ft, elive, ei);
   float* mine = &seg[wave][0][0][0];
   for (int c0 = kbeg + wave; c0 < kend; c0 += FO_UL * FO_FWD_WAVES) {
     f32x4 t[FO_UL];
@@ -167,19 +208,28 @@
     for (int g = 0; g < FO_FWD_WAVES; ++g) sum += red[g][o][l];
     const long long q = p0 + l;
     if (q < plane) {
-      if (splits > 1) out[(((size_t)split * nb + b) * N + o) * plane + q] = sum;
-      else out[((size_t)b * N + o) * plane + q] = sum + (bias ? bias[o] : 0.f);
+      if (splits > 1) {
+        out[(((size_t)split * nb + b) * N + o) * plane + q] = sum;
+      } else {
+        const float v = sum + (bias ? bias[o] : 0.f);
+        out[((size_t)b * N + o) * plane + q] = v;
+        flow_tail_store(ft, fti, ei, v);
+      }
     }
   }
 }
 
 __global__ void fewout_reduce_kernel(const float* __restrict__ part, const float* __restrict__ bias,
-                                     float* __restrict__ out, long long n, long long plane, int N, int splits) {
+                                     float* __restrict__ out, long long n, long long plane, int N, int splits,
+                                     FlowTail ft) {
   const long long step = (long long)gridDim.x * blockDim.x;
   for (long long i = (long long)blockIdx.x * blockDim.x + threadIdx.x; i < n; i += step) {
+    const FlowTailIn fti = flow_tail_fetch(ft, true, (size_t)i);
     float s = 0.f;
     for (int k = 0; k < splits; ++k) s += part[(size_t)k * n + i];
-    out[i] = s + (bias ? bias[(i / plane) % N] : 0.f);
+    const float v = s + (bias ? bias[(i / plane) % N] : 0.f);
+    out[i] = v;
+    flow_tail_store(ft, fti, (size_t)i, v);
   }
 }
 
@@ -401,8 +451,8 @@
   return splits > 1 ? (size_t)splits * B * N * plane * sizeof(float) : 0;
 }
 
-extern "C" int pcfa_conv3x3_fewout_fwd(const float* x, const float* w, const float* bias, float* out,
-                                       void* workspace, int B, int K, int N, int H, int W, void* stream) {
+static int fewout_fwd(const float* x, const float* w, const float* bias, float* out, void* workspace, int B, int K,
+                      int N, int H, int W, FlowTail tail, void* stream) {
   if (!x || !w || !out || B < 1 || K < 1 || H < 1 || W < 1) return PCFA_ERR_INVALID_ARG;
   if (N < 1 || N > 4) return PCFA_ERR_UNSUPPORTED;
   const long long plane = (long long)H * W;
@@ -413,19 +463,20 @@
   dim3 grid(pcfa_cdiv(plane, FO_PX), B * splits), block(FO_PX * FO_FWD_WAVES);
   hipStream_t s = (hipStream_t)stream;
   const bool wide = plane % 4 == 0 && (reinterpret_cast<uintptr_t>(x) & 15) == 0;
+  const FlowTail ft = splits > 1 ? FlowTail{nullptr, nullptr, nullptr, nullptr} : tail;
   if (wide) {
     switch (N) {
-      case 1: pcfa_launch(conv3x3_fewout_fwd_lds_kernel<1>, grid, block, 0, s, x, w, bias, dst, K, H, W, splits, kper); break;
-      case 2: pcfa_launch(conv3x3_fewout_fwd_lds_kernel<2>, grid, block, 0, s, x, w, bias, dst, K, H, W, splits, kper); break;
-      case 3: pcfa_launch(conv3x3_fewout_fwd_lds_kernel<3>, grid, block, 0, s, x, w, bias, dst, K, H, W, splits, kper); break;
-      default: pcfa_launch(conv3x3_fewout_fwd_lds_kernel<4>, grid, block, 0, s, x, w, bias, dst, K, H, W, splits, kper); break;
+      case 1: pcfa_launch(conv3x3_fewout_fwd_lds_kernel<1>, grid, block, 0, s, x, w, bias, dst, K, H, W, splits, kper, ft); break;
+      case 2: pcfa_launch(conv3x3_fewout_fwd_lds_kernel<2>, grid, block, 0, s, x, w, bias, dst, K, H, W, splits, kper, ft); break;
+      case 3: pcfa_launch(conv3x3_fewout_fwd_lds_kernel<3>, grid, block, 0, s, x, w, bias, dst, K, H, W, splits, kper, ft); break;
+      default: pcfa_launch(conv3x3_fewout_fwd_lds_kernel<4>, grid, block, 0, s, x, w, bias, dst, K, H, W, splits, kper, ft); break;
     }
   } else {
     switch (N) {
-      case 1: pcfa_launch(conv3x3_fewout_fwd_kernel<1>, grid, block, 0, s, x, w, bias, dst, K, H, W, splits, kper); break;
-      case 2: pcfa_launch(conv3x3_fewout_fwd_kernel<2>, grid, block, 0, s, x, w, bias, dst, K, H, W, splits, kper); break;
-      case 3: pcfa_launch(conv3x3_fewout_fwd_kernel<3>, grid, block, 0, s, x, w, bias, dst, K, H, W, splits, kper); break;
-      default: pcfa_launch(conv3x3_fewout_fwd_kernel<4>, grid, block, 0, s, x, w, bias, dst, K, H, W, splits, kper); break;
+      case 1: pcfa_launch(conv3x3_fewout_fwd_kernel<1>, grid, block, 0, s, x, w, bias, dst, K, H, W, splits, kper, ft); break;
+      case 2: pcfa_launch(conv3x3_fewout_fwd_kernel<2>, grid, block, 0, s, x, w, bias, dst, K, H, W, splits, kper, ft); break;
+      case 3: pcfa_launch(conv3x3_fewout_fwd_kernel<3>, grid, block, 0, s, x, w, bias, dst, K, H, W, splits, kper, ft); break;
+      default: pcfa_launch(conv3x3_fewout_fwd_kernel<4>, grid, block, 0, s, x, w, bias, dst, K, H, W, splits, kper, ft); break;
     }
   }
   PCFA_LAUNCH_CHECK();
@@ -434,10 +485,24 @@
     long long blocks = (n + 255) / 256;
     if (blocks > 1024) blocks = 1024;
     pcfa_launch(fewout_reduce_kernel, dim3((int)blocks), dim3(256), 0, s, (const float*)workspace, bias, out, n, plane,
-                N, splits);
+                N, splits, tail);
     PCFA_LAUNCH_CHECK();
   }
   return PCFA_OK;
+}
+
+extern "C" int pcfa_conv3x3_fewout_fwd(const float* x, const float* w, const float* bias, float* out,
+                                       void* workspace, int B, int K, int N, int H, int W, void* stream) {
+  return fewout_fwd(x, w, bias, out, workspace, B, K, N, H, W, FlowTail{nullptr, nullptr, nullptr, nullptr}, stream);
+}
+
+extern "C" int pcfa_conv3x3_fewout_flow_fwd(const float* x, const float* w, const float* bias, const float* coords1_in,
+                                            const float* coords0, float* delta, float* coords1_out, float* flow,
+                                            void* workspace, int B, int K, int N, int H, int W, void* stream) {
+  if (!coords1_in || !coords0 || !coords1_out || !flow) return PCFA_ERR_INVALID_ARG;
+  if (N != 2) return PCFA_ERR_UNSUPPORTED;
+  return fewout_fwd(x, w, bias, delta, workspace, B, K, N, H, W, FlowTail{coords1_in, coords0, coords1_out, flow},
+                    stream);
 }
 
 extern "C" int pcfa_conv3x3_fewout_bwd(const float* grad_out, const float* w, const float* addend, float* grad_x, int B,
@@ -499,7 +564,7 @@
     long long blocks = (n + 255) / 256;
     if (blocks > 1024) blocks = 1024;
     pcfa_launch(fewout_reduce_kernel, dim3((int)blocks), dim3(256), 0, s, (const float*)workspace, bias, out, n,
-                4 * plane, N, splits);
+                4 * plane, N, splits, FlowTail{nullptr, nullptr, nullptr, nullptr});
     PCFA_LAUNCH_CHECK();
   }
   return PCFA_OK;
diff --git a/pcfa_amd/nets/raft.py b/pcfa_amd/nets/raft.py
--- a/pcfa_amd/nets/raft.py
+++ b/pcfa_amd/nets/raft.py
@@ -244,6 +244,17 @@
     def forward(self, x):
         return _predict_flow(self.conv2, _conv_relu(self.conv1, x))
 
+    def step(self, x, coords1, coords0, next_channels=0):
+        o = ops.get()
+        y = _conv_relu(self.conv1, x)
+        c = self.conv2
+        if (hasattr(o, "flow_head_step") and y.is_cuda and _frozen_conv(c) and c.bias is not None
+                and c.stride == (1, 1) and c.padding == (1, 1) and c.dilation == (1, 1) and c.groups == 1
+                and c.padding_mode == "zeros"):
+            return o.flow_head_step(y, c.weight, c.bias, coords1, coords0, next_channels)
+        delta = _predict_flow(c, y)
+        return (delta,) + tuple(o.flow_step(coords1, delta, coords0))
+
 
 class SepConvGRU(nn.Module):
 
@@ -341,7 +352,7 @@
         return (flow.shape[0] == 1 and _all_frozen(self)
                 and all(_is_plain3x3(c) for c in (self.convc2, self.convf2, self.conv)))
 
-    def forward(self, flow, corr, defer_relu=False):
+    def forward(self, flow, corr, defer_relu=False, flow_in_place=False):
         cor1 = corr.conv_relu(self.convc1) if isinstance(corr, LookupRef) else _conv_relu(self.convc1, corr)
         if self.can_defer_relu(flow):
             o = ops.get()
@@ -349,7 +360,7 @@
             cf = o.conv3x3_cat([(cor1, self.convc2.weight, self.convc2.bias), (flo1, self.convf2.weight, self.convf2.bias)],
                                grad_premasked=defer_relu)
             return o.conv3x3_cat([(cf, self.conv.weight, self.conv.bias)], (flow,), grad_premasked=defer_relu,
-                                 mask_input_grads=defer_relu)
+                                 mask_input_grads=defer_relu, **({"adopt_tail": True} if flow_in_place else {}))
         if defer_relu:
             raise RuntimeError("BasicMotionEncoder: defer_relu needs the in-place path (check can_defer_relu first)")
         cor = _conv_relu(self.convc2, cor1)
@@ -385,14 +396,14 @@
         self.mask = _mask_head()
         self._mask_cache = {}
 
-    def forward(self, net, inp, corr, flow, want_mask=True, gru_ctx=None):
+    def forward(self, net, inp, corr, flow, want_mask=True, gru_ctx=None, step=None, flow_in_place=False):
         defer = cfg(self).defer_relu and gru_ctx is not None and self.encoder.can_defer_relu(flow)
-        motion_features = self.encoder(flow, corr, defer_relu=defer)
+        motion_features = self.encoder(flow, corr, defer_relu=defer, flow_in_place=flow_in_place)
         if gru_ctx is not None:
             net = self.gru.step(net, gru_ctx, motion_features, self.encoder.RELU_CHANNELS if defer else 0)
         else:
             net = self.gru(net, torch.cat([inp, motion_features], dim=1))
-        delta_flow = self.flow_head(net)
+        delta_flow = self.flow_head(net) if step is None else self.flow_head.step(net, *step)
         mask = mask_logits(self.mask, net, self._mask_cache) if want_mask else None
         return net, mask, delta_flow
 
@@ -403,7 +414,8 @@
 
 def coords_grid(batch, ht, wd, device, dtype=torch.float32):
     ys, xs = torch.meshgrid(torch.arange(ht, device=device), torch.arange(wd, device=device), indexing="ij")
-    return torch.stack([xs, ys], dim=0).to(dtype)[None].repeat(batch, 1, 1, 1)
+    grid = torch.stack([xs, ys], dim=0).to(dtype)[None]
+    return grid if batch == 1 else grid.repeat(batch, 1, 1, 1)
 
 
 def convex_upsample(flow, mask):
@@ -458,23 +470,31 @@
 
         N, _, H, W = image1.shape
         coords0 = coords_grid(N, H // 8, W // 8, image1.device, _f32(image1).dtype)
-        coords1 = coords_grid(N, H // 8, W // 8, image1.device, _f32(image1).dtype)
-        if flow_init is not None:
-            coords1 = coords1 + flow_init
+        coords1 = coords0 if flow_init is None else coords0 + flow_init
 
         gru = self.update_block.gru
         gru_ctx = gru.per_iteration(gru.precompute(inp), iters) if gru.frozen() else None
         flow_predictions = []
         flow_up = None
-        flow_cur = coords1 - coords0
+        enc = self.update_block.encoder
+        mf_channels = (enc.RELU_CHANNELS + 2 if hasattr(ops.get(), "flow_head_step") and coords1.is_cuda
+                       and enc.can_defer_relu(coords1) else 0)
+        flow_in_place = mf_channels > 0 and not coords1.requires_grad
+        if flow_in_place:
+            first = torch.empty((1, mf_channels) + tuple(coords1.shape[2:]), device=coords1.device, dtype=coords1.dtype)
+            flow_cur = torch.sub(coords1, coords0, out=first[:, mf_channels - 2:])
+        else:
+            flow_cur = coords1 - coords0
         for itr in range(iters):
             coords1 = coords1.detach()
             corr = LookupRef(corr_fn, coords1)
             flow = flow_cur.detach()
             need_up = (not test_mode) or itr == iters - 1
-            net, up_mask, delta_flow = self.update_block(net, inp, corr, flow, want_mask=need_up,
-                                                         gru_ctx=None if gru_ctx is None else gru_ctx[itr])
-            coords1, flow_cur = ops.get().flow_step(coords1, delta_flow, coords0)
+            nxt = mf_channels if itr + 1 < iters else 0
+            net, up_mask, (delta_flow, coords1, flow_cur) = self.update_block(
+                net, inp, corr, flow, want_mask=need_up, gru_ctx=None if gru_ctx is None else gru_ctx[itr],
+                step=(coords1, coords0, nxt), flow_in_place=flow_in_place)
+            flow_in_place = nxt > 0
             if need_up:
                 flow_up = convex_upsample(flow_cur, up_mask)
                 flow_predictions.append(flow_up)
diff --git a/pcfa_amd/ops/conv.py b/pcfa_amd/ops/conv.py
--- a/pcfa_amd/ops/conv.py
+++ b/pcfa_amd/ops/conv.py
@@ -492,7 +492,17 @@
             raise ValueError("conv3x3_cat: batch size 1 only")
         plane = H * W
         widths = [w.shape[0] for w in ws] + [t.shape[1] for t in tails]
-        buf = torch.empty((1, sum(widths), H, W), device=xs[0].device, dtype=torch.float32)
+        buf = None
+        if flags & 4 and len(tails) == 1:
+            t, total = tails[0], sum(widths)
+            if (t.is_contiguous() and tuple(t.shape) == (1, widths[-1], H, W)
+                    and t.untyped_storage().nbytes() == 4 * total * plane
+                    and t.storage_offset() == (total - widths[-1]) * plane):
+                buf = torch.empty(0, device=t.device, dtype=torch.float32).set_(
+                    t.untyped_storage(), 0, (1, total, H, W), (total * plane, plane, W, 1))
+        adopted = buf is not None
+        if not adopted:
+            buf = torch.empty((1, sum(widths), H, W), device=xs[0].device, dtype=torch.float32)
         off, packs, fwds, offs = 0, [], [], []
         for x, w, b in zip(xs, ws, bs):
             if tuple(x.shape) != (1, w.shape[1], H, W) or tuple(w.shape[2:]) != (3, 3):
@@ -514,7 +524,8 @@
                 _conv3x3_run(x.device, _ptr(x), fwd, _ptr(b), None, None, _ptr_off(buf, o_ * plane), 1, w.shape[1],
                              w.shape[0], H, W, 1, 0.)
         for t in tails:
-            buf[:, off:off + t.shape[1]].copy_(t)
+            if not adopted:
+                buf[:, off:off + t.shape[1]].copy_(t)
             off += t.shape[1]
         ctx.packs, ctx.dims, ctx.n_conv, ctx.tail_widths = packs, (H, W), n_conv, [t.shape[1] for t in tails]
         ctx.save_for_backward(buf, *(xs if ctx.mask_input_grads else ()))
@@ -551,11 +562,12 @@
         return tuple(grads)
 
 
-def conv3x3_cat(convs, tails=(), grad_premasked=False, mask_input_grads=False):
+def conv3x3_cat(convs, tails=(), grad_premasked=False, mask_input_grads=False, adopt_tail=False):
     flat = []
     for x, w, b in convs:
         flat += [x, w, b]
-    return _Conv3x3Cat.apply(len(convs), int(bool(grad_premasked)) | 2 * int(bool(mask_input_grads)), *flat, *tails)
+    return _Conv3x3Cat.apply(len(convs), int(bool(grad_premasked)) | 2 * int(bool(mask_input_grads))
+                             | 4 * int(bool(adopt_tail)), *flat, *tails)
 
 
 class _DenseBlock(torch.autograd.Function):
diff --git a/pcfa_amd/ops/core.py b/pcfa_amd/ops/core.py
--- a/pcfa_amd/ops/core.py
+++ b/pcfa_amd/ops/core.py
@@ -208,6 +208,7 @@
     "pcfa_instnorm_fwd": lambda a: _note_work("instnorm_fwd", 2.0 * a[4] * a[5] * 4, 0.0),
     "pcfa_instnorm_bwd": lambda a: _note_work("instnorm_bwd", 3.0 * a[5] * a[6] * 4, 0.0),
     "pcfa_conv3x3_fewout_fwd": lambda a: _note_work("conv3x3_fewout_fwd", 4.0 * a[5] * (a[6] + a[7]) * a[8] * a[9], 0.0),
+    "pcfa_conv3x3_fewout_flow_fwd": lambda a: _note_work("conv3x3_fewout_fwd", 4.0 * a[9] * (a[10] + a[11]) * a[12] * a[13], 0.0),
     "pcfa_conv3x3_fewout_bwd": lambda a: _note_work("conv3x3_fewout_bwd", 4.0 * a[4] * (a[5] + a[6]) * a[7] * a[8], 0.0),
     "pcfa_relu_bwd": lambda a: _note_work("relu_bwd", 12.0 * a[3], 0.0),
     "pcfa_relu_bwd2": lambda a: _note_work("relu_bwd2", 20.0 * a[5], 0.0),
diff --git a/pcfa_amd/ops/corr.py b/pcfa_amd/ops/corr.py
--- a/pcfa_amd/ops/corr.py
+++ b/pcfa_amd/ops/corr.py
@@ -28,7 +28,7 @@
                                              state.L)
         ctx.state = state
         ctx.save_for_backward(f1)
-        return torch.zeros(1, device=f1.device, dtype=torch.float32)
+        return torch.empty(1, device=f1.device, dtype=torch.float32)
 
     @staticmethod
     def backward(ctx, grad_token):
diff --git a/pcfa_amd/ops/gru.py b/pcfa_amd/ops/gru.py
--- a/pcfa_amd/ops/gru.py
+++ b/pcfa_amd/ops/gru.py
@@ -7,7 +7,7 @@
 from .. import _hip
 from . import core
 from .core import _call, _dev, _note_work, _pair, _ptr, _ptr_off, _stream
-from .conv import _sepconv5_packed, _SepConv5
+from .conv import _sepconv5_packed, _SepConv5, conv3x3_fewout
 
 
 def _plane_channels(t):
@@ -302,6 +302,60 @@
     return _FlowStep.apply(coords1, delta, coords0)
 
 
+_FLOW_TAIL = os.environ.get("PCFA_FLOW_TAIL", "1") != "0"
+
+
+class _FlowHeadStep(torch.autograd.Function):
+
+    @staticmethod
+    def forward(ctx, x, weight, bias, coords1, coords0, next_channels):
+        _dev(x, weight, bias, coords1, coords0)
+        ctx.set_materialize_grads(False)
+        B, K, H, W = x.shape
+        w = weight.detach().contiguous()
+        c1, c0 = coords1.contiguous(), coords0.contiguous()
+        delta, c1n = torch.empty_like(c1), torch.empty_like(c1)
+        if next_channels:
+            fl = torch.empty((1, next_channels, H, W), device=x.device, dtype=torch.float32)[:, next_channels - 2:]
+        else:
+            fl = torch.empty_like(c1)
+        nws = int(_hip.load().pcfa_conv3x3_fewout_workspace_bytes(B, K, 2, H, W))
+        ws = torch.empty(nws // 4, device=x.device, dtype=torch.float32) if nws else None
+        _call("pcfa_conv3x3_fewout_flow_fwd", _ptr(x), _ptr(w), _ptr(bias), _ptr(c1), _ptr(c0), _ptr(delta), _ptr(c1n),
+              _ptr(fl), _ptr(ws), B, K, 2, H, W)
+        ctx.save_for_backward(w)
+        ctx.dims = (B, K, H, W)
+        return delta, c1n, fl
+
+    @staticmethod
+    @torch.autograd.function.once_differentiable
+    def backward(ctx, gd, g1, g2):
+        if ctx.needs_input_grad[1] or ctx.needs_input_grad[2]:
+            raise RuntimeError("flow_head_step is the frozen-weight path: no weight / bias gradient")
+        gc = g1 if g2 is None else g2 if g1 is None else g1 + g2
+        g = gd if gc is None else gc if gd is None else gd + gc
+        gx = None
+        if g is not None and ctx.needs_input_grad[0]:
+            (w,) = ctx.saved_tensors
+            B, K, H, W = ctx.dims
+            g = g.contiguous()
+            gx = torch.empty((B, K, H, W), device=g.device, dtype=torch.float32)
+            _call("pcfa_conv3x3_fewout_bwd", _ptr(g), _ptr(w), None, _ptr(gx), B, K, 2, H, W)
+        return (gx, None, None, gc if ctx.needs_input_grad[3] else None,
+                (None if gc is None else -gc) if ctx.needs_input_grad[4] else None, None)
+
+
+def flow_head_step(x, weight, bias, coords1, coords0, next_channels=0):
+    fused = (_FLOW_TAIL and x.dim() == 4 and x.is_contiguous() and tuple(weight.shape) == (2, x.shape[1], 3, 3)
+             and coords1.shape == coords0.shape == (x.shape[0], 2) + tuple(x.shape[2:]))
+    if fused:
+        if next_channels and x.shape[0] != 1:
+            next_channels = 0
+        return _FlowHeadStep.apply(x, weight, bias, coords1, coords0, int(next_channels))
+    delta = conv3x3_fewout(x, weight, bias)
+    return (delta,) + flow_step(coords1, delta, coords0)
+
+
 def fanout(x, n):
     return _Fanout.apply(x, n) if n > 1 else (x,)
 
diff --git a/pcfa_amd/ops/profiling.py b/pcfa_amd/ops/profiling.py
--- a/pcfa_amd/ops/profiling.py
+++ b/pcfa_amd/ops/profiling.py
@@ -52,6 +52,7 @@
         "pcfa_pwc_warp_bwd": [("pwc_warp_bwd", 1)],
         "pcfa_pwc_warp_bwd_det": [("pwc_warp_bwd", 1)],
         "pcfa_conv3x3_fewout_fwd": [("conv3x3_fewout_fwd", 0)],
+        "pcfa_conv3x3_fewout_flow_fwd": [("conv3x3_fewout_fwd", 0)],
         "pcfa_conv3x3_fewout_bwd": [("conv3x3_fewout_bwd", 0)],
         "pcfa_instnorm_fwd": [("instnorm_stats_fwd", 0), ("instnorm_apply_fwd", 1)],
         "pcfa_instnorm_bwd": [("instnorm_stats_bwd", 0), ("instnorm_apply_bwd", 1)],
```

New measurement: 7.619 attack_steps/s (median of 6 runs). No clear change (+0.6%).
